# alibaba/graph-gpt

Measured on AMD Instinct MI355X. Metric: graph-tokens/sec (un-padded Eulerian tokens, whole job) + SMTP loss, PCQM4M-v2 base pre-train, higher is better.
Workload: dtype bf16; 1 GPU; pcqm4m-v2-pretrain-base; model=base d768/L12/H12 (122.1M params), per_gpu_batch=256, global_batch=256, seq_len=32, stacked_feat=13, vocab=756, parallelism=dp1, step=fwd+bwd+allreduce+clip+AdamW, reproducible_mode=True

## Files before the change

graph-gpt_amd/_lib.py:

```python
from __future__ import annotations

import contextlib
import ctypes as C
import os

HERE = os.path.dirname(os.path.abspath(__file__))
LIB_PATH = os.environ.get("GGET_LIB_PATH") or os.path.join(HERE, "lib", "libgget_hip.so")

i32, i64, u64, f32, vp, cp = C.c_int32, C.c_int64, C.c_uint64, C.c_float, C.c_void_p, C.c_char_p


class GgetConfig(C.Structure):
    _fields_ = [(n, i32) for n in ("kind", "vocab_size", "hidden_size", "intermediate_size", "num_layers", "num_heads",
                                   "stacked_feat", "next_n_token", "gated_agg", "causal", "max_position", "num_labels",
                                   "score_bias", "pad_token_id")] + \
               [("rms_eps", f32), ("rope_theta", f32), ("layer_scale_init", f32), ("max_tokens", i32), ("max_batch", i32),
                ("path_pdrop", f32), ("mlp_pdrop", f32), ("head_mlp_layers", i32), ("head_mlp", i32 * 4), ("embed_dim", i32)]


class GgetSizes(C.Structure):
    _fields_ = [(n, u64) for n in ("n_params", "param_bf16_bytes", "master_bytes", "adam_bytes", "grad_bf16_bytes",
                                   "workspace_bytes")]


class GgetBuffers(C.Structure):
    _fields_ = [(n, vp) for n in ("param_bf16_dev", "master_dev", "adam_m_dev", "adam_v_dev", "grad_bf16_dev",
                                  "workspace_dev", "rope_cos_dev", "rope_sin_dev")]


class GgetParamInfo(C.Structure):
    _fields_ = [("name", C.c_char * 96), ("ndim", i32), ("shape", i64 * 2), ("offset", u64), ("layer", i32)]


SIGNATURES = {
    "gget_last_error": (cp, []),
    "gget_version": (i32, []),
    "gget_query_sizes": (i32, [C.POINTER(GgetConfig), C.POINTER(GgetSizes)]),
    "gget_create": (i32, [C.POINTER(GgetConfig), C.POINTER(GgetBuffers), C.POINTER(vp)]),
    "gget_destroy": (i32, [vp]),
    "gget_param_count": (i32, [vp]),
    "gget_param_info": (i32, [vp, i32, C.POINTER(GgetParamInfo)]),
    "gget_bucket_count": (i32, [vp]),
    "gget_bucket_range": (i32, [vp, i32, C.POINTER(u64), C.POINTER(u64)]),
    "gget_sync_params": (i32, [vp, vp]),
    "gget_grad_acc_attach": (i32, [vp, vp]),
    "gget_grad_accumulate": (i32, [vp, vp]),
    "gget_grad_acc_count": (i32, [vp, C.POINTER(i32)]),
    "gget_grad_acc_set_count": (i32, [vp, i32]),
    "gget_set_frozen": (i32, [vp, i32]),
    "gget_trainable_ranges": (i32, [vp, vp, vp]),
    "gget_bucket_train_range": (i32, [vp, i32, C.POINTER(u64), C.POINTER(u64)]),
    "gget_ema_attach": (i32, [vp, vp]),
    "gget_set_ema_decay": (i32, [vp, f32]),
    "gget_ema_update": (i32, [vp, f32, vp]),
    "gget_ema_to_params": (i32, [vp, vp]),
    "gget_forward_pretrain": (i32, [vp, vp, vp, vp, vp, vp, i32, i32, vp, vp]),
    "gget_forward_pretrain_packed": (i32, [vp, vp, vp, vp, vp, vp, i32, i32, vp, vp]),
    "gget_forward_task": (i32, [vp, vp, vp, vp, vp, vp, i32, i32, i32, vp, vp, vp, vp]),
    "gget_backward": (i32, [vp, f32, vp]),
    "gget_backward_begin": (i32, [vp, f32, vp]),
    "gget_backward_layer": (i32, [vp, i32, vp]),
    "gget_backward_end": (i32, [vp, vp]),
    "gget_adamw_step": (i32, [vp, f32, f32, f32, f32, f32, f32, f32, i32, vp, vp]),
    "gget_comm_unique_id": (i32, [vp]),
    "gget_comm_init": (i32, [vp, i32, i32, vp]),
    "gget_comm_destroy": (i32, [vp]),
    "gget_comm_move": (i32, [vp, vp]),
    "gget_allreduce_grads_async": (i32, [vp, i32, i32, vp]),
    "gget_allreduce_range_async": (i32, [vp, u64, u64, i32, vp]),
    "gget_comm_init_loopback": (i32, [vp, i32]),
    "gget_shard_plan": (i32, [C.POINTER(GgetConfig), i32, i32, C.POINTER(u64)]),
    "gget_shard_init": (i32, [vp, i32, i32, C.POINTER(i32)]),
    "gget_shard_bucket": (i32, [vp, i32, C.POINTER(u64)]),
    "gget_reduce_scatter_grads_async": (i32, [vp, i32, i32, vp]),
    "gget_shard_sqnorm_partials": (i32, [vp, vp, vp]),
    "gget_shard_allgather_async": (i32, [vp, i32, vp, vp]),
    "gget_adamw_step_sharded": (i32, [vp, f32, f32, f32, f32, f32, f32, f32, i32, vp, vp, vp]),
    "gget_head_counts": (i32, [vp, C.POINTER(i32 * 2), vp]),
    "gget_head_logits": (i32, [vp, C.POINTER(vp), C.POINTER(i32)]),
    "gget_hidden_states": (i32, [vp, C.POINTER(vp)]),
    "gget_layer_hidden_states": (i32, [vp, i32, C.POINTER(vp)]),
    "gget_hidden_states_grid": (i32, [vp, i32, vp, vp]),
    "gget_op_gemm": (i32, [i32, i32, vp, vp, vp, vp, i32, i32, i32, i32, i32, i32, i32, vp]),
    "gget_op_gemm_streamk": (i32, [i32, i32, vp, vp, vp, vp, i32, i32, i32, i32, i32, i32, vp, vp]),
    "gget_op_gemm_streamk_bytes": (u64, []),
    "gget_debug_set": (i32, [i32, i32]),
    "gget_debug_get": (i32, [i32, C.POINTER(i32)]),
    "gget_debug_occupy": (i32, [vp, u64, i32, i32, i32, vp]),
    "gget_op_gemm_grouped": (i32, [i32, i32, vp, vp, vp, vp, vp, vp, vp, vp, vp, vp]),
    "gget_op_rmsnorm_fwd": (i32, [vp, vp, vp, vp, i32, i32, f32, vp]),
    "gget_op_rmsnorm_bwd": (i32, [vp, vp, vp, vp, vp, vp, vp, i32, i32, vp]),
    "gget_op_embed_fwd": (i32, [vp, vp, vp, vp, i32, i32, i32, i32, vp]),
    "gget_op_embed_bwd": (i32, [vp, vp, vp, vp, vp, vp, i32, i32, i32, i32, i32, i32, vp]),
    "gget_op_qkv_rope": (i32, [vp, vp, vp, vp, vp, vp, i32, i32, i32, vp]),
    "gget_op_smtp2d": (i32, [vp, i32, vp, i32, vp, vp, i32, i32, i32, f32, f32, f32, i32, i32, C.c_uint32, vp]),
    "gget_op_token_sample": (i32, [vp, i32, i32, i32, i32, f32, f32, i32, f32, C.c_uint32, vp, vp, vp]),
    "gget_op_unmask_origin": (i32, [vp, vp, i32, i32, f32, C.c_uint32, i32, vp]),
    "gget_op_token_confidence": (i32, [vp, i32, i32, i32, i32, vp, vp, vp]),
    "gget_op_smtp_rows": (i32, [vp, vp, vp, vp, vp, i32, i32, i32, C.c_double, C.c_double, C.c_double, C.c_uint32, vp]),
    "gget_op_rope": (i32, [vp, vp, vp, vp, i32, i32, i32, i32, vp]),
    "gget_op_attn_fwd": (i32, [vp, vp, vp, vp, i32, i32, i32, i32, vp, vp, vp, f32, C.c_uint32, vp]),
    "gget_op_attn_bwd": (i32, [vp, vp, vp, vp, vp, vp, vp, i32, i32, i32, i32, vp, vp, vp, f32, C.c_uint32, vp]),
    "gget_op_copy_from_host": (i32, [vp, vp, C.c_uint64, vp]),
    "gget_op_attn_fwd_varlen": (i32, [vp, vp, vp, vp, vp, i32, i32, i32, i32, vp, vp, vp, i32, f32, C.c_uint32, vp]),
    "gget_op_attn_bwd_varlen": (i32, [vp, vp, vp, vp, vp, vp, vp, vp, i32, i32, i32, i32, vp, vp, vp, i32, f32, C.c_uint32, vp]),
    "gget_op_attn_oproj_fwd": (i32, [vp, vp, vp, vp, vp, vp, vp, vp, vp, vp, vp, i32, i32, i32, i32, f32, f32, C.c_uint32, vp, vp]),
    "gget_op_pack_wo": (i32, [vp, C.c_uint64, vp, vp, i32, i32, vp]),
    "gget_op_attn_oproj_bwd": (i32, [vp, vp, vp, vp, vp, vp, vp, i32, C.c_uint64, vp, vp, vp, vp, vp, vp, i32, i32, i32, i32, vp, vp, vp, f32,
                                      C.c_uint32, i32, vp, vp, vp]),
    "gget_op_attn_fwd_ranges": (i32, [vp, vp, vp, vp, vp, i32, i32, i32, i32, f32, C.c_uint32, vp]),
    "gget_op_attn_bwd_ranges": (i32, [vp, vp, vp, vp, vp, vp, vp, vp, i32, i32, i32, i32, f32, C.c_uint32, vp]),
    "gget_op_ranges_from_mask3d": (i32, [vp, vp, vp, i32, i32, vp]),
    "gget_op_attn_bwd_fused": (i32, [vp, vp, vp, vp, vp, vp, vp, vp, vp, vp, i32, i32, i32, i32, f32, C.c_uint32, vp]),
    "gget_set_dropout": (i32, [vp, f32, f32, C.c_uint32]),
    "gget_set_auc": (i32, [vp, i32, C.c_uint32]),
    "gget_set_token_count": (i32, [vp, C.c_int64]),
    "gget_set_option": (i32, [vp, i32, i32]),
    "gget_set_dp_menu": (i32, [vp, i32, i32]),
    "gget_varlen_status": (i32, [vp, vp, vp]),
    "gget_position_status": (i32, [vp, vp, vp]),
    "gget_deferred_status": (i32, [vp, vp, vp]),
    "gget_set_focal_gamma": (i32, [vp, f32]),
    "gget_set_stack_method": (i32, [vp, i32]),
    "gget_set_rope_range": (i32, [vp, f32]),
    "gget_set_raw_embeds": (i32, [vp, vp, i32]),
    "gget_debug_probe": (i32, [vp, i32, C.POINTER(f32)]),
    "gget_debug_gemm_probe": (i32, [i32, C.POINTER(C.c_double), C.POINTER(C.c_double), C.POINTER(i32), C.POINTER(i32)]),
    "gget_set_dropout_ex": (i32, [vp, f32, f32, f32]),
    "gget_op_gateup_geglu": (i32, [vp, vp, vp, vp, i32, i32, i32, vp]),
    "gget_op_down_dgrad_geglu": (i32, [vp, vp, vp, vp, vp, i32, i32, i32, vp]),
    "gget_op_geglu_fwd": (i32, [vp, vp, i32, i32, vp]),
    "gget_op_geglu_bwd": (i32, [vp, vp, vp, i32, i32, vp]),
    "gget_op_ce_fwd_bwd": (i32, [vp, i32, vp, vp, vp, i32, i32, vp, vp, f32, i32, vp]),
    "gget_op_score_fwd": (i32, [vp, vp, vp, vp, vp, vp, i32, i32, i32, vp]),
    "gget_op_score_bwd": (i32, [vp, vp, vp, vp, vp, vp, vp, i32, i32, i32, vp]),
    "gget_op_tok_score_fwd": (i32, [vp, vp, vp, vp, i32, i32, i32, vp]),
    "gget_op_tok_intra_fwd": (i32, [vp, vp, vp, vp, i32, i32, i32, vp]),
    "gget_op_tok_intra_bwd": (i32, [vp, vp, vp, vp, vp, vp, i32, i32, i32, vp]),
    "gget_set_cls_idx": (i32, [vp, vp]),
    "gget_op_tok_ce": (i32, [vp, vp, vp, vp, vp, i32, i32, vp, i32, vp]),
    "gget_op_tok_score_bwd": (i32, [vp, vp, vp, vp, vp, vp, vp, i32, i32, i32, vp]),
    "gget_op_task_loss": (i32, [vp, vp, vp, i32, i32, i32, vp, vp, vp]),
    "gget_op_auc_loss": (i32, [vp, vp, i32, i32, i32, C.c_uint32, vp, vp, vp, vp]),
    "gget_op_pool_rows": (i32, [vp, vp, vp, i32, i32, vp]),
    "gget_op_scatter_rows_f32": (i32, [vp, vp, vp, i32, i32, vp]),
    "gget_op_head_linear_fwd": (i32, [vp, vp, vp, vp, vp, vp, i32, i32, i32, i32, vp]),
    "gget_op_head_linear_bwd": (i32, [vp, vp, vp, vp, vp, vp, vp, i32, i32, i32, i32, vp]),
    "gget_op_rank_metrics_workspace": (C.c_size_t, [i32, i32]),
    "gget_op_rank_metrics": (i32, [vp, i32, vp, i32, i32, i32, vp, vp, vp, vp, vp, vp, C.c_size_t, vp]),
    "gget_op_link_hits_workspace": (C.c_size_t, [i32]),
    "gget_op_link_hits": (i32, [vp, vp, i32, i64, vp, vp, vp, vp, vp, vp, C.c_size_t, vp]),
    "gget_op_link_mrr_workspace": (C.c_size_t, [i32]),
    "gget_op_link_mrr": (i32, [vp, vp, vp, i32, i32, i32, vp, vp, vp, vp, vp, vp, vp, vp, C.c_size_t, vp]),
}

GEMM_NT, GEMM_NN, GEMM_TN = 0, 1, 2
OPT_NORM_FROM_BACKWARD = 1
OPT_SKIP_NONFINITE_STEP = 2
SHARD_CHUNK = 4096
SHARD_PARAMS, SHARD_MASTER, SHARD_ADAM_M, SHARD_ADAM_V, SHARD_SLOTS, SHARD_EMA = 0, 1, 2, 3, 4, 5
TOKENS_AUTO = -2
EPI_NONE, EPI_RESIDUAL, EPI_ATOMIC_F32, EPI_SLAB_F32 = 0, 1, 2, 3

KEY_GEMM_VARIANT, KEY_GEMM_LDS_HEADROOM, KEY_GEMM_SPLIT_LAST, KEY_DETERMINISTIC, KEY_GEMM_STAGGER = 1, 2, 3, 4, 5
KEY_GEMM_ABLATE, KEY_HEAD_DENSE, KEY_HEAD_TILE, KEY_ATTN_OPROJ_OFF, KEY_LS_NORM_BWD_WIDE = 7, 8, 9, 10, 11
KEY_RMS_WIDE, KEY_CE_PARTS, KEY_GEMM_CU_RESERVE, KEY_OCCUPY_FAT, KEY_LINK_GRID = 13, 14, 15, 16, 18
MENU_KEYS = (1, 2, 3, 4, 5, 7, 8, 9, 10, 11, 13, 14, 15, 16, 18)
GEMM_NO_KSPLIT_ND, GEMM_NO_KSPLIT_WGRAD, GEMM_NO_192_ROWS, GEMM_NO_SPLIT_LAST, GEMM_KSPLIT_128_ONLY, GEMM_ONE_BLOCK_PER_CU = 1, 2, 4, 8, 16, 32
GEMM_KSPLIT_DMA8, GEMM_AREA_RULE = 128, 512


def debug_get(key: int) -> int:
    v = i32()
    check(load().gget_debug_get(int(key), C.byref(v)))
    return int(v.value)


@contextlib.contextmanager
def debug_menu(keys):
    saved = {k: debug_get(k) for k in keys}
    try:
        for k, v in keys.items():
            check(load().gget_debug_set(int(k), int(v)))
        yield
    finally:
        for k, v in saved.items():
            check(load().gget_debug_set(k, v))


def gemm_grouped(lib, mode, problems, stream):
    n = len(problems)
    PA, IA = vp * n, i32 * n
    ptr = lambda k: PA(*[p[k].data_ptr() for p in problems])
    num = lambda k: IA(*[int(p[k]) for p in problems])
    return lib.gget_op_gemm_grouped(mode, n, ptr(0), ptr(1), ptr(2), num(3), num(4), num(5), num(6), num(7), num(8), stream)
PROBLEM_SINGLE_LABEL, PROBLEM_REGRESSION_L1, PROBLEM_REGRESSION_MSE, PROBLEM_MULTI_LABEL, PROBLEM_AUC = 0, 1, 2, 3, 4
PROBLEM_TOKEN_CE_INTRA = 6
PROBLEM_TOKEN_CE = 5

_lib = None


class GgetError(RuntimeError):
    pass


def load(path: str = LIB_PATH):
    global _lib
    if _lib is not None:
        return _lib
    import torch
    if not os.path.exists(path):
        raise GgetError(f"{path} is missing: build it with `python graph-gpt_amd/build.py` "
                        "(or __graft_entry__.build()); this engine has no CPU fallback")
    lib = C.CDLL(path)
    for name, (res, args) in SIGNATURES.items():
        fn = getattr(lib, name)
        fn.restype = res
        fn.argtypes = args
    _lib = lib
    return lib


def check(rc: int):
    if rc != 0:
        raise GgetError(f"gget error {rc}: {load().gget_last_error().decode()}")
```

graph-gpt_amd/build.py:

```python
from __future__ import annotations

import hashlib
import os
import shutil
import subprocess
import sys

HERE = os.path.dirname(os.path.abspath(__file__))
CSRC = os.path.join(HERE, "csrc")
LIBDIR = os.path.join(HERE, "lib")
LIB = os.path.join(LIBDIR, "libgget_hip.so")
SOURCES = ["engine.hip", "gemm.hip", "kernels.hip", "attention.hip", "menu.hip", "metrics.hip"]
HEADERS = ["common.h", "gemm.h", "kernels.h", "menu.h", os.path.join("..", "..", "include", "gget.h")]
FLAGS = ["--offload-arch=gfx950", "-O3", "-std=c++17", "-fPIC", "-fno-gpu-rdc", "-Wall", "-Wno-unused-function"]
EXTRA_FLAGS = {}


def _hipcc() -> str:
    for cand in (os.environ.get("HIPCC"), shutil.which("hipcc"), "/opt/rocm/bin/hipcc"):
        if cand and os.path.exists(cand):
            return cand
    raise RuntimeError("hipcc not found (set HIPCC)")


def _digest() -> str:
    h = hashlib.sha256()
    for f in SOURCES + HEADERS:
        with open(os.path.join(CSRC, f), "rb") as fh:
            h.update(fh.read())
    h.update(" ".join(FLAGS).encode())
    h.update(repr(sorted(EXTRA_FLAGS.items())).encode())
    return h.hexdigest()


def build(force: bool = False, verbose: bool = False) -> str:
    os.makedirs(LIBDIR, exist_ok=True)
    stamp = os.path.join(LIBDIR, "libgget_hip.stamp")
    dig = _digest()
    if not force and os.path.exists(LIB) and os.path.exists(stamp) and open(stamp).read().strip() == dig:
        return LIB
    hipcc = _hipcc()
    objdir = os.path.join(HERE, "build")
    os.makedirs(objdir, exist_ok=True)
    objs = []
    procs = []
    for src in SOURCES:
        obj = os.path.join(objdir, src.replace(".hip", ".o"))
        cmd = [hipcc, *FLAGS, *EXTRA_FLAGS.get(src, []), "-c", os.path.join(CSRC, src), "-o", obj]
        if verbose:
            print(" ".join(cmd), flush=True)
        procs.append((src, subprocess.Popen(cmd, stdout=subprocess.PIPE, stderr=subprocess.STDOUT, text=True)))
        objs.append(obj)
    for src, p in procs:
        out, _ = p.communicate()
        if p.returncode != 0:
            raise RuntimeError(f"hipcc failed on {src}:\n{out}")
        if verbose and out.strip():
            print(out)
    cmd = [hipcc, "--offload-arch=gfx950", "-shared", "-fPIC", "-o", LIB, *objs]
    r = subprocess.run(cmd, stdout=subprocess.PIPE, stderr=subprocess.STDOUT, text=True)
    if r.returncode != 0:
        raise RuntimeError(f"link failed:\n{r.stdout}")
    with open(stamp, "w") as fh:
        fh.write(dig)
    return LIB


if __name__ == "__main__":
    print(build(force="--force" in sys.argv, verbose=True))
```

graph-gpt_amd/csrc/engine.hip:

```cpp
#include <dlfcn.h>
#include <stdarg.h>
#include <stdio.h>
#include <string.h>

#include <algorithm>
#include <chrono>
#include <string>
#include <functional>
#include <vector>

#include "common.h"
#include "gemm.h"
#include "kernels.h"
#include <rccl/rccl.h>

static thread_local char g_err[512] = "";
void gget_set_error(const char* fmt, ...) {
  va_list ap;
  va_start(ap, fmt);
  vsnprintf(g_err, sizeof(g_err), fmt, ap);
  va_end(ap);
}
extern "C" const char* gget_last_error(void) { return g_err; }
extern "C" int gget_version(void) { return 101; }
// ... 1505 lines not shown
    if (int e = k_gather_rows_remap(h->wsp<bf16_t>(w.hidden), h->wsp<int32_t>(w.row_idx), counts, h->wsp<int32_t>(w.vl_pad2c),
                                    h->wsp<bf16_t>(w.Hm), T, d, h->T > h->tc ? h->tc : 0, labels_dev ? h->wsp<int32_t>(w.vl_status) : nullptr, st))
      return e;
  } else if (int e = k_gather_rows(h->wsp<bf16_t>(w.hidden), h->wsp<int32_t>(w.row_idx), counts, h->wsp<bf16_t>(w.Hm), T, d, 0, st))
    return e;
  h->head_sorted_fwd = false;
  if (sorted_head) {
    if (int e = k_head_slot_sort(h->wsp<int32_t>(w.sel_src), h->wsp<int32_t>(w.row_idx), counts + 1, h->wsp<int32_t>(w.ss_state),
                                 h->wsp<int32_t>(w.ss_tok), h->wsp<int32_t>(w.ss_cell), h->wsp<int32_t>(w.ss_l), h->wsp<int32_t>(w.ss_pos),
                                 h->wsp<int32_t>(w.ss_tile), h->wsp<int32_t>(w.ss_total), T * n, n, (long)d * d, head_tile_rows(d), st))
      return e;
    GemmGroup g;
    memset(&g, 0, sizeof(g));
    g.count = 1;
    GemmProblem& p = g.p[0];
    p.A = h->wsp<bf16_t>(w.hidden); p.B = h->P + h->plan.ntp; p.C = h->wsp<bf16_t>(w.Hl);
    p.M = T * n + n * 256; p.N = d; p.K = d; p.lda = d; p.ldb = d; p.ldc = d;
    p.m_dev = h->wsp<int32_t>(w.ss_total);
    p.a_rows = h->wsp<int32_t>(w.ss_tok); p.b_tile_off = h->wsp<int32_t>(w.ss_tile); p.c_rows = h->wsp<int32_t>(w.ss_l);
    p.b_tile_rows = head_tile_rows(d);
    if (int e = gget_gemm_launch(GGET_GEMM_NT, GGET_EPI_NONE, g, 1, st)) return e;
    h->head_sorted_fwd = true;
  } else if (h->plan.has_ntp) {
    if (int e = gemm_nt(h->wsp<bf16_t>(w.Hm), h->P + h->plan.ntp, h->wsp<bf16_t>(w.Pp), nullptr, T, n * d, d, d, d, n * d,
                        counts, st))
      return e;
    if (int e = k_gather_rows(h->wsp<bf16_t>(w.Pp), h->wsp<int32_t>(w.sel_src), counts + 1, h->wsp<bf16_t>(w.Hl), T * n, d, 0,
                              st))
      return e;
  }
  if (int e = gemm_nt(h->wsp<bf16_t>(w.Hl), h->P + h->plan.lm, h->wsp<bf16_t>(w.logits), nullptr, T * n, V, d, d, d, Vp,
                      counts + 1, st))
    return e;
  h->have_labels = labels_dev != nullptr;
  if (h->stack_long && labels_dev) {
    if (int e = k_sample_mask_wgt(labels_dev, h->wsp<float>(w.long_wgt), B, S * n, st)) return e;
    sample_wgt_dev = h->wsp<float>(w.long_wgt);
  }
  h->sample_wgt = sample_wgt_dev;
  if (labels_dev) {
    const int mean_rows = sample_wgt_dev == nullptr;
    const float base = 1.0f / (float)((long)B * S * n);
    if (int e = k_ce_fwd_bwd(h->wsp<bf16_t>(w.logits), Vp, h->wsp<int32_t>(w.sel_label), h->wsp<int32_t>(w.sel_tok),
                             sample_wgt_dev, S, counts + 1, T * n, V, h->wsp<float>(w.loss_sum), h->wsp<bf16_t>(w.dlogits),
                             base, mean_rows, loss_dev, st, mean_rows ? h->focal_gamma : 0.f, h->wsp<float>(w.loss_part), 2048))
      return e;
    if (h->varlen && h->tc_from_caller && loss_dev)
      if (int e = k_poison_loss(h->wsp<int32_t>(w.vl_status), loss_dev, st)) return e;
  }
  h->fwd_valid = true;
  return 0;
}

extern "C" int gget_forward_pretrain(gget_handle_t h, const int64_t* input_ids_dev, const int64_t* attention_mask_dev,
                                     const int64_t* labels_dev, const float* sample_wgt_dev,
                                     const int64_t* position_ids_dev, int B, int S, float* loss_dev, void* stream) {
  return forward_pretrain_impl(h, input_ids_dev, attention_mask_dev, false, labels_dev, sample_wgt_dev, position_ids_dev, B, S,
                               loss_dev, stream);
}

extern "C" int gget_forward_pretrain_packed(gget_handle_t h, const int64_t* input_ids_dev, const int64_t* attention_mask3d_dev,
                                            const int64_t* labels_dev, const float* sample_wgt_dev,
                                            const int64_t* position_ids_dev, int B, int S, float* loss_dev, void* stream) {
  GGET_REQUIRE(attention_mask3d_dev != nullptr, "the packed forward needs the [B,S,S] mask");
  return forward_pretrain_impl(h, input_ids_dev, attention_mask3d_dev, true, labels_dev, sample_wgt_dev, position_ids_dev, B, S,
                               loss_dev, stream);
}

extern "C" int gget_forward_task(gget_handle_t h, const int64_t* input_ids_dev, const int64_t* attention_mask_dev,
                                 const int64_t* position_ids_dev, const void* task_labels_dev, const float* sample_wgt_dev,
                                 int problem_type, int B, int S, float* loss_dev, float* task_logits_dev,
                                 void* task_hidden_dev, void* stream) {
  GGET_REQUIRE(h != nullptr, "null argument");
  const long tc_hint = h->tc_next;
  h->tc_next = -1;
  const int64_t* cls_idx_dev = h->cls_idx_next;
  h->cls_idx_next = nullptr;
  GGET_REQUIRE(input_ids_dev, "null argument");
  GGET_REQUIRE(h->cfg.kind == GGET_KIND_TASK, "handle was not created as a task model");
  const bool tok = problem_type == GGET_PROBLEM_TOKEN_CE || problem_type == GGET_PROBLEM_TOKEN_CE_INTRA;
  GGET_REQUIRE(problem_type != GGET_PROBLEM_TOKEN_CE_INTRA || cls_idx_dev, "the intra-instance token head needs cls_idx (gget_set_cls_idx)");
  hipStream_t st = (hipStream_t)stream;
  const gget_config_t& c = h->cfg;
  CallScope scope(h);
  h->fwd_valid = false;
  if (int e = backbone_forward(h, tc_hint, input_ids_dev, c.stacked_feat, attention_mask_dev, position_ids_dev, B, S, st, false, nullptr))
    return e;
  const Ws& w = h->ws;
  const int d = c.hidden_size, C = c.num_labels;
  float* lg = h->wsp<float>(w.tlogits);
  GGET_REQUIRE(!tok || h->plan.n_lin == 0, "the token-level head is the Linear `score` (no MLP head)");
  if (h->plan.n_lin > 0) {
    const Plan& pl = h->plan;
    if (int e = k_pool_rows(h->wsp<bf16_t>(w.hidden), h->wsp<int32_t>(w.pool_row), h->wsp<bf16_t>(w.pooled_h), B, d, st)) return e;
    for (int i = 0; i < pl.n_lin; ++i)
      if (int e = k_head_linear_fwd(h->wsp<bf16_t>(w.head_x[i]), h->wsp<bf16_t>(w.head_a[i]), h->P + pl.head_w[i],
                                    c.score_bias ? h->P + pl.head_b[i] : nullptr, h->wsp<bf16_t>(w.head_x[i + 1]),
                                    i + 1 == pl.n_lin ? lg : nullptr, B, pl.head_dim[i], pl.head_dim[i + 1], i, h->head_drop(), st))
        return e;
  } else if (problem_type == GGET_PROBLEM_TOKEN_CE) {
    if (int e = k_tok_score_fwd(h->wsp<bf16_t>(w.hidden), h->P + h->plan.score, c.score_bias ? h->P + h->plan.sbias : nullptr, lg, h->T, C,
                                d, st))
      return e;
    if (int e = k_pool_rows(h->wsp<bf16_t>(w.hidden), h->wsp<int32_t>(w.pool_row), h->wsp<bf16_t>(w.pooled_h), B, d, st)) return e;
  } else if (problem_type == GGET_PROBLEM_TOKEN_CE_INTRA) {
    if (int e = k_intra_plan(cls_idx_dev, h->wsp<int32_t>(w.key_len), h->varlen ? h->wsp<int32_t>(w.vl_cu) : nullptr, h->wsp<int32_t>(w.intra_rs),
                             h->wsp<int64_t>(w.intra_cls), h->wsp<int32_t>(w.vl_status) + 4, B, S, C, st))
      return e;
    if (int e = k_tok_intra_fwd(h->wsp<bf16_t>(w.hidden), h->wsp<int32_t>(w.intra_rs), h->wsp<int64_t>(w.intra_cls), lg, B, C, d, st)) return e;
    if (int e = k_pool_rows(h->wsp<bf16_t>(w.hidden), h->wsp<int32_t>(w.pool_row), h->wsp<bf16_t>(w.pooled_h), B, d, st)) return e;
  } else if (int e = k_score_fwd(h->wsp<bf16_t>(w.hidden), h->wsp<int32_t>(w.pool_row), h->P + h->plan.score,
                                 c.score_bias ? h->P + h->plan.sbias : nullptr, lg, h->wsp<bf16_t>(w.pooled_h), B, C, d, st))
    return e;
  const int rows = tok ? h->T : B;
  const bool tok_vl = tok && h->varlen;
  if (task_logits_dev && tok_vl) {
    GGET_HIP_CHECK(hipMemsetAsync(task_logits_dev, 0, (size_t)B * S * C * 4, st));
    if (int e = k_scatter_rows_map_f32(lg, h->wsp<int32_t>(w.vl_c2p), task_logits_dev, h->T, C, B * S, st)) return e;
  } else if (task_logits_dev) GGET_HIP_CHECK(hipMemcpyAsync(task_logits_dev, lg, (size_t)rows * C * 4, hipMemcpyDeviceToDevice, st));
  if (task_hidden_dev)
    GGET_HIP_CHECK(hipMemcpyAsync(task_hidden_dev, h->wsp<bf16_t>(w.pooled_h), (size_t)B * d * 2, hipMemcpyDeviceToDevice, st));
  h->have_labels = task_labels_dev != nullptr;
  h->problem = problem_type;
  if (task_labels_dev) {
    GGET_REQUIRE(loss_dev != nullptr, "loss_dev is required when task labels are given");
    if (problem_type == GGET_PROBLEM_AUC) {
      GGET_REQUIRE(C >= 2, "the AUC loss reads logits[:, 1] - logits[:, 0]");
      if (int e = k_auc_loss(lg, (const int64_t*)task_labels_dev, B, C, h->auc_num_neg, h->auc_seed, loss_dev,
                             h->wsp<float>(w.tdlogits), h->wsp<int32_t>(w.auc_lists), st))
        return e;
    } else if (tok) {
      if (int e = k_tok_ce(lg, (const int64_t*)task_labels_dev, h->wsp<float>(w.tdlogits), h->wsp<float>(w.tok_stat), loss_dev, rows, C, st,
                           tok_vl ? h->wsp<int32_t>(w.vl_c2p) : nullptr, B * S))
        return e;
    } else if (int e = k_task_loss(lg, task_labels_dev, sample_wgt_dev, problem_type, B, C, loss_dev, h->wsp<float>(w.tdlogits), st))
      return e;
    if (h->varlen && h->tc_from_caller)
      if (int e = k_poison_loss(h->wsp<int32_t>(w.vl_status), loss_dev, st)) return e;
  }
  h->fwd_valid = true;
  return 0;
}

namespace {

int convert_bucket(gget_engine* h, int bucket, hipStream_t st) {
  if (h->defer_convert) return 0;
  if (h->truncated() && h->bucket_train_range(bucket).second == 0) return 0;
  const auto& bs = h->bucket_segs[bucket];
  return k_convert_segments(h->wsp<float>(h->ws.scratch32), h->G,
                            reinterpret_cast<const GgetSegment*>(h->W + h->ws.segs) + bs.first, bs.second, st);
}

int layer_backward(gget_engine* h, int i, hipStream_t st) {
  const gget_config_t& c = h->cfg;
  const int T = h->T, d = c.hidden_size, ff = c.intermediate_size, H = c.num_heads;
  const LayerOff& lo = h->plan.layers[i];
  const LayerWs& lw = h->ws.lw[i];
  const Ws& w = h->ws;
  float* s32 = h->wsp<float>(w.scratch32);
  bf16_t* bufs[3] = {h->wsp<bf16_t>(w.dxa), h->wsp<bf16_t>(w.dxb), h->wsp<bf16_t>(w.dxc)};
  bf16_t* dx_out = h->dx_cur;
  int oi = 0;
  while (oi < 3 && bufs[oi] != dx_out) ++oi;
  GGET_REQUIRE(oi < 3, "backward stages called out of order");
  bf16_t* dx_mid = bufs[(oi + 1) % 3];
  bf16_t* dx_in = bufs[(oi + 2) % 3];
  bf16_t* x_in = h->wsp<bf16_t>(w.xres[i]);
  bf16_t* xmid = h->wsp<bf16_t>(lw.xmid);
  bf16_t* dxn = h->wsp<bf16_t>(w.dxn);
  bf16_t* dqkv = h->wsp<bf16_t>(w.dqkv);
  bf16_t* dattn = h->wsp<bf16_t>(w.dattn);
  bf16_t* dgu = h->wsp<bf16_t>(w.dgu);
  bf16_t* dh = h->wsp<bf16_t>(w.dh);
  const bf16_t* dy_down = dx_out;
  const bf16_t* dy_o = nullptr;
  const int ls_rl = 256 / (d / 8);
  dim3 lsgrid((unsigned)std::min(512, (T + ls_rl - 1) / ls_rl));
  const size_t ls_lds_bytes = (size_t)ls_rl * d * sizeof(float);
  const bool fuse_ls = h->plan.has_res && ls_norm_fused();
  if (h->plan.has_res) {
    bf16_t* dsc = h->wsp<bf16_t>(w.dscaled);
    if (!h->ls2_done)
      hipLaunchKernelGGL(ls_bwd_kernel, lsgrid, dim3(256), ls_lds_bytes, st, dx_out, h->wsp<bf16_t>(lw.mraw),
                         h->plan.has_ls ? h->P + lo.lam2 : nullptr, dsc, h->plan.has_ls ? s32 + lo.lam2_32 : nullptr, T, d,
                         h->path_drop(i, 1), kAccumCopies, align_up((uint64_t)d, 128), h->mlp_drop(i));
    h->ls2_done = false;
    dy_down = dsc;
  }
  if (h->mlp_drop_p > 0.f) {
    if (int e = gemm_nn(dy_down, h->P + lo.wdown, dh, T, ff, d, d, ff, ff, nullptr, st)) return e;
    if (int e = k_elem_dropout(dh, T, ff, GGET_DROP_STREAM_MLP_ACT, h->mlp_drop(i), st)) return e;
    if (int e = k_geglu_bwd(h->wsp<bf16_t>(lw.gu), dh, dgu, T, ff, st)) return e;
  } else if (int e = down_dgrad_geglu(dy_down, h->P + lo.wdown, h->wsp<bf16_t>(lw.gu), dgu, dh, T, d, ff, st)) return e;
  if (int e = gemm_nn(dgu, h->P + lo.wgu, dxn, T, d, 2 * ff, 2 * ff, d, d, nullptr, st)) return e;
  bool front_fused = false;
  const bool ao_bwd_ok = menu().gemm_cu_reserve > 0 ? h->B <= gget_gemm_num_cu() : menu().gemm_lds_headroom < 2;
  if (!h->plan.has_res && !h->klo() && h->wo_packed && ao_bwd_ok) {
    int taken = 0;
    if (int e = k_attn_oproj_bwd(dxn, xmid, h->P + lo.ln2, h->wsp<float>(lw.rstd2), dx_out, dx_mid, s32 + lo.ln2_32, kAccumCopies,
                                 align_up((uint64_t)d, 128), h->wsp<bf16_t>(w.wot_pack) + (size_t)i * d * d, h->wsp<bf16_t>(lw.qkv),
                                 h->wsp<float>(lw.lse), h->wsp<int32_t>(w.key_len), h->row_base(), dqkv, h->B, h->S, H, c.causal, h->cos_cur,
                                 h->sin_cur, h->pos_cur, h->attn_drop_p, h->attn_drop_seed + 0x9E37u * (unsigned)i, T, st, &taken,
                                 dattn, h->long_list()))
      return e;
    front_fused = taken != 0;
  }
  if (front_fused) {
  } else if (fuse_ls) {
    if (int e = rmsnorm_bwd_ls(dxn, xmid, h->P + lo.ln2, h->wsp<float>(lw.rstd2), dx_out, dx_mid, s32 + lo.ln2_32, h->wsp<bf16_t>(lw.araw),
                               h->plan.has_ls ? h->P + lo.lam1 : nullptr, h->wsp<bf16_t>(w.dscaled2),
                               h->plan.has_ls ? s32 + lo.lam1_32 : nullptr, T, d, h->path_drop(i, 0), ElemDropArg{0, 1.f, 0}, st))
      return e;
  } else if (int e = k_rmsnorm_bwd(dxn, xmid, h->P + lo.ln2, h->wsp<float>(lw.rstd2), dx_out, dx_mid, s32 + lo.ln2_32, T, d, st, kAccumCopies, align_up((uint64_t)d, 128)))
    return e;
  dy_o = dx_mid;
  if (fuse_ls) {
    dy_o = h->wsp<bf16_t>(w.dscaled2);
  } else if (h->plan.has_res) {
    bf16_t* dsc = h->wsp<bf16_t>(w.dscaled2);
    hipLaunchKernelGGL(ls_bwd_kernel, lsgrid, dim3(256), ls_lds_bytes, st, dx_mid, h->wsp<bf16_t>(lw.araw),
                       h->plan.has_ls ? h->P + lo.lam1 : nullptr, dsc, h->plan.has_ls ? s32 + lo.lam1_32 : nullptr, T, d,
                       h->path_drop(i, 0), kAccumCopies, align_up((uint64_t)d, 128), ElemDropArg{0, 1.f, 0});
    dy_o = dsc;
  }
  if (!front_fused)
  if (int e = gemm_nn(dy_o, h->P + lo.wo, dattn, T, d, d, d, d, d, nullptr, st)) return e;
  if (!front_fused)
  if (int e = k_attn_bwd(h->wsp<bf16_t>(lw.qkv), h->wsp<bf16_t>(lw.attn), dattn, h->wsp<float>(lw.lse),
                         h->wsp<int32_t>(w.key_len), dqkv, h->wsp<float>(w.delta), h->B, h->S, H, c.causal, h->cos_cur,
                         h->sin_cur, h->pos_cur, 1, h->attn_drop_p, h->attn_drop_seed + 0x9E37u * (unsigned)i, st,
                         h->klo(), h->khi(), h->row_base(),
                         (w.dq_acc && (uint64_t)(h->S + 255) / 256 <= (c.max_tokens / (c.max_batch > 0 ? c.max_batch : 1) + 255) / 256) ? h->wsp<bf16_t>(w.dq_acc) : nullptr,
                         (size_t)c.max_tokens * d, h->long_list()))
    return e;
  if (int e = gemm_nn(dqkv, h->P + lo.wqkv, dxn, T, d, 3 * d, 3 * d, d, d, nullptr, st)) return e;
  const bool boundary = h->truncated() && i == h->frozen;
  const bool fuse_next = fuse_ls && i > 0 && !boundary;
  if (boundary) {
    if (int e = k_rmsnorm_dw(dxn, x_in, h->wsp<float>(lw.rstd1), s32 + lo.ln1_32, T, d, st, kAccumCopies, align_up((uint64_t)d, 128))) return e;
  } else if (!fuse_next)
    if (int e = k_rmsnorm_bwd(dxn, x_in, h->P + lo.ln1, h->wsp<float>(lw.rstd1), dx_mid, dx_in, s32 + lo.ln1_32, T, d, st, kAccumCopies, align_up((uint64_t)d, 128)))
      return e;
  const GemmProblem wg_gu{dgu, h->wsp<bf16_t>(lw.xn2), h->G + lo.wgu, nullptr, 2 * ff, d, T, 2 * ff, d, d, nullptr, nullptr, 0, 0};
  const GemmProblem wg_dn{dy_down, h->wsp<bf16_t>(lw.h), h->G + lo.wdown, nullptr, d, ff, T, d, ff, ff, nullptr, nullptr, 0, 0};
  const long t192[4] = {(long)2 * ff * d / (192 * 192), (long)d * ff / (192 * 192), (long)3 * d * d / (192 * 192), (long)d * d / (192 * 192)};
  int n_grouped = 4;
  if (d % 192 == 0 && ff % 192 == 0 && menu().gemm_cu_reserve > 0) {
    long acc_t = 0;
    n_grouped = 0;
    for (int q = 0; q < 4 && acc_t + t192[q] <= gget_gemm_num_cu(); ++q) { acc_t += t192[q]; ++n_grouped; }
    if (n_grouped < 2) n_grouped = 4;
  }
  if (d % 192 == 0 && ff % 192 == 0) {
    GemmGroup g;
    memset(&g, 0, sizeof(g));
    g.count = n_grouped;
    g.p[0] = wg_gu;
    g.p[1] = wg_dn;
    g.p[2] = GemmProblem{dqkv, h->wsp<bf16_t>(lw.xn1), h->G + lo.wqkv, nullptr, 3 * d, d, T, 3 * d, d, d, nullptr, nullptr, 0, 0};
    g.p[3] = GemmProblem{dy_o, h->wsp<bf16_t>(lw.attn), h->G + lo.wo, nullptr, d, d, T, d, d, d, nullptr, nullptr, 0, 0};
    const long wg_tiles = ((long)2 * ff * d + (long)d * ff + (long)4 * d * d) / (192 * 192);
    g.sq_partials = n_grouped == 4 && h->opt_norm_from_backward && wg_tiles <= kSqTilesPerLayer ? h->wsp<float>(w.sq_tiles) + (size_t)i * kSqTilesPerLayer : nullptr;
    if (h->probe) GGET_HIP_CHECK(hipEventRecord(h->probe_event(0, 2 * i), st));
    if (int e = gget_gemm_launch(GGET_GEMM_TN, GGET_EPI_NONE, g, 1, st)) return e;
    if (h->probe) GGET_HIP_CHECK(hipEventRecord(h->probe_event(0, 2 * i + 1), st));
    if (g.sq_written) {
      if (wg_tiles < kSqTilesPerLayer)
        GGET_HIP_CHECK(hipMemsetAsync(h->wsp<float>(w.sq_tiles) + (size_t)i * kSqTilesPerLayer + wg_tiles, 0, (kSqTilesPerLayer - wg_tiles) * sizeof(float), st));
      ++h->sq_layers;
    }
    if (n_grouped < 4) {
      float* wg = h->wsp<float>(w.wg32);
      const bool with_qkv = n_grouped == 2;
      const long slab = with_qkv ? (long)4 * d * d : (long)d * d;
      const int max_slabs = with_qkv ? kWgSplit : 4 * kWgSplit;
      const int rows_out = with_qkv ? 4 * d : d;
      const int t_big = ((rows_out + 255) / 256) * ((d + 127) / 128), t_small = ((rows_out + 127) / 128) * ((d + 127) / 128);
      int split = fit_split(t_big, max_slabs);
      if (t_big * split < 160) split = fit_split(t_small, max_slabs);
      while (split > 1 && (T + 63) / 64 < 4 * split) --split;
      GemmGroup go;
      memset(&go, 0, sizeof(go));
      if (with_qkv) {
        go.count = 2;
        go.p[0] = GemmProblem{dqkv, h->wsp<bf16_t>(lw.xn1), wg, nullptr, 3 * d, d, T, 3 * d, d, d, nullptr, nullptr, 0, 0, slab};
        go.p[1] = GemmProblem{dy_o, h->wsp<bf16_t>(lw.attn), wg + (size_t)3 * d * d, nullptr, d, d, T, d, d, d, nullptr, nullptr, 0, 0, slab};
      } else {
        go.count = 1;
        go.p[0] = GemmProblem{dy_o, h->wsp<bf16_t>(lw.attn), wg, nullptr, d, d, T, d, d, d, nullptr, nullptr, 0, 0, slab};
      }
      if (int e = gget_gemm_launch(GGET_GEMM_TN, GGET_EPI_SLAB_F32, go, split, st)) return e;
      const int ktiles = (T + 63) / 64, per = (ktiles + split - 1) / split;
      if (int e = k_slab_reduce(wg, slab, (ktiles + per - 1) / per, h->G + (with_qkv ? lo.wqkv : lo.wo), (size_t)slab, st)) return e;
    }
  } else {
    {
      GemmGroup g;
      memset(&g, 0, sizeof(g));
      g.count = 2;
      g.p[0] = wg_gu;
      g.p[1] = wg_dn;
      if (int e = gget_gemm_launch(GGET_GEMM_TN, GGET_EPI_NONE, g, 1, st)) return e;
    }
    float* wg = h->wsp<float>(w.wg32);
    const long slab = (long)4 * d * d;
    GemmGroup g;
    memset(&g, 0, sizeof(g));
    g.count = 2;
    g.p[0] = GemmProblem{dqkv, h->wsp<bf16_t>(lw.xn1), wg, nullptr, 3 * d, d, T, 3 * d, d, d, nullptr, nullptr, 0, 0, slab};
    g.p[1] = GemmProblem{dy_o, h->wsp<bf16_t>(lw.attn), wg + (size_t)3 * d * d, nullptr, d, d, T, d, d, d, nullptr, nullptr, 0, 0, slab};
    const int split = T >= kWgSplit * 1024 ? kWgSplit : 1;
    if (int e = gget_gemm_launch(GGET_GEMM_TN, GGET_EPI_SLAB_F32, g, split, st)) return e;
    if (int e = k_slab_reduce(wg, slab, split, h->G + lo.wqkv, (size_t)4 * d * d, st)) return e;
  }
  if (fuse_next) {
    const LayerOff& lp = h->plan.layers[i - 1];
    if (int e = rmsnorm_bwd_ls(dxn, x_in, h->P + lo.ln1, h->wsp<float>(lw.rstd1), dx_mid, dx_in, s32 + lo.ln1_32,
                               h->wsp<bf16_t>(h->ws.lw[i - 1].mraw), h->plan.has_ls ? h->P + lp.lam2 : nullptr, h->wsp<bf16_t>(w.dscaled),
                               h->plan.has_ls ? s32 + lp.lam2_32 : nullptr, T, d, h->path_drop(i - 1, 1), h->mlp_drop(i - 1), st))
      return e;
    h->ls2_done = true;
  }
  h->dx_cur = dx_in;
  return convert_bucket(h, h->bucket_of_layer(i), st);
}

}

static bool embed_dense_path(int T, int d, int V, bool gated, const ElemDropArg& E) {
  return !menu().embed_sorted && E.thresh == 0 && k_embed_dense_ok(V, gated) && T > 0 && ((long)V * d) % 4 == 0;
}

extern "C" int gget_backward_begin(gget_handle_t h, float loss_scale, void* stream) {
  GGET_REQUIRE(h, "null handle");
  GGET_REQUIRE(h->fwd_valid && h->have_labels, "backward needs a preceding forward with labels");
  GGET_REQUIRE(loss_scale == 1.0f, "loss scaling is not used on the bf16 path (pass 1.0)");
  h->sq_layers = 0;
  CallScope scope(h);
  hipStream_t st = (hipStream_t)stream;
  const gget_config_t& c = h->cfg;
  const Ws& w = h->ws;
  const int d = c.hidden_size;
  float* s32 = h->wsp<float>(w.scratch32);
  GgetZeroRanges zr;
  zr.n = 0;
  zr.add(s32, (size_t)h->plan.n_scratch32 * 4);
  bf16_t* dhid = h->wsp<bf16_t>(w.dxb);
  zr.add(dhid, (size_t)h->T * d * 2);
  if (h->varlen && h->T > h->tc)
    zr.add(h->wsp<bf16_t>(w.dqkv) + (size_t)h->tc * 3 * d, (size_t)(h->T - h->tc) * 3 * d * 2);
  int T = h->TP;
  if (c.kind == GGET_KIND_PRETRAIN) {
    if (h->plan.has_ntp && head_scatter_fused())
      zr.add(h->wsp<bf16_t>(w.dP), (size_t)(h->varlen ? h->T : T) * c.next_n_token * d * 2);
    zr.add(h->wsp<float>(w.lm_slab), (size_t)kLmSplit * c.vocab_size * d * sizeof(float));
  }
  h->emb_cnt_cleared = false;
  if (h->ws.emb_cnt && embed_dense_path(h->T, d, c.vocab_size, h->plan.has_gate, h->embed_drop()) && zr.n < kZeroRanges &&
      !h->truncated()) {
    zr.add(h->wsp<unsigned char>(h->ws.emb_cnt), (size_t)h->T * align_up((uint64_t)c.vocab_size, 64) * 2);
    h->emb_cnt_cleared = true;
  }
  if (int e = k_zero_ranges(zr, st)) return e;
  if (c.kind == GGET_KIND_PRETRAIN) {
    const int n = c.next_n_token, V = c.vocab_size, Vp = (int)align_up(V, 64);
    int32_t* counts = h->wsp<int32_t>(w.counts);
    bf16_t* dlog = h->wsp<bf16_t>(w.dlogits);
    const bool fuse_sc = h->plan.has_ntp && head_scatter_fused();
    if (fuse_sc) {
      if (int e = gemm_nn(dlog, h->P + h->plan.lm, h->wsp<bf16_t>(w.dP), T * n, d, Vp, Vp, d, d, counts + 1, st, h->wsp<int32_t>(w.sel_src)))
        return e;
    } else if (int e = gemm_nn(dlog, h->P + h->plan.lm, h->wsp<bf16_t>(w.dHl), T * n, d, Vp, Vp, d, d, counts + 1, st)) return e;
    {
      float* slabs = h->wsp<float>(w.lm_slab);
      const long slab = (long)V * d;
      GemmGroup g;
      memset(&g, 0, sizeof(g));
      g.count = 1;
      g.p[0] = GemmProblem{dlog, h->wsp<bf16_t>(w.Hl), slabs, nullptr, V, d, T * n, Vp, d, d, nullptr, counts + 1, 0, 0, slab};
      int lm_split = fit_split(((V + 255) / 256) * ((d + 127) / 128), kLmSplit);
      if (((V + 255) / 256) * ((d + 127) / 128) * lm_split < 160) lm_split = fit_split(((V + 127) / 128) * ((d + 127) / 128), kLmSplit);
      if (int e = gget_gemm_launch(GGET_GEMM_TN, GGET_EPI_SLAB_F32, g, lm_split, st)) return e;
      if (int e = k_slab_reduce(slabs, slab, lm_split, h->G + h->plan.lm, (size_t)V * d, st)) return e;
    }
    if (h->plan.has_ntp) {
      bf16_t* dP = h->wsp<bf16_t>(w.dP);
      if (!fuse_sc) {
        GGET_HIP_CHECK(hipMemsetAsync(dP, 0, (size_t)(h->varlen ? h->T : T) * n * d * 2, st));
        if (int e = k_gather_rows(h->wsp<bf16_t>(w.dHl), h->wsp<int32_t>(w.sel_src), counts + 1, dP, T * n, d, 1, st)) return e;
      }
      if (h->head_sorted_fwd) {
        bf16_t* dxs = h->wsp<bf16_t>(w.Pp);
        GemmGroup g;
        memset(&g, 0, sizeof(g));
        g.count = 1;
        GemmProblem& p = g.p[0];
        p.A = dP; p.B = h->P + h->plan.ntp; p.C = dxs;
        p.M = T * n + n * 256; p.N = d; p.K = d; p.lda = d; p.ldb = d; p.ldc = d;
        p.m_dev = h->wsp<int32_t>(w.ss_total);
        p.a_rows = h->wsp<int32_t>(w.ss_cell); p.b_tile_off = h->wsp<int32_t>(w.ss_tile);
        p.b_tile_rows = head_tile_rows(d);
        if (int e = gget_gemm_launch(GGET_GEMM_NN, GGET_EPI_NONE, g, 1, st)) return e;
        if (int e = k_head_cell_sum(dxs, h->wsp<int32_t>(w.ss_pos), h->wsp<int32_t>(w.cnt), h->wsp<int32_t>(w.l_off),
                                    h->varlen ? h->wsp<int32_t>(w.vl_pad2c) : nullptr, dhid, T, d, h->T > h->tc ? h->tc : 0, st))
          return e;
      } else if (head_scatter_fused()) {
        if (int e = gemm_nn(dP, h->P + h->plan.ntp, dhid, T, d, n * d, n * d, d, d, counts, st, h->wsp<int32_t>(w.row_idx))) return e;
      } else if (int e = gemm_nn(dP, h->P + h->plan.ntp, h->wsp<bf16_t>(w.dHm), T, d, n * d, n * d, d, d, counts, st)) return e;
      if (int e = gget_gemm_single(GGET_GEMM_TN, GGET_EPI_NONE, dP, h->wsp<bf16_t>(w.Hm), h->G + h->plan.ntp, nullptr, n * d, d,
                                   T, n * d, d, d, nullptr, counts, 1, st, true))
        return e;
    }
    if (!(h->plan.has_ntp && (head_scatter_fused() || h->head_sorted_fwd)))
      if (int e = k_gather_rows(h->wsp<bf16_t>(w.dHm), h->wsp<int32_t>(w.row_idx), counts, dhid, T, d, 1, st)) return e;
  } else if (h->plan.n_lin > 0) {
    const Plan& pl = h->plan;
    const float* dy = h->wsp<float>(w.tdlogits);
    for (int i = pl.n_lin - 1; i >= 0; --i) {
// ... 269 lines not shown
                          float grad_scale, int step, const float* slots_dev, float* gnorm_dev, hipStream_t st) {
  GgetAdamwArgs a{};
  a.master = h->master, a.m = h->am, a.v = h->av, a.param = h->P;
  a.lr = lr, a.beta1 = beta1, a.beta2 = beta2, a.eps = eps, a.wd = weight_decay, a.step = step;
  a.max_norm = max_grad_norm, a.grad_scale = grad_scale, a.gnorm_out = gnorm_dev, a.skip_nonfinite = h->opt_skip_nonfinite;
  a.ema_decay = h->ema_decay_next;
  h->ema_decay_next = -1.f;
  a.ema = a.ema_decay >= 0.f ? h->ema : nullptr;
  h->wo_packed = false;
  float* sq = h->wsp<float>(h->ws.sqnorm);
  const bool need_norm = h->step_needs_norm(max_grad_norm, gnorm_dev);
  a.sqnorm = need_norm ? sq : nullptr;
  a.grad_f32 = h->grad_from_acc();
  a.grad = h->grad_src();
  h->grad_acc_count = 0;
  const OptWork* w = h->opt_work(sharded);
  if (need_norm) {
    if (sharded) {
      if (int e = k_grad_sqnorm_slots(slots_dev, w->slot_of, w->nglobal, sq, st)) return e;
    } else if (w) {
      if (int e = k_grad_sqnorm_chunks(a.grad, w->chunks, w->nchunks, nullptr, 0, sq, st, a.grad_f32)) return e;
    } else if (h->opt_norm_from_backward && !a.grad_f32 && grad_scale == 1.0f && h->sq_layers == h->cfg.num_layers && h->n_sq_chunks >= 0) {
      if (int e = k_grad_sqnorm_chunks(h->G, h->wsp<GgetSqChunk>(h->ws.sq_chunks), h->n_sq_chunks, h->wsp<float>(h->ws.sq_tiles),
                                       h->cfg.num_layers * kSqTilesPerLayer, sq, st))
        return e;
    } else if (int e = k_grad_sqnorm(a.grad, h->plan.n_params, sq, st, a.grad_f32)) return e;
  }
  return w ? k_adamw_items(a, w->items, w->nitems, st) : k_adamw(a, h->plan.n_params, st);
}

extern "C" int gget_adamw_step(gget_handle_t h, float lr, float beta1, float beta2, float eps, float weight_decay,
                               float max_grad_norm, float grad_scale, int step, float* gnorm_dev, void* stream) {
  GGET_REQUIRE(h && h->master && h->am && h->av, "adamw needs master/m/v arenas");
  GGET_REQUIRE(step >= 1, "step is 1-based");
  return optimizer_step(h, false, lr, beta1, beta2, eps, weight_decay, max_grad_norm, grad_scale, step, nullptr, gnorm_dev, (hipStream_t)stream);
}

extern "C" int gget_shard_plan(const gget_config_t* cfg, int world, int bucket, uint64_t out[5]) {
  if (int e = check_cfg(cfg)) return e;
  GGET_REQUIRE(out && world >= 1, "shard_plan: bad arguments (world %d)", world);
  GGET_REQUIRE(bucket >= 0 && bucket < cfg->num_layers + 2, "shard_plan: bucket %d out of range", bucket);
  const auto r = bucket_ranges(*cfg, make_plan(*cfg))[bucket];
  const ShardBucket sb = shard_bucket(r.first, r.second - r.first, world);
  out[0] = sb.off, out[1] = sb.cnt, out[2] = sb.slice, out[3] = sb.tail_off, out[4] = sb.tail_cnt;
  return 0;
}

extern "C" int gget_shard_init(gget_handle_t h, int world, int rank, int32_t* slots_per_rank) {
  GGET_REQUIRE(h && world >= 0 && (world == 0 || (rank >= 0 && rank < world)), "shard_init: bad arguments (rank %d world %d)", rank, world);
  GGET_REQUIRE(world == 0 || !(h->comm || h->comm_loopback) || (world == h->comm_world && rank == h->comm_rank),
               "shard_init: rank %d of %d does not match the communicator (rank %d of %d)", rank, world, h->comm_rank, h->comm_world);
  if (int e = h->shard_work.reset()) return e;
  h->shard_world = h->shard_rank = h->shard_slots = 0;
  h->shard_plan.clear();
  if (slots_per_rank) *slots_per_rank = 0;
  if (world == 0) return 0;
  const bool all_ranks = h->comm_loopback;
  const uint64_t C = GGET_SHARD_CHUNK;
  std::vector<ShardBucket> plan;
  for (int b = 0; b < (int)h->bucket_range.size(); ++b) {
    const auto r = h->bucket_train_range(b);
    plan.push_back(shard_bucket(r.first, r.second, world));
  }
  std::vector<GgetSqChunk> grid;
  std::vector<int> owner;
  for (const ShardBucket& b : plan)
    for (uint64_t j = 0; j * C < b.cnt; ++j) {
      grid.push_back(GgetSqChunk{b.off + j * C, std::min(C, b.cnt - j * C)});
      owner.push_back(j * C < (uint64_t)world * b.slice ? (int)(j * C / b.slice) : 0);
    }
  std::vector<int> count(world, 0);
  std::vector<int32_t> local(grid.size());
  for (size_t j = 0; j < grid.size(); ++j) local[j] = count[owner[j]]++;
  const int S = *std::max_element(count.begin(), count.end());
  std::vector<int32_t> slot_of(grid.size()), chunk_slot;
  std::vector<GgetSqChunk> chunks;
  for (size_t j = 0; j < grid.size(); ++j) {
    slot_of[j] = owner[j] * S + local[j];
    if (all_ranks || owner[j] == rank) {
      chunks.push_back(grid[j]);
      chunk_slot.push_back(slot_of[j]);
    }
  }
  std::vector<std::pair<uint64_t, uint64_t>> share;
  for (const ShardBucket& b : plan) {
    for (int r = 0; r < world; ++r)
      if (all_ranks || r == rank) share.push_back({b.off + (uint64_t)r * b.slice, b.slice});
    share.push_back({b.tail_off, b.tail_cnt});
  }
  if (int e = h->shard_work.upload(cut_items(share), chunks, chunk_slot, slot_of)) return e;
  h->shard_world = world;
  h->shard_rank = rank;
  h->shard_slots = S;
  h->shard_plan = plan;
  if (slots_per_rank) *slots_per_rank = S;
  return 0;
}

extern "C" int gget_shard_bucket(gget_handle_t h, int bucket, uint64_t out[5]) {
  GGET_REQUIRE(h != nullptr && out != nullptr, "shard_bucket: null argument");
  GGET_REQUIRE(h->shard_world > 0, "shard_bucket: no plan is active (gget_shard_init)");
  GGET_REQUIRE(bucket >= 0 && bucket < (int)h->shard_plan.size(), "shard_bucket: bucket %d out of range", bucket);
  const ShardBucket& sb = h->shard_plan[bucket];
  out[0] = sb.off, out[1] = sb.cnt, out[2] = sb.slice, out[3] = sb.tail_off, out[4] = sb.tail_cnt;
  return 0;
}

extern "C" int gget_shard_sqnorm_partials(gget_handle_t h, float* slots_dev, void* stream) {
  GGET_REQUIRE(h && h->shard_world > 0 && slots_dev, "shard_sqnorm_partials: call gget_shard_init first (and pass the slot vector)");
  const OptWork& w = h->shard_work;
  return k_grad_sqnorm_partials(h->grad_src(), w.chunks, w.chunk_slot, w.nchunks, slots_dev, (hipStream_t)stream, h->grad_from_acc());
}

extern "C" int gget_adamw_step_sharded(gget_handle_t h, float lr, float beta1, float beta2, float eps, float weight_decay,
                                       float max_grad_norm, float grad_scale, int step, const float* slots_dev, float* gnorm_dev, void* stream) {
  GGET_REQUIRE(h && h->master && h->am && h->av, "adamw needs master/m/v arenas");
  GGET_REQUIRE(h->shard_world > 0, "adamw_step_sharded: call gget_shard_init first");
  GGET_REQUIRE(step >= 1, "step is 1-based");
  GGET_REQUIRE(slots_dev || !h->step_needs_norm(max_grad_norm, gnorm_dev), "adamw_step_sharded: the norm needs the gathered partial vector");
  return optimizer_step(h, true, lr, beta1, beta2, eps, weight_decay, max_grad_norm, grad_scale, step, slots_dev, gnorm_dev, (hipStream_t)stream);
}

extern "C" int gget_head_counts(gget_handle_t h, int32_t counts[2], void* stream) {
  GGET_REQUIRE(h && counts, "null argument");
  GGET_REQUIRE(h->cfg.kind == GGET_KIND_PRETRAIN, "head counts exist only for the pre-train head");
  GGET_HIP_CHECK(hipMemcpyAsync(counts, h->wsp<int32_t>(h->ws.counts), 8, hipMemcpyDeviceToHost, (hipStream_t)stream));
  GGET_HIP_CHECK(hipStreamSynchronize((hipStream_t)stream));
  return 0;
}

extern "C" int gget_head_logits(gget_handle_t h, const void** logits_dev, int32_t* ld) {
  GGET_REQUIRE(h && logits_dev && ld, "null argument");
  GGET_REQUIRE(h->cfg.kind == GGET_KIND_PRETRAIN, "head logits exist only for the pre-train head");
  *logits_dev = h->wsp<bf16_t>(h->ws.logits);
  *ld = (int32_t)align_up(h->cfg.vocab_size, 64);
  return 0;
}

extern "C" int gget_hidden_states(gget_handle_t h, const void** hidden_dev) {
  GGET_REQUIRE(h && hidden_dev, "null argument");
  GGET_REQUIRE(!h->varlen, "hidden_states: the last forward ran on the var-len token layout (rows are compacted): run that forward on the padded grid - no token count at the C ABI, num_tokens=None with a host-side mask or GGET_VARLEN=0 through the model classes, or ask the model for output_hidden_states=True");
  *hidden_dev = h->wsp<bf16_t>(h->ws.hidden);
  return 0;
}

extern "C" int gget_layer_hidden_states(gget_handle_t h, int layer, const void** hidden_dev) {
  GGET_REQUIRE(h && hidden_dev, "null argument");
  GGET_REQUIRE(layer >= 0 && layer <= h->cfg.num_layers, "layer_hidden_states: layer %d out of range", layer);
  GGET_REQUIRE(!h->varlen, "layer_hidden_states: the last forward ran on the var-len token layout (rows are compacted): run that forward on the padded grid - no token count at the C ABI, num_tokens=None with a host-side mask or GGET_VARLEN=0 through the model classes, or ask the model for output_hidden_states=True");
  *hidden_dev = h->wsp<bf16_t>(h->ws.xres[layer]);
  return 0;
}

extern "C" int gget_hidden_states_grid(gget_handle_t h, int layer, void* out_dev, void* stream) {
  GGET_REQUIRE(h && out_dev, "null argument");
  GGET_REQUIRE(layer >= -1 && layer <= h->cfg.num_layers, "hidden_states_grid: layer %d out of range", layer);
  GGET_REQUIRE(h->B > 0 && h->S > 0, "hidden_states_grid: no forward has run");
  const bf16_t* src = layer < 0 ? h->wsp<bf16_t>(h->ws.hidden) : h->wsp<bf16_t>(h->ws.xres[layer]);
  const int d = h->cfg.hidden_size;
  const long n_pos = (long)h->B * h->S;
  if (!h->varlen) {
    GGET_HIP_CHECK(hipMemcpyAsync(out_dev, src, (size_t)n_pos * d * 2, hipMemcpyDeviceToDevice, (hipStream_t)stream));
    return 0;
  }
  return k_rows_to_grid(src, h->wsp<int32_t>(h->ws.vl_pad2c), out_dev, n_pos, d, (hipStream_t)stream);
}

__global__ void __launch_bounds__(256) occupy_kernel(float* buf, size_t n, long long ticks) {
  extern __shared__ float occ_lds[];
  const long long t0 = wall_clock64();
  float acc = 0.f;
  size_t i = ((size_t)blockIdx.x * 256 + threadIdx.x) % n;
  while (wall_clock64() - t0 < ticks) {
    acc += buf[i];
    i = (i + 65536) % n;
    if (threadIdx.x == 0) occ_lds[0] = acc;
  }
  if (acc == 1.2345e-30f) buf[0] = acc;
}
__global__ void __launch_bounds__(256) occupy_fat_kernel(float* buf, size_t n, long long ticks) {
  extern __shared__ float occ_lds[];
  asm volatile("" ::: "v255", "a7");
  const long long t0 = wall_clock64();
  float acc = 0.f;
  size_t i = ((size_t)blockIdx.x * 256 + threadIdx.x) % n;
  while (wall_clock64() - t0 < ticks) {
    acc += buf[i];
    i = (i + 65536) % n;
    if (threadIdx.x == 0) occ_lds[0] = acc;
  }
  if (acc == 1.2345e-30f) buf[0] = acc;
}
extern "C" int gget_debug_occupy(void* scratch, uint64_t scratch_bytes, int blocks, int lds_bytes, int microseconds, void* stream) {
  GGET_REQUIRE(scratch && scratch_bytes >= 4096 && blocks > 0 && lds_bytes >= 4 && lds_bytes <= 160 * 1024, "debug_occupy: bad arguments");
  static bool attr = false;
  if (!attr) {
    GGET_HIP_CHECK(hipFuncSetAttribute(reinterpret_cast<const void*>(&occupy_kernel), hipFuncAttributeMaxDynamicSharedMemorySize, 160 * 1024));
    GGET_HIP_CHECK(hipFuncSetAttribute(reinterpret_cast<const void*>(&occupy_fat_kernel), hipFuncAttributeMaxDynamicSharedMemorySize, 160 * 1024));
    attr = true;
  }
  if (menu().occupy_fat) {
    hipLaunchKernelGGL(occupy_fat_kernel, dim3(blocks), dim3(256), lds_bytes, (hipStream_t)stream, (float*)scratch, scratch_bytes / 4,
                       (long long)microseconds * 100);
    GGET_LAUNCH_CHECK();
    return 0;
  }
  hipLaunchKernelGGL(occupy_kernel, dim3(blocks), dim3(256), lds_bytes, (hipStream_t)stream, (float*)scratch, scratch_bytes / 4,
                     (long long)microseconds * 100);
  GGET_LAUNCH_CHECK();
  return 0;
}

extern "C" int gget_debug_probe(gget_handle_t h, int enable, float* avg_ms_out ) {
  GGET_REQUIRE(h != nullptr, "null handle");
  if (avg_ms_out) {
    for (int w = 0; w < 2; ++w) {
      double sum = 0.0;
      int n = 0;
      for (size_t k = 0; k + 1 < h->probe_ev[w].size(); k += 2) {
        float ms = 0.f;
        if (hipEventSynchronize(h->probe_ev[w][k + 1]) == hipSuccess && hipEventElapsedTime(&ms, h->probe_ev[w][k], h->probe_ev[w][k + 1]) == hipSuccess) {
          sum += ms;
          ++n;
        }
      }
      avg_ms_out[w] = n ? (float)(sum / n) : 0.f;
    }
  }
  h->probe = enable != 0;
  return 0;
}
extern "C" int gget_op_gemm(int mode, int epilogue, const void* A, const void* B, void* C, const void* R, int M, int N, int K,
                            int lda, int ldb, int ldc, int split_k, void* stream) {
  return gget_gemm_single(mode, epilogue, A, B, C, R, M, N, K, lda, ldb, ldc, nullptr, nullptr, split_k, (hipStream_t)stream);
}
extern "C" int gget_op_gemm_streamk(int mode, int epilogue, const void* A, const void* B, void* C, const void* R, int M, int N, int K,
                                    int lda, int ldb, int ldc, void* streamk_ws, void* stream) {
  GGET_REQUIRE(streamk_ws != nullptr, "gemm_streamk: null workspace");
  gget_gemm_streamk_workspace(streamk_ws);
  const int rc = gget_gemm_single(mode, epilogue, A, B, C, R, M, N, K, lda, ldb, ldc, nullptr, nullptr, 1, (hipStream_t)stream);
  gget_gemm_streamk_workspace(nullptr);
  return rc;
}
extern "C" uint64_t gget_op_gemm_streamk_bytes(void) { return gget_gemm_streamk_bytes(); }
extern "C" int gget_op_gemm_grouped(int mode, int count, const void* const* A, const void* const* B, void* const* Cs, const int* M,
                                   const int* N, const int* K, const int* lda, const int* ldb, const int* ldc, void* stream) {
  GGET_REQUIRE(count >= 1 && count <= GGET_MAX_GROUP && A && B && Cs && M && N && K && lda && ldb && ldc, "gemm_grouped: bad arguments");
  GemmGroup g;
  memset(&g, 0, sizeof(g));
  g.count = count;
  for (int i = 0; i < count; ++i) {
    GemmProblem& p = g.p[i];
    p.A = static_cast<const bf16_t*>(A[i]); p.B = static_cast<const bf16_t*>(B[i]); p.C = Cs[i];
    p.M = M[i]; p.N = N[i]; p.K = K[i]; p.lda = lda[i]; p.ldb = ldb[i]; p.ldc = ldc[i];
  }
  return gget_gemm_launch(mode, GGET_EPI_NONE, g, 1, (hipStream_t)stream);
}
extern "C" int gget_op_qkv_rope(const void* x, const void* wqkv, void* qkv, const float* cos_tab, const float* sin_tab,
                                const int64_t* position_ids, int T, int S, int d, void* stream) {
  GGET_REQUIRE(x && wqkv && qkv && cos_tab && sin_tab, "qkv_rope: null argument");
  GGET_REQUIRE(d > 0 && d % 64 == 0 && T > 0 && S > 0, "qkv_rope: bad shape T %d S %d d %d", T, S, d);
  GemmGroup g;
  memset(&g, 0, sizeof(g));
  g.count = 1;
  GemmProblem& p = g.p[0];
  p.A = static_cast<const bf16_t*>(x); p.B = static_cast<const bf16_t*>(wqkv); p.C = qkv;
  p.M = T; p.N = 3 * d; p.K = d; p.lda = d; p.ldb = d; p.ldc = 3 * d;
  p.rope_cos = cos_tab; p.rope_sin = sin_tab; p.rope_pos = position_ids; p.rope_S = S; p.rope_cols = 2 * d;
  return gget_gemm_launch(GGET_GEMM_NT, GGET_EPI_ROPE, g, 1, (hipStream_t)stream);
}
extern "C" int gget_op_smtp2d(const int64_t* ids_in, int ld_in, const int64_t* node_idx, int ld_node, int64_t* ids_out,
                              int64_t* labels_out, int B, int S, int F, float smtp_2d_rate, float power, float replace_rate,
                              int vocab, int global_2d_mask, uint32_t seed, void* stream) {
  GGET_REQUIRE(ids_in && node_idx && ids_out && labels_out, "smtp2d: null argument");
  GGET_REQUIRE(B >= 0 && S >= 0 && F >= 1 && ld_in >= F && ld_node >= 1 && vocab >= 2, "smtp2d: bad shape");
  return k_smtp2d(ids_in, ld_in, node_idx, ld_node, ids_out, labels_out, B, S, F, smtp_2d_rate, power, replace_rate, vocab,
                  global_2d_mask, seed, (hipStream_t)stream);
}
extern "C" int gget_op_token_sample(const void* logits, int ld, int R, int V, int mode, float temperature, float top_p, int top_k,
                                   float alg_temp, uint32_t seed, float* conf, int64_t* tok, void* stream) {
  GGET_REQUIRE(logits && conf && tok && R >= 0 && V >= 1 && ld >= V && mode >= 0 && mode <= 2, "token_sample: bad arguments");
  return k_token_sample(logits, ld, R, V, mode, temperature, top_p, top_k, alg_temp, seed, conf, tok, (hipStream_t)stream);
}
extern "C" int gget_op_unmask_origin(int64_t* x, const int64_t* cand, int B, int N, float p_transfer, uint32_t seed, int mask_token_id,
                                     void* stream) {
  GGET_REQUIRE(x && cand && B >= 0 && N >= 0, "unmask_origin: bad arguments");
  return k_unmask_origin(x, cand, B, N, p_transfer, seed, mask_token_id, (hipStream_t)stream);
}
extern "C" int gget_op_token_confidence(const void* logits, int ld, int R, int V, int mode, float* conf, int64_t* tok, void* stream) {
  GGET_REQUIRE(logits && conf && tok, "token_confidence: null argument");
  GGET_REQUIRE(R >= 0 && V >= 2 && ld >= V && mode >= 0 && mode <= 2, "token_confidence: bad arguments (R %d V %d ld %d mode %d)", R, V, ld, mode);
  return k_token_confidence(logits, ld, R, V, mode, conf, tok, (hipStream_t)stream);
}
extern "C" int gget_op_smtp_rows(const int64_t* ids_in, const int32_t* lengths, int64_t* ids_out, int64_t* labels_out,
                                 float* wgt_out, int B, int S, int F, double umr_min, double umr_max, double power, uint32_t seed,
                                 void* stream) {
  GGET_REQUIRE(ids_in && lengths && ids_out && labels_out, "smtp_rows: null argument");
  GGET_REQUIRE(B >= 0 && S >= 1 && F >= 1 && (long)S * F < (1l << 20), "smtp_rows: bad shape (S*F must be < 2^20)");
  GGET_REQUIRE(0.0 <= umr_min && umr_min <= umr_max && umr_max <= 1.0 && power > 0.0, "smtp_rows: bad schedule");
  return k_smtp_rows(ids_in, lengths, ids_out, labels_out, wgt_out, B, S, F, umr_min, umr_max, power, seed, (hipStream_t)stream);
}
extern "C" int gget_op_rmsnorm_fwd(const void* x, const void* w, void* y, float* rstd, int T, int d, float eps, void* stream) {
  return k_rmsnorm_fwd(x, w, y, rstd, T, d, eps, (hipStream_t)stream);
}
extern "C" int gget_op_rmsnorm_bwd(const void* dy, const void* x, const void* w, const float* rstd, const void* dres, void* dx,
                                   float* dw_accum, int T, int d, void* stream) {
  return k_rmsnorm_bwd(dy, x, w, rstd, dres, dx, dw_accum, T, d, (hipStream_t)stream);
}
extern "C" int gget_op_embed_fwd(const int64_t* ids, const void* emb, const void* gate, void* out, int T, int F, int ldF, int d,
                                 void* stream) {
  return k_embed_fwd(ids, emb, gate, out, T, F, ldF, d, (hipStream_t)stream);
}
extern "C" int gget_op_embed_bwd(const int64_t* ids, const void* dx, const void* emb, const void* gate, float* demb_accum,
                                 float* dgate_accum, int T, int F, int ldF, int d, int V, int pad_id, void* stream) {
  int32_t* ws = nullptr;
  GGET_HIP_CHECK(hipMalloc(&ws, k_embed_bwd_ws_elems((size_t)T * F, (size_t)V) * sizeof(int32_t)));
  void* cnt = nullptr;
  if (k_embed_dense_ok(V, gate != nullptr))
    GGET_HIP_CHECK(hipMalloc(&cnt, (size_t)T * align_up((uint64_t)V, 64) * 2 + (size_t)kEmbDenseSplit * V * d * 4));
  void* slab = cnt ? static_cast<unsigned char*>(cnt) + (size_t)T * align_up((uint64_t)V, 64) * 2 : nullptr;
  const int rc = embed_bwd(ids, dx, emb, gate, demb_accum, dgate_accum, T, F, ldF, d, V, pad_id, ws, cnt, slab, (hipStream_t)stream,
                           ElemDropArg{0, 1.f, 0});
  (void)hipStreamSynchronize((hipStream_t)stream);
  (void)hipFree(ws);
  if (cnt) (void)hipFree(cnt);
  return rc;
}
extern "C" int gget_op_rope(void* qkv, const float* cos_tab, const float* sin_tab, const int64_t* position_ids, int B, int S,
                            int H, int inverse, void* stream) {
  return k_rope(qkv, cos_tab, sin_tab, position_ids, B * S, S, H, inverse, (hipStream_t)stream);
}
extern "C" int gget_op_attn_fwd(const void* qkv, const int32_t* key_len, void* out, float* lse, int B, int S, int H, int causal,
                                const float* cos_tab, const float* sin_tab, const int64_t* position_ids, float dropout_p,
                                uint32_t dropout_seed, void* stream) {
  return k_attn_fwd(qkv, key_len, out, lse, B, S, H, causal, cos_tab, sin_tab, position_ids, dropout_p, dropout_seed,
                    (hipStream_t)stream);
}
extern "C" int gget_op_attn_oproj_fwd(const void* qkv, const int32_t* key_len, const int32_t* row_base, void* attn_out, float* lse,
                                      const void* wo, const void* x_in, void* x_mid, const void* norm_w, void* xn, float* rstd, int B, int S,
                                      int H, int causal, float eps, float dropout_p, uint32_t dropout_seed, void* stream, int32_t* taken) {
  GGET_REQUIRE(qkv && attn_out && wo && x_in && x_mid && norm_w && xn && taken, "null argument");
  int t = 0;
  const int rc = k_attn_oproj_fwd(qkv, key_len, row_base, attn_out, lse, wo, x_in, x_mid, norm_w, xn, rstd, B, S, H, causal, eps, dropout_p,
                                  dropout_seed, (hipStream_t)stream, &t);
  *taken = t;
  return rc;
}
extern "C" int gget_op_pack_wo(const void* w, uint64_t layer_stride, void* fwd, void* bwd, int d, int layers, void* stream) {
  GGET_REQUIRE(w && fwd && bwd, "null argument");
  return k_pack_wo(w, (size_t)layer_stride, fwd, bwd, d, layers, (hipStream_t)stream);
}
extern "C" int gget_op_attn_oproj_bwd(const void* dxn, const void* x_mid, const void* norm_w, const float* rstd, const void* dres, void* dx_mid,
                                      float* dw_accum, int copies, uint64_t copy_stride, const void* wot_packed, const void* qkv, const float* lse,
                                      const int32_t* key_len, const int32_t* row_base, void* dqkv, int B, int S, int H, int causal,
                                      const float* cos_tab, const float* sin_tab, const int64_t* position_ids, float dropout_p,
                                      uint32_t dropout_seed, int t_rows, void* stream, int32_t* taken, void* dattn_long) {
  GGET_REQUIRE(dxn && x_mid && norm_w && rstd && dres && dx_mid && dw_accum && wot_packed && qkv && lse && dqkv && taken, "null argument");
  int t = 0;
  const int rc = k_attn_oproj_bwd(dxn, x_mid, norm_w, rstd, dres, dx_mid, dw_accum, copies, copy_stride, wot_packed, qkv, lse, key_len, row_base,
                                  dqkv, B, S, H, causal, cos_tab, sin_tab, position_ids, dropout_p, dropout_seed, t_rows, (hipStream_t)stream, &t,
                                  dattn_long, nullptr);
  *taken = t;
  return rc;
}
extern "C" int gget_op_attn_fwd_ranges(const void* qkv, const int32_t* key_lo, const int32_t* key_hi, void* out, float* lse, int B,
                                       int S, int H, int causal, float dropout_p, uint32_t dropout_seed, void* stream) {
  GGET_REQUIRE(key_lo && key_hi, "attn_fwd_ranges: null ranges");
  return k_attn_fwd(qkv, nullptr, out, lse, B, S, H, causal, nullptr, nullptr, nullptr, dropout_p, dropout_seed,
                    (hipStream_t)stream, key_lo, key_hi);
}
extern "C" int gget_op_attn_bwd_ranges(const void* qkv, const void* out, const void* dout, const float* lse, const int32_t* key_lo,
                                       const int32_t* key_hi, void* dqkv, float* delta_ws, int B, int S, int H, int causal,
                                       float dropout_p, uint32_t dropout_seed, void* stream) {
  GGET_REQUIRE(key_lo && key_hi, "attn_bwd_ranges: null ranges");
  return k_attn_bwd(qkv, out, dout, lse, nullptr, dqkv, delta_ws, B, S, H, causal, nullptr, nullptr, nullptr, 0, dropout_p,
                    dropout_seed, (hipStream_t)stream, key_lo, key_hi);
}
extern "C" int gget_op_ranges_from_mask3d(const int64_t* mask3d, int32_t* key_lo, int32_t* key_hi, int B, int S, void* stream) {
  GGET_REQUIRE(mask3d && key_lo && key_hi, "ranges_from_mask3d: null argument");
  return k_ranges_from_mask3d(mask3d, key_lo, key_hi, B, S, (hipStream_t)stream);
}
extern "C" int gget_op_attn_bwd(const void* qkv, const void* out, const void* dout, const float* lse, const int32_t* key_len,
                                void* dqkv, float* delta_ws, int B, int S, int H, int causal, const float* cos_tab,
                                const float* sin_tab, const int64_t* position_ids, float dropout_p, uint32_t dropout_seed,
                                void* stream) {
  return k_attn_bwd(qkv, out, dout, lse, key_len, dqkv, delta_ws, B, S, H, causal, cos_tab, sin_tab, position_ids,
                    0, dropout_p, dropout_seed, (hipStream_t)stream);
}
extern "C" int gget_op_copy_from_host(const void* src_pinned_host, void* dst_dev, uint64_t bytes, void* stream) {
  GGET_REQUIRE(src_pinned_host && dst_dev, "copy_from_host: null argument");
  return k_copy_from_host(src_pinned_host, dst_dev, (size_t)bytes, (hipStream_t)stream);
}
extern "C" int gget_op_attn_fwd_varlen(const void* qkv, const int32_t* key_len, const int32_t* row_base, void* out, float* lse, int B, int S,
                                       int H, int causal, const float* cos_tab, const float* sin_tab, const int64_t* position_ids,
                                       int qk_rotated, float dropout_p, uint32_t dropout_seed, void* stream) {
  GGET_REQUIRE(qkv && key_len && row_base && out, "attn_fwd_varlen: null argument");
  return k_attn_fwd(qkv, key_len, out, lse, B, S, H, causal, qk_rotated ? nullptr : cos_tab, qk_rotated ? nullptr : sin_tab,
                    qk_rotated ? nullptr : position_ids, dropout_p, dropout_seed, (hipStream_t)stream, nullptr, nullptr, row_base);
}
extern "C" int gget_op_attn_bwd_varlen(const void* qkv, const void* out, const void* dout, const float* lse, const int32_t* key_len,
                                       const int32_t* row_base, void* dqkv, float* delta_ws, int B, int S, int H, int causal,
                                       const float* cos_tab, const float* sin_tab, const int64_t* position_ids, int qk_rotated,
                                       float dropout_p, uint32_t dropout_seed, void* stream) {
  GGET_REQUIRE(qkv && dout && key_len && row_base && dqkv, "attn_bwd_varlen: null argument");
  return k_attn_bwd(qkv, out, dout, lse, key_len, dqkv, delta_ws, B, S, H, causal, cos_tab, sin_tab, position_ids, qk_rotated, dropout_p,
                    dropout_seed, (hipStream_t)stream, nullptr, nullptr, row_base);
}
extern "C" int gget_op_attn_bwd_fused(const void* qkv, const void* out, const void* dout, const float* lse, const int32_t* key_len,
                                      const int32_t* key_lo, const int32_t* key_hi, void* dqkv, float* delta_ws, void* dq_ws, int B, int S,
// ... 357 lines not shown
```

graph-gpt_amd/csrc/gemm.h:

```cpp
#pragma once
#include <hip/hip_runtime.h>
#include "../../include/gget.h"
#include "common.h"

#define GGET_MAX_GROUP 4

struct GemmProblem {
  const bf16_t* A;
  const bf16_t* B;
  void* C;
  const bf16_t* R;
  int M, N, K;
  int lda, ldb, ldc;
  const int* m_dev;
  const int* k_dev;
  int tiles_n, tile_begin;
  long slab_stride;
  const float* rope_cos;
  const float* rope_sin;
  const int64_t* rope_pos;
  int rope_S, rope_cols;
  int k_pad_zero;
  void* C2;
  const bf16_t* G;
  int ldc2, ldg, ff;
  const int* c_rows;
  const int* a_rows;
  const int* b_tile_off;
  int b_tile_rows;
};

struct GemmGroup {
  GemmProblem p[GGET_MAX_GROUP];
  int count;
  int super;
  int ablate;
  float* sk_partial;
  unsigned* sk_flags;
  unsigned sk_epoch;
  int sk_rounds, sk_rem, sk_parts, sk_a;
  unsigned* cu_slots;
  int stagger_ticks;
  float* sq_partials;
  int sq_written;
};

constexpr size_t kStreamKBlocks = 512;
constexpr size_t kStreamKSlotBytes = (size_t)128 * 192 * 4;
constexpr size_t kStreamKFlagBytes = (kStreamKBlocks + 64) * sizeof(unsigned);
inline size_t gget_gemm_streamk_bytes() { return kStreamKFlagBytes + kStreamKBlocks * kStreamKSlotBytes; }
void gget_gemm_streamk_workspace(void* ws);

int gget_gemm_num_cu();

int gget_gemm_launch(int mode, int epi, GemmGroup& g, int split_k, hipStream_t st);
int gget_gemm_single(int mode, int epi, const void* A, const void* B, void* C, const void* R, int M, int N, int K,
                     int lda, int ldb, int ldc, const int* m_dev, const int* k_dev, int split_k, hipStream_t st, bool k_pad_zero = false,
                     const int* c_rows = nullptr);
```

graph-gpt_amd/csrc/gemm.hip:

```cpp
#include <stdlib.h>
#include <string.h>
#include <deque>

#include "common.h"
#include "gemm.h"

#define LDS_AS __attribute__((address_space(3)))

int gget_gemm_num_cu() {
  static int dev_cus = 0;
  if (!dev_cus) {
    int dev = 0;
    hipDeviceProp_t prop;
    dev_cus = (hipGetDevice(&dev) == hipSuccess && hipGetDeviceProperties(&prop, dev) == hipSuccess && prop.multiProcessorCount > 0)
                  ? prop.multiProcessorCount : 256;
  }
  const LaunchMenu& m = menu();
  int n = (m.gemm_num_cu > 0 ? m.gemm_num_cu : dev_cus) - (m.gemm_cu_reserve > 0 ? m.gemm_cu_reserve : 0);
  if (m.gemm_cu_reserve > 0) n &= ~7;
  return n < 8 ? 8 : n;
}

namespace {

// ... 747 lines not shown
    }
  }

  Ctx ic, cc;
  int ir = 0, ik = 0, cr = 0, ck = 0;
  bool ivalid = tile_at(0, ic);
  bool cvalid = ivalid;
  cc = ic;
  int islot = 0, cslot = 0, inflight = 0;
  const unsigned lds0 = __builtin_amdgcn_readfirstlane((unsigned)(uintptr_t)(LDS_AS const void*)smem) + (unsigned)wave * 1024u;
  const unsigned char* kA = nullptr;
  const unsigned char* kB = nullptr;
  long strideA = 0, strideB = 0;
  unsigned islot_off = lds0;
  unsigned offA[TA::PIECES], offB[TB::PIECES];
  auto load_issue_tile = [&]() {
    if (!ivalid) return;
    const GemmProblem& P = g.p[ic.pi];
    strideA = A_MC ? (long)BK * P.lda * 2 : (long)BK * 2;
    strideB = B_MC ? (long)BK * P.ldb * 2 : (long)BK * 2;
    kA = reinterpret_cast<const unsigned char*>(P.A) + (SK ? ic.kb * strideA : 0);
    kB = reinterpret_cast<const unsigned char*>(P.B) + (SK ? ic.kb * strideB : 0);
    if (P.b_tile_off)
      kB += (long)__builtin_amdgcn_readfirstlane(P.b_tile_off[__builtin_amdgcn_readfirstlane(ic.m0) / BM]) * 2;
#pragma unroll
    for (int i = 0; i < TA::PIECES; ++i) offA[i] = TA::piece_off(P.lda, ic.m0, ic.M, wave, lane, i, A_MC ? nullptr : P.a_rows);
#pragma unroll
    for (int i = 0; i < TB::PIECES; ++i) {
      if constexpr (EPI == GGET_EPI_GEGLU_FWD) offB[i] = TB::template piece_off_geglu<BN / WN>(P.ldb, ic.n0, P.ff, wave, lane, i);
      else offB[i] = TB::piece_off(P.ldb, ic.n0, P.N, wave, lane, i);
    }
  };
  load_issue_tile();
  auto issue_piece = [&](int q) {
    if (q < TA::PIECES) glds16m(kA, offA[q < TA::PIECES ? q : 0], islot_off + (unsigned)(q * TA::NWAVES * 1024));
    else glds16m(kB, offB[q >= TA::PIECES ? q - TA::PIECES : 0], islot_off + (unsigned)(A_BYTES + (q - TA::PIECES) * TB::NWAVES * 1024));
  };
  auto issue_advance = [&]() {
    islot = islot == NSLOT - 1 ? 0 : islot + 1;
    islot_off = islot == 0 ? lds0 : islot_off + (unsigned)STAGE;
    ++inflight;
    kA += strideA;
    kB += strideB;
    if (++ik == ic.nk) { ik = 0; ++ir; ivalid = tile_at(ir, ic); load_issue_tile(); }
  };
  auto issue_next = [&]() {
    if (!ivalid) return;
#pragma unroll
    for (int q = 0; q < PIECES; ++q) issue_piece(q);
    issue_advance();
  };
#pragma unroll
  for (int i = 0; i < NSLOT - 1; ++i) issue_next();
  auto wait_oldest = [&]() {
    if (inflight == NSLOT - 1) vm_wait<(NSLOT - 2) * PIECES>();
    else vm_wait<0>();
  };
  auto finish_tile = [&]() {
    const GemmProblem& P = g.p[cc.pi];
    bool store = true;
    if constexpr (SK) {
      typedef __attribute__((address_space(1))) unsigned gu32;
      constexpr int SLOT4 = BM * BN / 4;
      if (!cc.owner) {
        float4* slot = reinterpret_cast<float4*>(g.sk_partial) + (size_t)cc.slot * SLOT4;
#pragma unroll
        for (int i = 0; i < MI; ++i)
#pragma unroll
          for (int j = 0; j < NJ; ++j)
            slot[(i * NJ + j) * NT + tid] = make_float4(acc[i][j][0], acc[i][j][1], acc[i][j][2], acc[i][j][3]);
        asm volatile("s_waitcnt vmcnt(0)" ::: "memory");
        __syncthreads();
        if (tid == 0) {
          __builtin_amdgcn_fence(__ATOMIC_RELEASE, "agent");
          asm volatile("s_waitcnt vmcnt(0)" ::: "memory");
          __hip_atomic_store((gu32*)(g.sk_flags + cc.slot), g.sk_epoch, __ATOMIC_RELAXED, __HIP_MEMORY_SCOPE_AGENT);
        }
        store = false;
      } else {
        for (int w = 0; w < cc.nwait; ++w) {
          const int sl = cc.slot + w * g.sk_rem;
          if (tid == 0) {
            unsigned spins = 0;
            while (__hip_atomic_load((gu32*)(g.sk_flags + sl), __ATOMIC_RELAXED, __HIP_MEMORY_SCOPE_AGENT) != g.sk_epoch) {
              __builtin_amdgcn_s_sleep(2);
              if (++spins > (1u << 24)) {
                __hip_atomic_store((gu32*)(g.sk_flags + kStreamKBlocks), 1u, __ATOMIC_RELAXED, __HIP_MEMORY_SCOPE_AGENT);
                break;
              }
            }
            __builtin_amdgcn_fence(__ATOMIC_ACQUIRE, "agent");
          }
          __syncthreads();
          const float4* slot = reinterpret_cast<const float4*>(g.sk_partial) + (size_t)sl * SLOT4;
#pragma unroll
          for (int i = 0; i < MI; ++i)
#pragma unroll
            for (int j = 0; j < NJ; ++j) {
              const float4 v = slot[(i * NJ + j) * NT + tid];
              acc[i][j][0] += v.x; acc[i][j][1] += v.y; acc[i][j][2] += v.z; acc[i][j][3] += v.w;
            }
        }
      }
    }
    if (store && (g.ablate != 32 || acc[0][0][0] == 123.456f))
      store_tile<EPI, MI, NJ, ILV>(acc, P, cc.M, (P.N + 3) & ~3, cc.m0 + wm * (MI * 16),
                                   EPI == GGET_EPI_GEGLU_FWD ? (cc.n0 >> 1) + wn * (NJ * 8) : cc.n0 + wn * (ILV ? 16 : NJ * 16), lane, 0, wn * 16);
#pragma unroll
    for (int i = 0; i < MI; ++i)
#pragma unroll
      for (int j = 0; j < NJ; ++j) acc[i][j] = f32x4_t{0.f, 0.f, 0.f, 0.f};
    ck = 0;
    ++cr;
    cvalid = tile_at(cr, cc);
  };
  while (cvalid) {
    wait_oldest();
    __syncthreads();
    const bool did = ivalid;
    --inflight;
    {
      const unsigned char* a_l = smem + cslot * STAGE;
      const unsigned char* b_l = a_l + A_BYTES;
      constexpr int KK = BK / 32, NG = KK * MI;
      bf16x8_t af[KK][MI], bf[KK][NJ];
#pragma unroll
      for (int kk = 0; kk < KK; ++kk) {
#pragma unroll
        for (int i = 0; i < MI; ++i) af[kk][i] = TA::frag(a_l, wm * MI + i, kk, lane);
#pragma unroll
        for (int j = 0; j < NJ; ++j) bf[kk][j] = TB::frag(b_l, ILV ? (j >> 1) * 4 + (j & 1) * 2 + wn : wn * NJ + j, kk, lane);
      }
#pragma unroll
      for (int kk = 0; kk < KK; ++kk)
#pragma unroll
        for (int i = 0; i < MI; ++i) {
#pragma unroll
          for (int j = 0; j < NJ; ++j)
            acc[i][j] = __builtin_amdgcn_mfma_f32_16x16x32_bf16(bf[kk][j], af[kk][i], acc[i][j], 0, 0, 0);
          const int grp = kk * MI + i;
          constexpr int NGI = NSLOT == 2 ? 1 : NG;
          if (did && grp < NGI) {
#pragma unroll
            for (int q = grp * PIECES / NGI; q < (grp + 1) * PIECES / NGI; ++q) issue_piece(q);
          }
        }
    }
    if (did) issue_advance();
    cslot = cslot == NSLOT - 1 ? 0 : cslot + 1;
    if (++ck == cc.nk) finish_tile();
  }
}

template <int BM, int BN, bool A_MC, bool B_MC, int EPI, int NSLOT_ = 0, int DW = 8>
__global__ void __launch_bounds__(512, 2) gemm_ks_kernel(const GemmGroup g, int total_tiles) {
  extern __shared__ __attribute__((aligned(16))) unsigned char smem[];
  constexpr int BK = 64, NT = DW * 64;
  using TA = TileIO<BM, A_MC, NT, BK>;
  using TB = TileIO<BN, B_MC, NT, BK>;
  constexpr int A_BYTES = BM * BK * 2, B_BYTES = BN * BK * 2;
  constexpr int STAGE = A_BYTES + B_BYTES;
  constexpr int NSLOT = NSLOT_ > 0 ? NSLOT_ : persist_slots(STAGE);
  constexpr int PIECES = TA::PIECES + TB::PIECES;
  constexpr int MI = BM / 2 / 16, NJ = BN / 2 / 16, H0 = (MI + 1) / 2, H1 = MI - H0, HT = H0 * NJ;
  static_assert(H1 >= 1, "at least two row blocks per wave");
  static_assert(8 * HT * 64 * 16 <= NSLOT * STAGE, "accumulator exchange fits in the ring");
  static_assert(!TB::WRAP, "only the A tile may have a wrapped piece list");

  const int G = gridDim.x;
  const int tile = (blockIdx.x & 7) * (G >> 3) + (blockIdx.x >> 3);
  if (tile >= total_tiles) return;
  const int tid = threadIdx.x, lane = tid & 63;
  const int wave = __builtin_amdgcn_readfirstlane(tid >> 6);
  const int wk = wave >> 2, wm = (wave >> 1) & 1, wn = wave & 1;
  int pi = 0;
#pragma unroll
  for (int i = 1; i < GGET_MAX_GROUP; ++i)
    if (i < g.count && tile >= g.p[i].tile_begin) pi = i;
  const GemmProblem& P = g.p[pi];
  int m0, n0;
  tile_origin(P, P.M, tile - P.tile_begin, BM, BN, g.super, m0, n0);
  const int nk = P.K >> 6;

  f32x4_t acc[MI][NJ];
#pragma unroll
  for (int i = 0; i < MI; ++i)
#pragma unroll
    for (int j = 0; j < NJ; ++j) acc[i][j] = f32x4_t{0.f, 0.f, 0.f, 0.f};

  const int pw = DW == 8 ? wave : (wave & (DW - 1));
  const unsigned lds0 = __builtin_amdgcn_readfirstlane((unsigned)(uintptr_t)(LDS_AS const void*)smem) + (unsigned)pw * 1024u;
  const unsigned char* kA = reinterpret_cast<const unsigned char*>(P.A);
  const unsigned char* kB = reinterpret_cast<const unsigned char*>(P.B);
  const long strideA = A_MC ? (long)BK * P.lda * 2 : (long)BK * 2;
  const long strideB = B_MC ? (long)BK * P.ldb * 2 : (long)BK * 2;
  unsigned offA[TA::PIECES], offB[TB::PIECES];
#pragma unroll
  for (int i = 0; i < TA::PIECES; ++i) offA[i] = TA::piece_off(P.lda, m0, P.M, pw, lane, i);
#pragma unroll
  for (int i = 0; i < TB::PIECES; ++i) offB[i] = TB::piece_off(P.ldb, n0, P.N, pw, lane, i);
  int islot = 0, cslot = 0, issued = 0;
  unsigned islot_off = lds0;
  int adjA[TA::PIECES];
#pragma unroll
  for (int i = 0; i < TA::PIECES; ++i) adjA[i] = (TA::piece_index(pw, i) - (pw + i * TA::NWAVES)) * 1024;
  auto issue_piece = [&](int q) {
    if (q < TA::PIECES) glds16m(kA, offA[q < TA::PIECES ? q : 0], islot_off + (unsigned)(q * TA::NWAVES * 1024 + (TA::WRAP ? adjA[q < TA::PIECES ? q : 0] : 0)));
    else glds16m(kB, offB[q >= TA::PIECES ? q - TA::PIECES : 0], islot_off + (unsigned)(A_BYTES + (q - TA::PIECES) * TB::NWAVES * 1024));
  };
  auto issue_advance = [&]() {
    islot = islot == NSLOT - 1 ? 0 : islot + 1;
    islot_off = islot == 0 ? lds0 : islot_off + (unsigned)STAGE;
    kA += strideA;
    kB += strideB;
    ++issued;
  };
  const bool dma_wave = DW == 8 || wave < DW;
#pragma unroll
  for (int i = 0; i < NSLOT - 1; ++i) {
    if (issued < nk) {
      if (dma_wave) {
#pragma unroll
        for (int q = 0; q < PIECES; ++q) issue_piece(q);
      }
      issue_advance();
    }
  }
  for (int t = 0; t < nk; ++t) {
    if (dma_wave) {
      if (issued - t == NSLOT - 1) vm_wait<(NSLOT - 2) * PIECES>();
      else vm_wait<0>();
    }
    __syncthreads();
    const bool did = issued < nk;
    const unsigned char* a_l = smem + cslot * STAGE;
    const unsigned char* b_l = a_l + A_BYTES;
    bf16x8_t af[MI], bf[NJ];
#pragma unroll
    for (int i = 0; i < MI; ++i) af[i] = TA::frag(a_l, wm * MI + i, wk, lane);
#pragma unroll
    for (int j = 0; j < NJ; ++j) bf[j] = TB::frag(b_l, wn * NJ + j, wk, lane);
#pragma unroll
    for (int i = 0; i < MI; ++i) {
#pragma unroll
      for (int j = 0; j < NJ; ++j) acc[i][j] = __builtin_amdgcn_mfma_f32_16x16x32_bf16(bf[j], af[i], acc[i][j], 0, 0, 0);
      if (did && dma_wave) {
#pragma unroll
        for (int q = i * PIECES / MI; q < (i + 1) * PIECES / MI; ++q) issue_piece(q);
      }
    }
    if (did) issue_advance();
    cslot = cslot == NSLOT - 1 ? 0 : cslot + 1;
  }
  __syncthreads();
  float4* xch = reinterpret_cast<float4*>(smem);
  const int partner = wave ^ 4;
  if (wk == 0) {
#pragma unroll
    for (int ii = 0; ii < H1; ++ii)
#pragma unroll
      for (int j = 0; j < NJ; ++j) {
        const f32x4_t v = acc[H0 + ii][j];
        xch[(size_t)(wave * HT + ii * NJ + j) * 64 + lane] = make_float4(v[0], v[1], v[2], v[3]);
      }
  } else {
#pragma unroll
    for (int ii = 0; ii < H0; ++ii)
#pragma unroll
      for (int j = 0; j < NJ; ++j) {
        const f32x4_t v = acc[ii][j];
        xch[(size_t)(wave * HT + ii * NJ + j) * 64 + lane] = make_float4(v[0], v[1], v[2], v[3]);
      }
  }
  __syncthreads();
  constexpr bool SQ = A_MC && B_MC && EPI == GGET_EPI_NONE;
  float sq = 0.f;
  auto sq_add = [&](const f32x4_t& v) {
#pragma unroll
    for (int e = 0; e < 4; ++e) { const float r = bf2f(f2bf(v[e])); sq = fmaf(r, r, sq); }
  };
  if (wk == 0) {
    f32x4_t own[H0][NJ];
#pragma unroll
    for (int ii = 0; ii < H0; ++ii)
#pragma unroll
      for (int j = 0; j < NJ; ++j) {
        const float4 o = xch[(size_t)(partner * HT + ii * NJ + j) * 64 + lane];
        const f32x4_t mine = acc[ii][j];
        own[ii][j] = f32x4_t{mine[0] + o.x, mine[1] + o.y, mine[2] + o.z, mine[3] + o.w};
        if constexpr (SQ) sq_add(own[ii][j]);
      }
    store_tile<EPI, H0, NJ>(own, P, P.M, (P.N + 3) & ~3, m0 + wm * (MI * 16), n0 + wn * (NJ * 16), lane);
  } else {
    f32x4_t own[H1][NJ];
#pragma unroll
    for (int ii = 0; ii < H1; ++ii)
#pragma unroll
      for (int j = 0; j < NJ; ++j) {
        const float4 o = xch[(size_t)(partner * HT + ii * NJ + j) * 64 + lane];
        const f32x4_t mine = acc[H0 + ii][j];
        own[ii][j] = f32x4_t{mine[0] + o.x, mine[1] + o.y, mine[2] + o.z, mine[3] + o.w};
        if constexpr (SQ) sq_add(own[ii][j]);
      }
    store_tile<EPI, H1, NJ>(own, P, P.M, (P.N + 3) & ~3, m0 + wm * (MI * 16) + H0 * 16, n0 + wn * (NJ * 16), lane);
  }
  if constexpr (SQ) {
    if (g.sq_partials) {
      float* red = reinterpret_cast<float*>(smem + NSLOT * STAGE);
      sq = wave_sum(sq);
      if (lane == 0) red[wave] = sq;
      __syncthreads();
      if (tid == 0) {
        float t = 0.f;
#pragma unroll
        for (int w = 0; w < 8; ++w) t += red[w];
        g.sq_partials[tile] = t;
      }
    }
  }
}

template <int BM, int BN, bool A_MC, bool B_MC, int EPI, int NSLOT_ = 0, int DW = 8>
int launch_ks_cfg(GemmGroup& g, int total, hipStream_t st) {
  if constexpr (DW == 8 && BM != 64) {
    if (!(menu().gemm_variant & kGemmKsplitDma8)) return launch_ks_cfg<BM, BN, A_MC, B_MC, EPI, NSLOT_, 4>(g, total, st);
  }
  constexpr int STG = (BM + BN) * 64 * 2;
  constexpr int SM = (NSLOT_ > 0 ? NSLOT_ : persist_slots(STG)) * STG + (A_MC && B_MC && EPI == GGET_EPI_NONE ? 64 : 0);
  static_assert(SM <= 160 * 1024, "LDS ring");
  const int G = (total + 7) & ~7;
  static bool attr0 = false;
  if (!attr0) {
    GGET_HIP_CHECK(hipFuncSetAttribute(reinterpret_cast<const void*>(&gemm_ks_kernel<BM, BN, A_MC, B_MC, EPI, NSLOT_, DW>),
                                       hipFuncAttributeMaxDynamicSharedMemorySize, SM));
    attr0 = true;
  }
  hipLaunchKernelGGL((gemm_ks_kernel<BM, BN, A_MC, B_MC, EPI, NSLOT_, DW>), dim3(G), dim3(512), SM, st, g, total);
  GGET_LAUNCH_CHECK();
  return 0;
}

template <int BM, int BN, int BK, int WM, int WN, bool A_MC, bool B_MC, int EPI, int NSLOT_ = 0, bool SK = false, int MODE = 0>
int launch_persist_cfg(GemmGroup& g, int total, int num_cu, hipStream_t st) {
  constexpr int STG = (BM + BN) * BK * 2;
  constexpr int SM = (NSLOT_ > 0 ? NSLOT_ : persist_slots(STG)) * STG;
  if (MODE == 2) num_cu *= 2;
  static_assert(SM <= 160 * 1024, "LDS ring");
  static_assert(!SK || (size_t)BM * BN * 4 <= kStreamKSlotBytes, "stream-K slot");
  if constexpr (MODE == 2) {
    static unsigned* cu_slots = nullptr;
    const int stagger = menu().gemm_stagger_ticks;
    if (!cu_slots && stagger > 0) {
      GGET_HIP_CHECK(hipMalloc(reinterpret_cast<void**>(&cu_slots), 2048 * sizeof(unsigned)));
      GGET_HIP_CHECK(hipMemset(cu_slots, 0, 2048 * sizeof(unsigned)));
    }
    g.cu_slots = cu_slots;
    g.stagger_ticks = cu_slots ? stagger : 0;
  }
  int G = total < num_cu && !SK ? total : num_cu;
  G = (G + 7) & ~7;
  static bool attr0 = false;
  if (!attr0) {
    GGET_HIP_CHECK(hipFuncSetAttribute(reinterpret_cast<const void*>(&gemm_persist_kernel<BM, BN, BK, WM, WN, A_MC, B_MC, EPI, NSLOT_, SK, MODE>),
                                       hipFuncAttributeMaxDynamicSharedMemorySize, SM));
    attr0 = true;
  }
  hipLaunchKernelGGL((gemm_persist_kernel<BM, BN, BK, WM, WN, A_MC, B_MC, EPI, NSLOT_, SK, MODE>), dim3(G), dim3(WM * WN * 64), SM, st, g, total);
  GGET_LAUNCH_CHECK();
  return 0;
}

thread_local void* t_streamk_ws = nullptr;
unsigned g_streamk_epoch = 0;
inline bool streamk_plan(GemmGroup& g, int tiles, int num_cu, int bk) {
  if (!menu().gemm_split_last || !t_streamk_ws || g.count != 1 || (menu().gemm_variant & kGemmNoSplitLast)) return false;
  const GemmProblem& p = g.p[0];
  if (p.m_dev || p.k_dev || num_cu > 256 || num_cu % 8 != 0) return false;
  const int nk = p.K / bk, G = num_cu;
  const int R = tiles / G, rem = tiles % G;
  if (rem == 0 || nk < 8) return false;
  int parts = 1, a = nk, last;
  if (rem <= G / 2) {
    parts = G / rem < 4 ? G / rem : 4;
    last = (nk + parts - 1) / parts;
  } else {
    const int H = G - rem, q = (rem + H - 1) / H;
    a = (nk * q + q) / (q + 1);
    if (a >= nk) return false;
    last = a > q * (nk - a) ? a : q * (nk - a);
  }
  const long plain = (long)(R + 1) * nk, split = (long)R * nk + last + 4;
  if (split > plain - plain / 16) return false;
  g.sk_rounds = R; g.sk_rem = rem; g.sk_parts = parts; g.sk_a = a;
  g.sk_flags = static_cast<unsigned*>(t_streamk_ws);
  g.sk_partial = reinterpret_cast<float*>(static_cast<unsigned char*>(t_streamk_ws) + kStreamKFlagBytes);
  g.sk_epoch = ++g_streamk_epoch ? g_streamk_epoch : ++g_streamk_epoch;
  return true;
}

template <int WM, int WN, bool A_MC, bool B_MC, int EPI>
int launch_t(GemmGroup& g, int split_k, hipStream_t st) {
  constexpr int BM = WM * 64, BN = WN * 64;
  int total = 0;
  for (int i = 0; i < g.count; ++i) {
    GemmProblem& p = g.p[i];
    const int tm = (p.M + BM - 1) / BM;
    p.tiles_n = (p.N + BN - 1) / BN;
    p.tile_begin = total;
    total += tm * p.tiles_n;
  }
  if (total == 0) return 0;
  constexpr int SMEM = kStages * (BM + BN) * 128;
  const LaunchMenu& menu = ::menu();
  const int variant = menu.gemm_variant;
  bool persist = split_k <= 1 && EPI != GGET_EPI_ATOMIC_F32 && EPI != GGET_EPI_SLAB_F32 && (!g.ablate || g.ablate >= 8) && !menu.gemm_no_persist;
  for (int i = 0; i < g.count; ++i)
    persist = persist && (g.p[i].m_dev == nullptr || (g.count == 1 && !A_MC && !menu.gemm_no_dyn)) &&
              (g.p[i].k_dev == nullptr || (g.count == 1 && g.p[i].k_pad_zero && !menu.gemm_no_dyn)) &&
              (g.p[i].K % 64) == 0 && g.p[i].K >= 64;
  if (persist) {
    const int num_cu = gget_gemm_num_cu();
    if constexpr (WM == 4 && WN == 2 && !A_MC && EPI != GGET_EPI_SLAB_F32 && EPI != GGET_EPI_ATOMIC_F32 && EPI != GGET_EPI_GEGLU_FWD) {
      long t256 = 0;
      bool ok256 = !menu.gemm_no_256;
      for (int i = 0; i < g.count; ++i) {
        t256 += (long)((g.p[i].M + 255) / 256) * ((g.p[i].N + 255) / 256);
        ok256 = ok256 && (g.p[i].N % 256) == 0;
      }
      const long r256 = (t256 + num_cu - 1) / num_cu, r_cur = (total + num_cu - 1) / num_cu;
      const bool near = 2 * t256 >= 3L * num_cu && r256 * 256 * 256 * 9 <= r_cur * BM * BN * 10;
      if (ok256 && EPI != GGET_EPI_ROPE && (t256 >= (5 * num_cu) / 2 || near)) {
        int tot2 = 0;
        for (int i = 0; i < g.count; ++i) {
          GemmProblem& p = g.p[i];
          p.tiles_n = (p.N + 255) / 256;
          p.tile_begin = tot2;
          tot2 += ((p.M + 255) / 256) * p.tiles_n;
        }
        if constexpr (!B_MC) {
          if (menu.gemm_bk64) return launch_persist_cfg<256, 256, 64, 2, 4, A_MC, B_MC, EPI, 2>(g, tot2, num_cu, st);
        }
        return launch_persist_cfg<256, 256, 32, 2, 4, A_MC, B_MC, EPI>(g, tot2, num_cu, st);
      }
    }
    if constexpr (!A_MC && (EPI == GGET_EPI_NONE || EPI == GGET_EPI_RESIDUAL || EPI == GGET_EPI_ROPE)) {
      bool ok = menu.gemm_192 != 0;
      long t192 = 0;
      for (int i = 0; i < g.count; ++i) {
        ok = ok && ((g.p[i].N % 192) == 0 || (!B_MC && EPI != GGET_EPI_ROPE && g.p[i].N > 384));
        t192 += (long)((g.p[i].M + 127) / 128) * ((g.p[i].N + 191) / 192);
      }
      const long cur_rounds = (total + num_cu - 1) / num_cu, r192 = (t192 + num_cu - 1) / num_cu;
      bool ks_first = false;
      if constexpr (EPI != GGET_EPI_ROPE) {
        if (ok && !(variant & kGemmNoKsplitNd) && cur_rounds == 1 && total * 10 >= (long)num_cu * 3 && !(variant & kGemmAreaRule)) {
          bool can = true;
          for (int i = 0; i < g.count; ++i) can = can && !g.p[i].m_dev && !g.p[i].k_dev && (g.p[i].N % 192) == 0 && g.p[i].K >= 1536;
          if (can)
            for (int cand : {64, 96, 128}) {
              long t = 0;
              for (int i = 0; i < g.count; ++i) t += (long)((g.p[i].M + cand - 1) / cand) * (g.p[i].N / 192);
              if (t <= num_cu) { ks_first = (long)cand * 192 * 10 <= (long)BM * BN * 13; break; }
            }
        }
      }
      if (ok && (r192 * 128 * 192 < cur_rounds * BM * BN || ks_first)) {
        int tot3 = 0;
        for (int i = 0; i < g.count; ++i) {
          GemmProblem& p = g.p[i];
          p.tiles_n = (p.N + 191) / 192;
          p.tile_begin = tot3;
          tot3 += ((p.M + 127) / 128) * p.tiles_n;
        }
        if constexpr (EPI != GGET_EPI_ROPE) {
          bool ks = tot3 <= num_cu && !(variant & kGemmNoKsplitNd);
          for (int i = 0; i < g.count; ++i)
            ks = ks && !g.p[i].m_dev && !g.p[i].k_dev && (g.p[i].N % 192) == 0 && g.p[i].K >= 1536;
          if (ks) {
            int bm = 128;
            if (!(variant & kGemmKsplit128Only))
              for (int cand : {64, 96}) {
                long t = 0;
                for (int i = 0; i < g.count; ++i) t += (long)((g.p[i].M + cand - 1) / cand) * (g.p[i].N / 192);
                if (t <= num_cu) { bm = cand; break; }
              }
            int tot = 0;
            for (int i = 0; i < g.count; ++i) {
              GemmProblem& p = g.p[i];
              p.tiles_n = p.N / 192;
              p.tile_begin = tot;
              tot += ((p.M + bm - 1) / bm) * p.tiles_n;
            }
            if (bm == 64) return launch_ks_cfg<64, 192, A_MC, B_MC, EPI, 3>(g, tot, st);
            if (bm == 96) return launch_ks_cfg<96, 192, A_MC, B_MC, EPI, 3>(g, tot, st);
            if (menu.gemm_lds_headroom) return launch_ks_cfg<128, 192, A_MC, B_MC, EPI, 3>(g, tot, st);
            return launch_ks_cfg<128, 192, A_MC, B_MC, EPI>(g, tot, st);
          }
        }
        if constexpr (EPI != GGET_EPI_ROPE) {
          if (streamk_plan(g, tot3, num_cu, 64)) {
            return launch_persist_cfg<128, 192, 64, 4, 2, A_MC, B_MC, EPI, 3, true>(g, tot3, num_cu, st);
          }
        }
        if (menu.gemm_lds_headroom) return launch_persist_cfg<128, 192, 64, 4, 2, A_MC, B_MC, EPI, 3>(g, tot3, num_cu, st);
        return launch_persist_cfg<128, 192, 64, 4, 2, A_MC, B_MC, EPI>(g, tot3, num_cu, st);
      }
    }
    if constexpr (A_MC && B_MC && EPI == GGET_EPI_NONE) {
      bool ok = menu.gemm_192 != 0;
      long t192 = 0;
      for (int i = 0; i < g.count; ++i) {
        ok = ok && (g.p[i].N % 192) == 0 && (g.p[i].M % 192) == 0;
        t192 += (long)(g.p[i].M / 192) * (g.p[i].N / 192);
      }
      const long cur_rounds = (total + num_cu - 1) / num_cu, r192 = (t192 + num_cu - 1) / num_cu;
      if (ok && r192 * 192 * 192 < cur_rounds * BM * BN) {
        int tot4 = 0;
        for (int i = 0; i < g.count; ++i) {
          GemmProblem& p = g.p[i];
          p.tiles_n = p.N / 192;
          p.tile_begin = tot4;
          tot4 += (p.M / 192) * p.tiles_n;
        }
        if (tot4 <= num_cu && !(variant & kGemmNoKsplitWgrad)) {
          bool ks = true;
          for (int i = 0; i < g.count; ++i) ks = ks && !g.p[i].m_dev && !g.p[i].k_dev;
          if (ks) {
            g.sq_written = g.sq_partials != nullptr;
            return launch_ks_cfg<192, 192, true, true, EPI>(g, tot4, st);
          }
        }
        return launch_persist_cfg<192, 192, 64, 4, 2, true, true, EPI>(g, tot4, num_cu, st);
      }
    }
    if constexpr (WM == 4 && WN == 2 && !A_MC && (EPI == GGET_EPI_GEGLU_BWD || EPI == GGET_EPI_NONE || EPI == GGET_EPI_RESIDUAL)) {
      bool ok = !(variant & kGemmNo192Rows);
      long t192 = 0;
      for (int i = 0; i < g.count; ++i) {
        ok = ok && !g.p[i].m_dev && !g.p[i].k_dev && (g.p[i].N % BN) == 0;
        t192 += (long)((g.p[i].M + 191) / 192) * (g.p[i].N / BN);
      }
      const long cur_rounds = (total + num_cu - 1) / num_cu, r192 = (t192 + num_cu - 1) / num_cu;
      if (ok && r192 * 192 * 100 < cur_rounds * 256 * 92) {
        int tot5 = 0;
        for (int i = 0; i < g.count; ++i) {
          GemmProblem& p = g.p[i];
          p.tiles_n = p.N / BN;
          p.tile_begin = tot5;
          tot5 += ((p.M + 191) / 192) * p.tiles_n;
        }
        if constexpr (EPI == GGET_EPI_GEGLU_BWD && BN == 128) {
          if (!(variant & kGemmOneBlockPerCu) && menu.gemm_lds_headroom < 2) return launch_persist_cfg<192, BN, 64, WM, WN, A_MC, B_MC, EPI, 2, false, 2>(g, tot5, num_cu, st);
        }
        if (menu.gemm_lds_headroom) return launch_persist_cfg<192, BN, 64, WM, WN, A_MC, B_MC, EPI, 3>(g, tot5, num_cu, st);
        return launch_persist_cfg<192, BN, 64, WM, WN, A_MC, B_MC, EPI>(g, tot5, num_cu, st);
      }
    }
    return launch_persist_cfg<BM, BN, 64, WM, WN, A_MC, B_MC, EPI>(g, total, num_cu, st);
  }
  static bool attr_done = false;
  if (!attr_done) {
    GGET_HIP_CHECK(hipFuncSetAttribute(reinterpret_cast<const void*>(&gemm_kernel<WM, WN, A_MC, B_MC, EPI>),
                                       hipFuncAttributeMaxDynamicSharedMemorySize, SMEM));
    attr_done = true;
  }
  dim3 grid(total, split_k > 0 ? split_k : 1, 1);
  hipLaunchKernelGGL((gemm_kernel<WM, WN, A_MC, B_MC, EPI>), grid, dim3(WM * WN * 64), SMEM, st, g);
  GGET_LAUNCH_CHECK();
  return 0;
}

template <bool A_MC, bool B_MC, int EPI>
int launch_shape(GemmGroup& g, int split_k, hipStream_t st) {
  long tiles_big = 0;
  for (int i = 0; i < g.count; ++i) tiles_big += (long)((g.p[i].M + 255) / 256) * ((g.p[i].N + 127) / 128);
  tiles_big *= (split_k > 1 ? split_k : 1);
  if (tiles_big >= 160) return launch_t<4, 2, A_MC, B_MC, EPI>(g, split_k, st);
  return launch_t<2, 2, A_MC, B_MC, EPI>(g, split_k, st);
}

template <bool A_MC, bool B_MC>
int launch_mode(GemmGroup& g, int epi, int split_k, hipStream_t st) {
  switch (epi) {
    case GGET_EPI_NONE: return launch_shape<A_MC, B_MC, GGET_EPI_NONE>(g, split_k, st);
    case GGET_EPI_RESIDUAL: return launch_shape<A_MC, B_MC, GGET_EPI_RESIDUAL>(g, split_k, st);
    case GGET_EPI_ATOMIC_F32: return launch_shape<A_MC, B_MC, GGET_EPI_ATOMIC_F32>(g, split_k, st);
    case GGET_EPI_SLAB_F32: return launch_shape<A_MC, B_MC, GGET_EPI_SLAB_F32>(g, split_k, st);
    case GGET_EPI_ROPE:
      if constexpr (!A_MC && !B_MC) return launch_shape<false, false, GGET_EPI_ROPE>(g, split_k, st);
      break;
    case GGET_EPI_GEGLU_BWD:
      if constexpr (!A_MC && B_MC) return launch_shape<false, true, GGET_EPI_GEGLU_BWD>(g, split_k, st);
      break;
    case GGET_EPI_GEGLU_FWD:
      if constexpr (!A_MC && !B_MC) {
        int total = 0;
        for (int i = 0; i < g.count; ++i) {
          GemmProblem& p = g.p[i];
          p.tiles_n = p.N / 256;
          p.tile_begin = total;
          total += ((p.M + 255) / 256) * p.tiles_n;
        }
        if (total == 0) return 0;
        const int num_cu = gget_gemm_num_cu();
        long t192 = 0;
        for (int i = 0; i < g.count; ++i) t192 += (long)((g.p[i].M + 191) / 192) * (g.p[i].N / 256);
        if (!(menu().gemm_variant & kGemmNo192Rows) && ((t192 + num_cu - 1) / num_cu) * 192 * 100 < ((total + num_cu - 1) / num_cu) * 256 * 92) {
          int tot2 = 0;
          for (int i = 0; i < g.count; ++i) {
            GemmProblem& p = g.p[i];
            p.tile_begin = tot2;
            tot2 += ((p.M + 191) / 192) * p.tiles_n;
          }
          return launch_persist_cfg<192, 256, 64, 4, 2, false, false, GGET_EPI_GEGLU_FWD, 2>(g, tot2, num_cu, st);
        }
        return launch_persist_cfg<256, 256, 64, 4, 2, false, false, GGET_EPI_GEGLU_FWD, 2>(g, total, num_cu, st);
      }
      break;
  }
  gget_set_error("gemm: unknown epilogue %d", epi);
  return 2;
}

}

void gget_gemm_streamk_workspace(void* ws) { t_streamk_ws = ws; }

struct GemmProbeRec { hipEvent_t e0, e1; double flops; bool dyn; };
static std::deque<GemmProbeRec> g_probe;
static bool g_probe_on = false;

int gget_gemm_launch(int mode, int epi, GemmGroup& g, int split_k, hipStream_t st) {
  GGET_REQUIRE(g.count >= 1 && g.count <= GGET_MAX_GROUP, "gemm: bad group size %d", g.count);
  g.sk_partial = nullptr; g.sk_flags = nullptr; g.sk_epoch = 0;
  g.sk_rounds = g.sk_rem = g.sk_a = 0; g.sk_parts = 1;
  g.cu_slots = nullptr; g.stagger_ticks = 0;
  g.sq_written = 0;
  const LaunchMenu& m = menu();
  g.ablate = m.gemm_ablate > 0 ? m.gemm_ablate : 0;
  g.super = m.gemm_super > 0 ? m.gemm_super : (mode == GGET_GEMM_TN ? 1 : kSuper);
  GGET_REQUIRE(split_k <= 1 || epi == GGET_EPI_ATOMIC_F32 || epi == GGET_EPI_SLAB_F32,
               "gemm: split-K needs the fp32 atomic or slab epilogue");
  for (int i = 0; i < g.count; ++i) {
    const GemmProblem& p = g.p[i];
    GGET_REQUIRE(p.c_rows == nullptr || (epi == GGET_EPI_NONE && split_k <= 1), "gemm: the fused row scatter needs the plain bf16 epilogue");
    if (epi == GGET_EPI_GEGLU_FWD || epi == GGET_EPI_GEGLU_BWD) {
      const bool fwd = epi == GGET_EPI_GEGLU_FWD;
      GGET_REQUIRE(mode == (fwd ? GGET_GEMM_NT : GGET_GEMM_NN) && split_k <= 1 && !p.m_dev && !p.k_dev, "gemm: GEGLU epilogue: wrong mode");
      GGET_REQUIRE(p.ff > 0 && p.N == (fwd ? 2 * p.ff : p.ff) && p.N % (fwd ? 256 : 64) == 0 && (p.K % 64) == 0,
                   "gemm: GEGLU epilogue needs ff %% %d == 0 and K %% 64 == 0 (ff %d N %d K %d)", fwd ? 128 : 64, p.ff, p.N, p.K);
      GGET_REQUIRE((p.ldc % 64) == 0 && ((uintptr_t)p.C & 127) == 0 && p.ldc >= 2 * p.ff, "gemm: GEGLU epilogue: gu / dgu must be [M][>= 2 ff], 128-byte aligned rows");
      if (fwd) GGET_REQUIRE(p.C2 && (p.ldc2 % 64) == 0 && ((uintptr_t)p.C2 & 127) == 0 && p.ldc2 >= p.ff, "gemm: GEGLU forward: h must be [M][>= ff], 128-byte aligned rows");
      else GGET_REQUIRE(p.G && (p.ldg % 8) == 0 && ((uintptr_t)p.G & 15) == 0 && p.ldg >= 2 * p.ff, "gemm: GEGLU backward: gu must be [M][>= 2 ff]");
    }
    GGET_REQUIRE((p.lda % 8) == 0 && (p.ldb % 8) == 0 && (p.ldc % 8) == 0,
                 "gemm: leading dims must be multiples of 8 (lda %d ldb %d ldc %d)", p.lda, p.ldb, p.ldc);
    GGET_REQUIRE((p.N % 4) == 0 || (mode == GGET_GEMM_NT && p.ldc >= ((p.N + 3) & ~3) && epi != GGET_EPI_RESIDUAL),
                 "gemm: N = %d must be a multiple of 4 (or NT mode with ldc >= N rounded up to 4)", p.N);
    GGET_REQUIRE(((size_t)p.M + 64) * (size_t)p.lda * 2 < (1ull << 32) && ((size_t)p.N + 64) * (size_t)p.ldb * 2 < (1ull << 32),
                 "gemm: operand spans more than 4 GiB (M %d lda %d N %d ldb %d)", p.M, p.lda, p.N, p.ldb);
  }
  GemmProbeRec* rec = nullptr;
  if (g_probe_on) {
    double fl = 0;
    bool dyn = false;
    for (int i = 0; i < g.count; ++i) {
      fl += 2.0 * g.p[i].M * g.p[i].N * g.p[i].K;
      dyn = dyn || g.p[i].m_dev || g.p[i].k_dev;
    }
    g_probe.emplace_back();
    rec = &g_probe.back();
    rec->flops = fl;
    rec->dyn = dyn;
    GGET_HIP_CHECK(hipEventCreate(&rec->e0));
    GGET_HIP_CHECK(hipEventCreate(&rec->e1));
    GGET_HIP_CHECK(hipEventRecord(rec->e0, st));
  }
  int rc = 2;
  if (g.count == 1 && (g.p[0].b_tile_off || g.p[0].a_rows)) {
    GemmProblem& p = g.p[0];
    GGET_REQUIRE((mode == GGET_GEMM_NT || mode == GGET_GEMM_NN) && epi == GGET_EPI_NONE && split_k <= 1 && p.m_dev && !p.k_dev &&
                 (p.N % 192) == 0 && (p.K % 64) == 0 && p.K >= 64,
                 "gemm: a_rows / b_tile_off need a single NT / NN problem with the plain epilogue, a device-side row count, N %% 192 == 0 and K %% 64 == 0");
    static int ncu = 0;
    if (!ncu) {
      int dev = 0;
      hipDeviceProp_t prop;
      GGET_HIP_CHECK(hipGetDevice(&dev));
      GGET_HIP_CHECK(hipGetDeviceProperties(&prop, dev));
      ncu = prop.multiProcessorCount > 0 ? prop.multiProcessorCount : 256;
    }
    const bool big = p.b_tile_rows == 256 && (p.N % 256) == 0;
    p.tiles_n = big ? p.N / 256 : p.N / 192;
    p.tile_begin = 0;
    const int total = big ? ((p.M + 255) / 256) * p.tiles_n : ((p.M + 127) / 128) * p.tiles_n;
    if (total <= 0) rc = 0;
    else if (big && mode == GGET_GEMM_NT) rc = launch_persist_cfg<256, 256, 64, 2, 4, false, false, GGET_EPI_NONE, 2>(g, total, ncu, st);
    else if (big) rc = launch_persist_cfg<256, 256, 32, 2, 4, false, true, GGET_EPI_NONE>(g, total, ncu, st);
    else if (mode == GGET_GEMM_NT) rc = launch_persist_cfg<128, 192, 64, 4, 2, false, false, GGET_EPI_NONE, 3>(g, total, ncu, st);
    else rc = launch_persist_cfg<128, 192, 64, 4, 2, false, true, GGET_EPI_NONE, 3>(g, total, ncu, st);
    if (rec) GGET_HIP_CHECK(hipEventRecord(rec->e1, st));
    return rc;
  }
  switch (mode) {
    case GGET_GEMM_NT: rc = launch_mode<false, false>(g, epi, split_k, st); break;
    case GGET_GEMM_NN: rc = launch_mode<false, true>(g, epi, split_k, st); break;
    case GGET_GEMM_TN: rc = launch_mode<true, true>(g, epi, split_k, st); break;
    default: gget_set_error("gemm: unknown mode %d", mode);
  }
  if (rec) GGET_HIP_CHECK(hipEventRecord(rec->e1, st));
  return rc;
}

extern "C" int gget_debug_gemm_probe(int enable, double* flops_out, double* ms_out, int* launches_out, int* skipped_out) {
  if (enable) {
    for (auto& r : g_probe) { (void)hipEventDestroy(r.e0); (void)hipEventDestroy(r.e1); }
    g_probe.clear();
    g_probe_on = true;
    return 0;
  }
  g_probe_on = false;
  double fl = 0, ms = 0;
  int n = 0, skipped = 0;
  for (auto& r : g_probe) {
    GGET_HIP_CHECK(hipEventSynchronize(r.e1));
    float t = 0.f;
    GGET_HIP_CHECK(hipEventElapsedTime(&t, r.e0, r.e1));
    if (r.dyn) { ++skipped; }
    else { fl += r.flops; ms += t; ++n; }
    (void)hipEventDestroy(r.e0);
    (void)hipEventDestroy(r.e1);
  }
  g_probe.clear();
  if (flops_out) *flops_out = fl;
  if (ms_out) *ms_out = ms;
  if (launches_out) *launches_out = n;
  if (skipped_out) *skipped_out = skipped;
  return 0;
}

int gget_gemm_single(int mode, int epi, const void* A, const void* B, void* C, const void* R, int M, int N, int K,
                     int lda, int ldb, int ldc, const int* m_dev, const int* k_dev, int split_k, hipStream_t st, bool k_pad_zero,
                     const int* c_rows) {
  GemmGroup g;
  memset(&g, 0, sizeof(g));
  g.count = 1;
  GemmProblem& p = g.p[0];
  p.A = static_cast<const bf16_t*>(A);
  p.B = static_cast<const bf16_t*>(B);
  p.C = C;
  p.R = static_cast<const bf16_t*>(R);
  p.M = M; p.N = N; p.K = K;
  p.lda = lda; p.ldb = ldb; p.ldc = ldc;
  p.m_dev = m_dev; p.k_dev = k_dev;
  p.k_pad_zero = k_pad_zero ? 1 : 0;
  p.slab_stride = (long)M * ldc;
  p.c_rows = c_rows;
  return gget_gemm_launch(mode, epi, g, split_k, st);
}
```

graph-gpt_amd/csrc/kernels.hip:

```cpp
#include "common.h"
#include "kernels.h"

static float* g_det_scratch = nullptr;
static size_t g_det_bytes = 0;

namespace {

constexpr int kBlock = 256;

__device__ __forceinline__ uint4 ldg16(const bf16_t* p) { return *reinterpret_cast<const uint4*>(p); }
__device__ __forceinline__ void stg16(bf16_t* p, const uint4& v) {
  typedef unsigned u4nt __attribute__((ext_vector_type(4)));
  __builtin_nontemporal_store(u4nt{v.x, v.y, v.z, v.w}, reinterpret_cast<u4nt*>(p));
}

__global__ void __launch_bounds__(128) embed_fwd_kernel(const int64_t* __restrict__ ids, const bf16_t* __restrict__ emb,
                                                        const bf16_t* __restrict__ gate, bf16_t* __restrict__ out,
                                                        int T, int F, int ldF, int d, ElemDropArg E) {
  const int t = blockIdx.x;
  const int64_t* row = ids + (size_t)t * ldF;
  for (int c = threadIdx.x; c * 8 < d; c += blockDim.x) {
    float acc[8] = {0, 0, 0, 0, 0, 0, 0, 0};
    for (int f0 = 0; f0 < F; f0 += 4) {
      uint4 r[4], gr[4];
#pragma unroll
      for (int u = 0; u < 4; ++u) {
        const int fu = min(f0 + u, F - 1);
        r[u] = ldg16(emb + (size_t)row[fu] * d + c * 8);
        if (gate) gr[u] = ldg16(gate + (size_t)fu * d + c * 8);
      }
#pragma unroll
      for (int u = 0; u < 4; ++u) {
        const int f = f0 + u;
        if (f >= F) break;
        float v[8];
        unpack8(r[u], v);
        if (E.thresh) {
#pragma unroll
          for (int e = 0; e < 8; ++e)
            v[e] = bf2f(f2bf(v[e] * elem_drop_mul(E, GGET_DROP_STREAM_EMBED, elem_row(E, t) * (unsigned)F + (unsigned)f, (unsigned)(c * 8 + e))));
        }
        if (gate) {
          float gv[8];
          unpack8(gr[u], gv);
#pragma unroll
          for (int e = 0; e < 8; ++e) acc[e] += v[e] * gv[e];
        } else {
#pragma unroll
          for (int e = 0; e < 8; ++e) acc[e] += v[e];
        }
      }
    }
    stg16(out + (size_t)t * d + c * 8, pack8(acc));
  }
}

__global__ void __launch_bounds__(128) embed_long_ratio_kernel(const int64_t* __restrict__ ids, bf16_t* __restrict__ x, int F,
                                                               int ldF, int d) {
  const int t = blockIdx.x;
  const int64_t* row = ids + (size_t)t * ldF;
  int nnz = 0;
  for (int f = 0; f < F; ++f) nnz += row[f] != 0;
  const float ratio = fminf(bf2f(f2bf(1.0f / ((float)nnz + 1e-7f))), 1.0f);
  if (ratio == 1.0f) return;
  for (int c = threadIdx.x; c * 8 < d; c += blockDim.x) {
    float v[8];
    unpack8(ldg16(x + (size_t)t * d + c * 8), v);
#pragma unroll
    for (int e = 0; e < 8; ++e) v[e] *= ratio;
    stg16(x + (size_t)t * d + c * 8, pack8(v));
  }
}

__global__ void __launch_bounds__(kBlock) sample_mask_wgt_kernel(const int64_t* __restrict__ labels, float* __restrict__ w,
                                                                 int cells) {
  __shared__ int part[kBlock / GGET_WAVE];
  const int64_t* row = labels + (size_t)blockIdx.x * cells;
  int n = 0;
  for (int i = threadIdx.x; i < cells; i += kBlock) n += row[i] != -100;
  n = (int)wave_sum((float)n);
  if ((threadIdx.x & 63) == 0) part[threadIdx.x >> 6] = n;
  __syncthreads();
  if (threadIdx.x == 0) {
    int tot = 0;
    for (int i = 0; i < kBlock / GGET_WAVE; ++i) tot += part[i];
    w[blockIdx.x] = 1.0f / ((float)tot + 1e-7f);
  }
}

__global__ void __launch_bounds__(128) raw_blend_kernel(const float* __restrict__ raw, const int64_t* __restrict__ labels, int n,
                                                        int first_only, const bf16_t* __restrict__ tok, bf16_t* __restrict__ out,
                                                        int32_t* __restrict__ flag, int e, const int32_t* __restrict__ rows_map, int n_logical) {
  const int t = blockIdx.x;
  const int lt = rows_map ? rows_map[t] : t;
  if (lt >= n_logical) {
    if (threadIdx.x == 0) flag[t] = 0;
    for (int j = threadIdx.x; j < e; j += blockDim.x) out[(size_t)t * e + j] = 0;
    return;
  }
  bool masked = false;
  if (labels) {
    const int64_t* lr = labels + (size_t)lt * n;
    int unset = 0;
    for (int f = 0; f < (first_only ? 1 : n); ++f) unset += lr[f] == -100;
    masked = unset == 0;
  }
  if (threadIdx.x == 0) flag[t] = masked ? 1 : 0;
  for (int j = threadIdx.x; j < e; j += blockDim.x) out[(size_t)t * e + j] = masked ? tok[j] : f2bf(raw[(size_t)lt * e + j]);
}
__global__ void __launch_bounds__(kBlock) raw_tok_grad_kernel(const bf16_t* __restrict__ dx, const int32_t* __restrict__ flag,
                                                              float* __restrict__ dtok, int T, int e) {
  const int t0 = blockIdx.x * 256, t1 = min(T, t0 + 256);
  for (int j = threadIdx.x; j < e; j += kBlock) {
    float s = 0.f;
    for (int t = t0; t < t1; ++t)
      if (flag[t]) s += bf2f(dx[(size_t)t * e + j]);
    if (s != 0.f) unsafeAtomicAdd(dtok + j, s);
  }
}

constexpr int kEmbLdsV = 8192;
constexpr int kEmbCells = 4096;
template <bool LDS_PATH>
__global__ void __launch_bounds__(256) embed_hist_kernel(const int64_t* __restrict__ ids, int32_t* __restrict__ hist,
                                                         long ncell, int F, int ldF, int pad_id, int V, int hot_id) {
  extern __shared__ int lh[];
  const long c0 = (long)blockIdx.x * kEmbCells;
  if (LDS_PATH) {
    for (int v = threadIdx.x; v < V; v += 256) lh[v] = 0;
    __syncthreads();
  }
  for (int i = threadIdx.x; i < kEmbCells; i += 256) {
    const long c = c0 + i;
    const bool in = c < ncell;
    const int id = in ? (int)ids[(c / F) * ldF + (c % F)] : pad_id;
    if (LDS_PATH) {
      if (id != pad_id) atomicAdd(lh + id, 1);
    } else {
      const unsigned long long hot = __ballot(id == hot_id && id != pad_id);
      if (id == hot_id) {
        if ((threadIdx.x & 63) == __builtin_ctzll(hot)) atomicAdd(hist + id, (int)__builtin_popcountll(hot));
      } else if (id != pad_id) {
        atomicAdd(hist + id, 1);
      }
    }
  }
  if (LDS_PATH) {
    __syncthreads();
    for (int v = threadIdx.x; v < V; v += 256)
      if (lh[v]) atomicAdd(hist + v, lh[v]);
  }
}
__global__ void __launch_bounds__(1024) embed_scan_kernel(const int32_t* __restrict__ hist, int32_t* __restrict__ offs,
                                                          int32_t* __restrict__ cursor, int V) {
// ... 84 lines not shown
    int cur = id_sorted[beg];
    auto flush = [&](int id, const float (&a)[8]) {
      float* dst = demb + (size_t)id * d + c * 8;
      if (offs[id] >= beg && offs[id + 1] <= end) {
        float4 lo = *reinterpret_cast<const float4*>(dst), up = *reinterpret_cast<const float4*>(dst + 4);
        lo.x += a[0]; lo.y += a[1]; lo.z += a[2]; lo.w += a[3];
        up.x += a[4]; up.y += a[5]; up.z += a[6]; up.w += a[7];
        *reinterpret_cast<float4*>(dst) = lo;
        *reinterpret_cast<float4*>(dst + 4) = up;
      } else {
#pragma unroll
        for (int e = 0; e < 8; ++e) unsafeAtomicAdd(dst + e, a[e]);
      }
    };
    for (int j0 = beg; j0 < end; j0 += 8) {
      int idv[8], cellv[8];
      uint4 raw[8];
#pragma unroll
      for (int u = 0; u < 8; ++u) {
        const int j = min(j0 + u, end - 1);
        idv[u] = id_sorted[j];
        cellv[u] = cell_sorted[j];
      }
#pragma unroll
      for (int u = 0; u < 8; ++u) raw[u] = ldg16(dx + (size_t)(cellv[u] / F) * d + c * 8);
#pragma unroll
      for (int u = 0; u < 8; ++u) {
        if (j0 + u >= end) break;
        if (idv[u] != cur) {
          flush(cur, acc);
#pragma unroll
          for (int e = 0; e < 8; ++e) acc[e] = 0.f;
          cur = idv[u];
        }
        float g[8];
        unpack8(raw[u], g);
        if (E.thresh) {
#pragma unroll
          for (int e = 0; e < 8; ++e) g[e] *= elem_drop_mul(E, GGET_DROP_STREAM_EMBED, elem_row(E, cellv[u] / F) * (unsigned)F + (unsigned)(cellv[u] % F), (unsigned)(c * 8 + e));
        }
        if (gate) {
          float gv[8];
          unpack8(ldg16(gate + (size_t)(cellv[u] % F) * d + c * 8), gv);
#pragma unroll
          for (int e = 0; e < 8; ++e) acc[e] += g[e] * gv[e];
        } else {
#pragma unroll
          for (int e = 0; e < 8; ++e) acc[e] += g[e];
        }
      }
    }
    flush(cur, acc);
  }
}
__global__ void __launch_bounds__(kBlock) embed_count_kernel(const int64_t* __restrict__ ids, bf16_t* __restrict__ cnt, int T,
                                                             int F, int ldF, int ldc, int pad_id) {
  const long cell = (long)blockIdx.x * kBlock + threadIdx.x;
  if (cell >= (long)T * F) return;
  const int t = (int)(cell / F), f = (int)(cell - (long)t * F);
  const int64_t* row = ids + (size_t)t * ldF;
  const int id = (int)row[f];
  if (id == pad_id) return;
  int c = 0;
  for (int g = 0; g < F; ++g) c += (int)row[g] == id ? 1 : 0;
  cnt[(size_t)t * ldc + id] = f2bf((float)c);
}

constexpr int kEmbTok = 64;
__global__ void __launch_bounds__(128) embed_dgate_kernel(const int64_t* __restrict__ ids, const bf16_t* __restrict__ dx,
                                                          const bf16_t* __restrict__ emb, float* __restrict__ dgate, int T,
                                                          int F, int ldF, int d, ElemDropArg E) {
  const int t0 = blockIdx.x * kEmbTok;
  const int f = blockIdx.y;
  for (int c = threadIdx.x; c * 8 < d; c += blockDim.x) {
    float acc[8] = {0, 0, 0, 0, 0, 0, 0, 0};
    for (int tt = 0; tt < kEmbTok && t0 + tt < T; ++tt) {
      const int t = t0 + tt;
      float g[8], ev[8];
      unpack8(ldg16(dx + (size_t)t * d + c * 8), g);
      unpack8(ldg16(emb + (size_t)ids[(size_t)t * ldF + f] * d + c * 8), ev);
      if (E.thresh) {
#pragma unroll
        for (int e = 0; e < 8; ++e)
          ev[e] = bf2f(f2bf(ev[e] * elem_drop_mul(E, GGET_DROP_STREAM_EMBED, elem_row(E, t) * (unsigned)F + (unsigned)f, (unsigned)(c * 8 + e))));
      }
#pragma unroll
      for (int e = 0; e < 8; ++e) acc[e] += g[e] * ev[e];
    }
#pragma unroll
    for (int e = 0; e < 8; ++e) unsafeAtomicAdd(dgate + (size_t)f * d + c * 8 + e, acc[e]);
  }
}

constexpr int kMaxChunksPerLane = 4;
template <int NCH>
__global__ void __launch_bounds__(kBlock) rmsnorm_fwd_kernel(const bf16_t* __restrict__ x, const bf16_t* __restrict__ w,
                                                             bf16_t* __restrict__ y, float* __restrict__ rstd_out,
                                                             int T, int d, float eps) {
  const int lane = threadIdx.x & 63;
  const int nchunk = d >> 3;
  const int stride = gridDim.x * (kBlock / 64);
  int row = blockIdx.x * (kBlock / 64) + (threadIdx.x >> 6);
  uint4 cur[NCH], nxt[NCH];
  float wv[NCH][8];
#pragma unroll
  for (int i = 0; i < NCH; ++i) {
    const int c = lane + i * 64;
    cur[i] = make_uint4(0, 0, 0, 0);
    if (c < nchunk) {
      unpack8(ldg16(w + c * 8), wv[i]);
      if (row < T) cur[i] = ldg16(x + (size_t)row * d + c * 8);
    }
  }
  for (; row < T; row += stride) {
    const int nrow = row + stride;
#pragma unroll
    for (int i = 0; i < NCH; ++i) {
      const int c = lane + i * 64;
      nxt[i] = (c < nchunk && nrow < T) ? ldg16(x + (size_t)nrow * d + c * 8) : make_uint4(0, 0, 0, 0);
    }
    float v[NCH][8];
    float ss = 0.f;
#pragma unroll
    for (int i = 0; i < NCH; ++i) {
      unpack8(cur[i], v[i]);
#pragma unroll
      for (int e = 0; e < 8; ++e) ss += v[i][e] * v[i][e];
    }
    ss = wave_sum(ss);
    const float rstd = rsqrtf(ss / (float)d + eps);
    if (lane == 0 && rstd_out) rstd_out[row] = rstd;
#pragma unroll
    for (int i = 0; i < NCH; ++i) {
      const int c = lane + i * 64;
      if (c < nchunk) {
        float o[8];
#pragma unroll
        for (int e = 0; e < 8; ++e) o[e] = wv[i][e] * bf2f(f2bf(v[i][e] * rstd));
        stg16(y + (size_t)row * d + c * 8, pack8(o));
      }
    }
#pragma unroll
    for (int i = 0; i < NCH; ++i) cur[i] = nxt[i];
  }
}

template <int NCH>
__global__ void __launch_bounds__(kBlock) rmsnorm_bwd_kernel(const bf16_t* __restrict__ dy, const bf16_t* __restrict__ x,
                                                             const bf16_t* __restrict__ w, const float* __restrict__ rstd_in,
                                                             const bf16_t* __restrict__ dres, bf16_t* __restrict__ dx,
                                                             float* __restrict__ dw_accum, int T, int d, int copies,
                                                             uint64_t copy_stride, float* __restrict__ dw_part) {
  extern __shared__ float dw_lds[];
  const int lane = threadIdx.x & 63, wave = threadIdx.x >> 6;
  const int nchunk = d >> 3;
  float dwp[NCH][8];
  float wv[NCH][8];
#pragma unroll
  for (int i = 0; i < NCH; ++i) {
    const int c = lane + i * 64;
#pragma unroll
    for (int e = 0; e < 8; ++e) dwp[i][e] = 0.f;
    if (c < nchunk) unpack8(ldg16(w + c * 8), wv[i]);
  }
  const int stride = gridDim.x * (kBlock / 64);
  int row = blockIdx.x * (kBlock / 64) + wave;
  uint4 xr[NCH], dr[NCH], rr[NCH];
  float rstd = 0.f;
  auto fetch = [&](int r) {
    rstd = rstd_in[r];
#pragma unroll
    for (int i = 0; i < NCH; ++i) {
      const int c = lane + i * 64;
      if (c < nchunk) {
        xr[i] = ldg16(x + (size_t)r * d + c * 8);
        dr[i] = ldg16(dy + (size_t)r * d + c * 8);
        rr[i] = dres ? ldg16(dres + (size_t)r * d + c * 8) : make_uint4(0, 0, 0, 0);
      }
    }
  };
  if (row < T) fetch(row);
  for (; row < T; row += stride) {
    const float rs = rstd;
    float xh[NCH][8], g[NCH][8], res[NCH][8];
    float dot = 0.f;
#pragma unroll
    for (int i = 0; i < NCH; ++i) {
      const int c = lane + i * 64;
      if (c < nchunk) {
        float xv[8], dv[8];
        unpack8(xr[i], xv);
        unpack8(dr[i], dv);
        unpack8(rr[i], res[i]);
#pragma unroll
        for (int e = 0; e < 8; ++e) {
          xh[i][e] = xv[e] * rs;
          g[i][e] = dv[e] * wv[i][e];
          dot += g[i][e] * xh[i][e];
          dwp[i][e] += dv[e] * xh[i][e];
        }
      }
    }
    if (row + stride < T) fetch(row + stride);
    dot = wave_sum(dot) / (float)d;
#pragma unroll
    for (int i = 0; i < NCH; ++i) {
      const int c = lane + i * 64;
      if (c < nchunk) {
        float o[8];
#pragma unroll
        for (int e = 0; e < 8; ++e) o[e] = res[i][e] + rs * (g[i][e] - xh[i][e] * dot);
        stg16(dx + (size_t)row * d + c * 8, pack8(o));
      }
    }
  }
#pragma unroll
  for (int i = 0; i < NCH; ++i) {
    const int c = lane + i * 64;
    if (c < nchunk) {
      *reinterpret_cast<float4*>(dw_lds + wave * d + c * 4) = make_float4(dwp[i][0], dwp[i][1], dwp[i][2], dwp[i][3]);
      *reinterpret_cast<float4*>(dw_lds + wave * d + (d >> 1) + c * 4) = make_float4(dwp[i][4], dwp[i][5], dwp[i][6], dwp[i][7]);
    }
  }
  __syncthreads();
  for (int t = threadIdx.x; t < d; t += kBlock) {
    const int hd = d >> 1, pl = t >= hd ? 1 : 0, ix = t - pl * hd;
    const int j = (ix >> 2) * 8 + pl * 4 + (ix & 3);
    const float s = dw_lds[t] + dw_lds[d + t] + dw_lds[2 * d + t] + dw_lds[3 * d + t];
    if (dw_part) dw_part[(size_t)blockIdx.x * d + j] = s;
    else unsafeAtomicAdd(dw_accum + (size_t)(blockIdx.x % copies) * copy_stride + j, s);
  }
}

template <int NCH>
__global__ void __launch_bounds__(kBlock) rmsnorm_dw_kernel(const bf16_t* __restrict__ dy, const bf16_t* __restrict__ x,
                                                            const float* __restrict__ rstd_in, float* __restrict__ dw_accum, int T, int d,
                                                            int copies, uint64_t copy_stride, float* __restrict__ dw_part) {
  extern __shared__ float dw_lds[];
  const int lane = threadIdx.x & 63, wave = threadIdx.x >> 6;
  const int nchunk = d >> 3;
  float dwp[NCH][8];
#pragma unroll
  for (int i = 0; i < NCH; ++i)
#pragma unroll
    for (int e = 0; e < 8; ++e) dwp[i][e] = 0.f;
  const int stride = gridDim.x * (kBlock / 64);
  int row = blockIdx.x * (kBlock / 64) + wave;
  uint4 xr[NCH], dr[NCH];
  float rstd = 0.f;
  auto fetch = [&](int r) {
    rstd = rstd_in[r];
#pragma unroll
    for (int i = 0; i < NCH; ++i) {
      const int c = lane + i * 64;
      if (c < nchunk) {
        xr[i] = ldg16(x + (size_t)r * d + c * 8);
        dr[i] = ldg16(dy + (size_t)r * d + c * 8);
      }
    }
  };
  if (row < T) fetch(row);
  for (; row < T; row += stride) {
    const float rs = rstd;
    float xv[NCH][8], dv[NCH][8];
#pragma unroll
    for (int i = 0; i < NCH; ++i) {
      unpack8(xr[i], xv[i]);
      unpack8(dr[i], dv[i]);
    }
    if (row + stride < T) fetch(row + stride);
#pragma unroll
    for (int i = 0; i < NCH; ++i) {
      const int c = lane + i * 64;
      if (c < nchunk) {
#pragma unroll
        for (int e = 0; e < 8; ++e) dwp[i][e] += dv[i][e] * (xv[i][e] * rs);
      }
    }
  }
#pragma unroll
  for (int i = 0; i < NCH; ++i) {
    const int c = lane + i * 64;
    if (c < nchunk) {
      *reinterpret_cast<float4*>(dw_lds + wave * d + c * 4) = make_float4(dwp[i][0], dwp[i][1], dwp[i][2], dwp[i][3]);
      *reinterpret_cast<float4*>(dw_lds + wave * d + (d >> 1) + c * 4) = make_float4(dwp[i][4], dwp[i][5], dwp[i][6], dwp[i][7]);
    }
  }
  __syncthreads();
  for (int t = threadIdx.x; t < d; t += kBlock) {
    const int hd = d >> 1, pl = t >= hd ? 1 : 0, ix = t - pl * hd;
    const int j = (ix >> 2) * 8 + pl * 4 + (ix & 3);
    const float s = dw_lds[t] + dw_lds[d + t] + dw_lds[2 * d + t] + dw_lds[3 * d + t];
    if (dw_part) dw_part[(size_t)blockIdx.x * d + j] = s;
    else unsafeAtomicAdd(dw_accum + (size_t)(blockIdx.x % copies) * copy_stride + j, s);
  }
}

template <int NCH, int NW>
__global__ void __launch_bounds__(NW * 64) rmsnorm_bwd_wide_kernel(const bf16_t* __restrict__ dy, const bf16_t* __restrict__ x,
                                                                  const bf16_t* __restrict__ w, const float* __restrict__ rstd_in,
                                                                  const bf16_t* __restrict__ dres, bf16_t* __restrict__ dx,
                                                                  float* __restrict__ dw_accum, int T, int d, int copies,
                                                                  uint64_t copy_stride, float* __restrict__ dw_part) {
  extern __shared__ float dw_lds[];
  const int lane = threadIdx.x & 63, wave = threadIdx.x >> 6;
  const int nchunk = d >> 3;
  float dwp[NCH][8];
  uint4 wp[NCH];
#pragma unroll
  for (int i = 0; i < NCH; ++i) {
    const int c = lane + i * 64;
#pragma unroll
    for (int e = 0; e < 8; ++e) dwp[i][e] = 0.f;
    wp[i] = c < nchunk ? ldg16(w + c * 8) : make_uint4(0, 0, 0, 0);
  }
  struct RowRegs { uint4 x[NCH], d[NCH], r[NCH]; float rs; };
  RowRegs ra, rb;
  const unsigned lo = lane * 8;
  auto fetch = [&](int r0, RowRegs& q) {
    const int r = __builtin_amdgcn_readfirstlane(r0);
    const size_t rbase = (size_t)r * d;
    const bf16_t *xrow = x + rbase, *dyrow = dy + rbase, *rrow = dres ? dres + rbase : nullptr;
    q.rs = rstd_in[r];
#pragma unroll
    for (int i = 0; i < NCH; ++i) {
      const int c = lane + i * 64;
      if (c < nchunk) {
        q.x[i] = ldg16(xrow + lo + i * 512);
        q.d[i] = ldg16(dyrow + lo + i * 512);
        q.r[i] = rrow ? ldg16(rrow + lo + i * 512) : make_uint4(0, 0, 0, 0);
      }
    }
  };
  auto keep4 = [](uint4& v) { asm volatile("" : "+v"(v.x), "+v"(v.y), "+v"(v.z), "+v"(v.w)); };
  auto work = [&](int row0, RowRegs& q) {
    const int row = __builtin_amdgcn_readfirstlane(row0);
    const float rs = q.rs;
    float dot = 0.f;
#pragma unroll
    for (int i = 0; i < NCH; ++i) {
      const int c = lane + i * 64;
      if (c < nchunk) {
        float xv[8], dv[8], wv[8];
        keep4(wp[i]);
        unpack8(q.x[i], xv);
        unpack8(q.d[i], dv);
        unpack8(wp[i], wv);
#pragma unroll
        for (int e = 0; e < 8; ++e) {
          const float xh = xv[e] * rs;
          const float g = dv[e] * wv[e];
          dot += g * xh;
          dwp[i][e] += dv[e] * xh;
        }
      }
    }
    dot = wave_sum(dot) / (float)d;
    bf16_t* dxrow = dx + (size_t)row * d;
#pragma unroll
    for (int i = 0; i < NCH; ++i) {
      const int c = lane + i * 64;
      if (c < nchunk) {
        float xv[8], dv[8], wv[8], res[8], o[8];
        keep4(q.x[i]);
        keep4(q.d[i]);
        keep4(wp[i]);
        unpack8(q.x[i], xv);
        unpack8(q.d[i], dv);
        unpack8(wp[i], wv);
        unpack8(q.r[i], res);
#pragma unroll
        for (int e = 0; e < 8; ++e) {
          const float xh = xv[e] * rs;
          float g = dv[e] * wv[e];
          asm volatile("" : "+v"(g));
          o[e] = res[e] + rs * (g - xh * dot);
        }
        stg16(dxrow + lo + i * 512, pack8(o));
      }
    }
  };
  int row = (int)((long)blockIdx.x * T / gridDim.x) + wave;
  const int r_end = (int)((long)(blockIdx.x + 1) * T / gridDim.x);
  if (row < r_end) fetch(row, ra);
// ... 2638 lines not shown
```

graph-gpt_amd/csrc/menu.h:

```cpp
#pragma once

struct LaunchMenu {
  int gemm_variant;
  int gemm_lds_headroom;
  int gemm_split_last;
  int gemm_stagger_ticks;
  int gemm_ablate;
  int gemm_cu_reserve;
  int gemm_num_cu;
  int gemm_no_persist;
  int gemm_no_dyn;
  int gemm_no_256;
  int gemm_bk64;
  int gemm_192;
  int gemm_super;
  int attn_by_sample;
  int attn_big;
  int attn_dense;
  int attn_small;
  int attn_fused;
  int attn_fused_min_s;
  int attn_stg128;
  int attn_oproj;
  int attn_oproj_off;
  int head_sorted;
  int head_dense;
  int head_tile;
  int no_head_scatter_fusion;
  int no_geglu_fusion;
  int no_ls_norm_fusion;
  int ls_norm_bwd_wide;
  int no_varlen;
  int count_copy;
  int embed_sorted;
  int occupy_fat;
  int deterministic;
  int rms_wide;
  int rms_rows;
  int ce_parts;
  int ce_generic;
  int link_grid;
};

enum : int {
  kGemmNoKsplitNd = 1,
  kGemmNoKsplitWgrad = 2,
  kGemmNo192Rows = 4,
  kGemmNoSplitLast = 8,
  kGemmKsplit128Only = 16,
  kGemmOneBlockPerCu = 32,
  kGemmKsplitDma8 = 128,
  kGemmAreaRule = 512,
};

struct MenuRow {
  int LaunchMenu::*field;
  int key;
  const char* env;
  bool env_presence;
  int def;
  const char* meaning;
};

inline constexpr MenuRow kMenuRows[] = {
    {&LaunchMenu::gemm_variant, 1, "GGET_GEMM_VARIANT", false, 0, "bit mask of GEMM kernel variants (kGemm*)"},
    {&LaunchMenu::gemm_lds_headroom, 2, "GGET_GEMM_LDS_HEADROOM", false, 1, "LDS headroom of the 128x192 / 192x128 tiles: 0 4-slot rings, 1 3-slot, 2 also one block per CU"},
    {&LaunchMenu::gemm_split_last, 3, "GGET_GEMM_SPLIT_LAST", false, 0, "1: split the K range of the last, partial round's tiles among the idle blocks"},
    {&LaunchMenu::deterministic, 4, "GGET_DETERMINISTIC", false, 0, "1: reproducible mode, RMSNorm weight gradients summed in block order"},
    {&LaunchMenu::gemm_stagger_ticks, 5, "GGET_GEMM_STAGGER", false, 0, "MODE 2 GEMM launches: start delay of a CU's second workgroup (100 MHz ticks)"},
    {&LaunchMenu::gemm_ablate, 7, "GGET_GEMM_ABLATE", false, 0, "GEMM diagnostics: 1 no LDS-DMA, 2 no MFMA, 4 no C store, 32 no epilogue (timing only)"},
    {&LaunchMenu::head_dense, 8, nullptr, false, 0, "1: SMTP head as a dense projection through all slots"},
    {&LaunchMenu::head_tile, 9, nullptr, false, 0, "SMTP head slot tile rows: 0 automatic, 128 / 256 forced"},
    {&LaunchMenu::attn_oproj_off, 10, nullptr, false, 0, "1: S <= 32 attention, o projection, RMSNorm as three launches"},
    {&LaunchMenu::ls_norm_bwd_wide, 11, "GGET_LS_NORM_BWD_WIDE", false, 0, "1: fused RMSNorm + LayerScale backward in its 16-byte-chunk form for every width"},
    {&LaunchMenu::rms_wide, 13, "GGET_RMS_WIDE", false, 1, "0: short RMSNorm backward launches in 4-wave blocks instead of one 16-wave block per CU"},
    {&LaunchMenu::ce_parts, 14, "GGET_CE_PARTS", false, 1, "0: cross-entropy adds its loss with one atomic per block instead of per-block partial sums"},
    {&LaunchMenu::gemm_cu_reserve, 15, nullptr, false, 0, "CUs every GEMM plan leaves free for a collective's workgroups"},
    {&LaunchMenu::occupy_fat, 16, nullptr, false, 0, "1: gget_debug_occupy's stand-in takes RCCL's register footprint"},
    {&LaunchMenu::link_grid, 18, nullptr, false, 0, "> 0: most workgroups a streaming launch of the link metrics takes (0: 1024)"},
    {&LaunchMenu::gemm_num_cu, 0, "GGET_GEMM_NUM_CU", false, 0, "> 0: GEMM plans pretend the chip has this many CUs"},
    {&LaunchMenu::gemm_no_persist, 0, "GGET_GEMM_NO_PERSIST", true, 0, "set: no persistent GEMM kernels"},
    {&LaunchMenu::gemm_no_dyn, 0, "GGET_GEMM_NO_DYN", true, 0, "set: no persistent GEMM kernels for device-sized launches"},
    {&LaunchMenu::gemm_no_256, 0, "GGET_GEMM_NO_256", true, 0, "set: no 256x256 GEMM tiles"},
    {&LaunchMenu::gemm_bk64, 0, "GGET_GEMM_BK64", false, 1, "0: 256x256 NT tiles with 32-deep instead of 64-deep K-tiles"},
    {&LaunchMenu::gemm_192, 0, "GGET_GEMM_192", false, 1, "0: no 128x192 / 192x192 GEMM tiles"},
    {&LaunchMenu::gemm_super, 0, "GGET_GEMM_SUPER", false, 0, "> 0: tile-order supergroup size of every GEMM launch"},
    {&LaunchMenu::attn_by_sample, 0, "GGET_ATTN_BY_SAMPLE", false, 1, "0: var-len 32 < S <= 64 attention keyed by S instead of every sample's own rows"},
    {&LaunchMenu::attn_big, 0, "GGET_ATTN_BIG", false, 1, "0: S >= 256 attention on the register-prefetch kernels"},
    {&LaunchMenu::attn_dense, 0, "GGET_ATTN_DENSE", false, 1, "0: no dense attention forward for S >= 512"},
    {&LaunchMenu::attn_small, 0, "GGET_ATTN_SMALL", false, 1, "0: no per-sample attention backward for S <= 64"},
    {&LaunchMenu::attn_fused, 0, "GGET_ATTN_FUSED", false, 1, "0: long-sequence attention backward as two kernels instead of one pass"},
    {&LaunchMenu::attn_fused_min_s, 0, "GGET_ATTN_FUSED_MIN_S", false, 256, "sequence length from which the one-pass attention backward runs"},
    {&LaunchMenu::attn_stg128, 0, "GGET_ATTN_STG128", false, 1, "0: S >= 512 dK / dV kernel with 64-row instead of 128-row stages"},
    {&LaunchMenu::attn_oproj, 0, "GGET_ATTN_OPROJ", false, 1, "0: S <= 32 attention, o projection, RMSNorm as three launches"},
    {&LaunchMenu::head_sorted, 0, "GGET_HEAD_SORTED", false, 1, "0: SMTP head as a dense projection through all slots"},
    {&LaunchMenu::no_head_scatter_fusion, 0, "GGET_NO_HEAD_SCATTER_FUSION", true, 0, "set: SMTP head rows scattered by their own launch (implies the dense head)"},
    {&LaunchMenu::no_geglu_fusion, 0, "GGET_NO_GEGLU_FUSION", true, 0, "set: GEGLU as GEMM + element-wise kernel"},
    {&LaunchMenu::no_ls_norm_fusion, 0, "GGET_NO_LS_NORM_FUSION", true, 0, "set: LayerScale residual and the next RMSNorm as separate launches"},
    {&LaunchMenu::no_varlen, 0, "GGET_NO_VARLEN", true, 0, "set: the padded token grid instead of the var-len layout"},
    {&LaunchMenu::count_copy, 0, "GGET_COUNT_COPY", false, 0, "1: token count back by device-to-host copy + event instead of a polled host word"},
    {&LaunchMenu::embed_sorted, 0, "GGET_EMBED_SORTED", true, 0, "set: embedding backward always as the sorted scatter-add"},
    {&LaunchMenu::rms_rows, 0, "GGET_RMS_ROWS", false, 4, "RMSNorm backward rows per wave"},
    {&LaunchMenu::ce_generic, 0, "GGET_CE_GENERIC", true, 0, "set: cross-entropy never on the vectorised row kernels"},
};

extern LaunchMenu g_menu;
extern thread_local const LaunchMenu* t_call_menu;
inline const LaunchMenu& menu() { return t_call_menu ? *t_call_menu : g_menu; }
```

include/gget.h:

```cpp
#ifndef GGET_H_
#define GGET_H_

#include <stddef.h>
#include <stdint.h>

#ifdef __cplusplus
extern "C" {
#endif

#define GGET_KIND_PRETRAIN 0
#define GGET_KIND_TASK 1

#define GGET_PROBLEM_SINGLE_LABEL 0
#define GGET_PROBLEM_REGRESSION_L1 1
#define GGET_PROBLEM_REGRESSION_MSE 2
#define GGET_PROBLEM_TOKEN_CE 5
#define GGET_PROBLEM_TOKEN_CE_INTRA 6
#define GGET_PROBLEM_AUC 4
#define GGET_PROBLEM_MULTI_LABEL 3

typedef struct gget_config_t {
  int32_t kind;
  int32_t vocab_size;
  int32_t hidden_size;
// ... 23 lines not shown
typedef struct gget_sizes_t {
  uint64_t n_params;
  uint64_t param_bf16_bytes;
  uint64_t master_bytes;
  uint64_t adam_bytes;
  uint64_t grad_bf16_bytes;
  uint64_t workspace_bytes;
} gget_sizes_t;

typedef struct gget_buffers_t {
  void* param_bf16_dev;
  void* master_dev;
  void* adam_m_dev;
  void* adam_v_dev;
  void* grad_bf16_dev;
  void* workspace_dev;
  const float* rope_cos_dev;
  const float* rope_sin_dev;
} gget_buffers_t;

typedef struct gget_param_info_t {
  char name[96];
  int32_t ndim;
  int64_t shape[2];
  uint64_t offset;
  int32_t layer;
} gget_param_info_t;

typedef struct gget_engine* gget_handle_t;

const char* gget_last_error(void);
int gget_version(void);

int gget_query_sizes(const gget_config_t* cfg, gget_sizes_t* out);
int gget_create(const gget_config_t* cfg, const gget_buffers_t* bufs, gget_handle_t* out);
int gget_destroy(gget_handle_t h);

int gget_param_count(gget_handle_t h);
int gget_param_info(gget_handle_t h, int index, gget_param_info_t* out);
int gget_bucket_count(gget_handle_t h);
int gget_bucket_range(gget_handle_t h, int bucket, uint64_t* offset, uint64_t* count);

int gget_set_dropout(gget_handle_t h, float attention_p, float path_p, uint32_t seed);

#define GGET_TOKENS_AUTO (-2)
int gget_set_token_count(gget_handle_t h, int64_t n_real_tokens);
int gget_position_status(gget_handle_t h, int32_t* clamped_out, void* stream);
int gget_varlen_status(gget_handle_t h, int32_t out[3], void* stream);
int gget_deferred_status(gget_handle_t h, int32_t out[2], void* stream);

int gget_set_dropout_ex(gget_handle_t h, float embed_p, float mlp_p, float head_p);

int gget_set_raw_embeds(gget_handle_t h, const float* raw_embeds_dev, int first_label_only);

int gget_set_rope_range(gget_handle_t h, float rope_range);

int gget_set_stack_method(gget_handle_t h, int stack_long);

int gget_set_focal_gamma(gget_handle_t h, float gamma);

int gget_set_auc(gget_handle_t h, int num_neg, uint32_t seed);

int gget_set_cls_idx(gget_handle_t h, const int64_t* cls_idx_dev);

int gget_sync_params(gget_handle_t h, void* stream);

int gget_forward_pretrain(gget_handle_t h, const int64_t* input_ids_dev, const int64_t* attention_mask_dev,
                          const int64_t* labels_dev, const float* sample_wgt_dev, const int64_t* position_ids_dev,
                          int B, int S, float* loss_dev, void* stream);

int gget_forward_pretrain_packed(gget_handle_t h, const int64_t* input_ids_dev, const int64_t* attention_mask3d_dev,
                                 const int64_t* labels_dev, const float* sample_wgt_dev, const int64_t* position_ids_dev,
                                 int B, int S, float* loss_dev, void* stream);
int gget_forward_task(gget_handle_t h, const int64_t* input_ids_dev, const int64_t* attention_mask_dev,
                      const int64_t* position_ids_dev, const void* task_labels_dev, const float* sample_wgt_dev,
                      int problem_type, int B, int S, float* loss_dev, float* task_logits_dev,
                      void* task_hidden_dev, void* stream);

int gget_backward(gget_handle_t h, float loss_scale, void* stream);
int gget_backward_begin(gget_handle_t h, float loss_scale, void* stream);
int gget_backward_layer(gget_handle_t h, int layer, void* stream);
int gget_backward_end(gget_handle_t h, void* stream);

#define GGET_OPT_NORM_FROM_BACKWARD 1
#define GGET_OPT_SKIP_NONFINITE_STEP 2
int gget_set_option(gget_handle_t h, int option, int value);
int gget_set_dp_menu(gget_handle_t h, int reserve_cus, int lds_headroom);

#define GGET_UNIQUE_ID_BYTES 128
int gget_comm_unique_id(void* out_bytes );
int gget_comm_init(gget_handle_t h, int rank, int world, const void* unique_id_bytes);
int gget_comm_destroy(gget_handle_t h);
int gget_comm_move(gget_handle_t dst, gget_handle_t src);
int gget_allreduce_grads_async(gget_handle_t h, int bucket, int fp32_accumulate, void* side_stream);
int gget_allreduce_range_async(gget_handle_t h, uint64_t offset, uint64_t count, int fp32_accumulate, void* side_stream);
int gget_comm_init_loopback(gget_handle_t h, int world);

int gget_adamw_step(gget_handle_t h, float lr, float beta1, float beta2, float eps, float weight_decay,
                    float max_grad_norm, float grad_scale, int step, float* gnorm_dev, void* stream);

int gget_grad_acc_attach(gget_handle_t h, float* acc_dev);
int gget_grad_accumulate(gget_handle_t h, void* stream);
int gget_grad_acc_count(gget_handle_t h, int32_t* out);
int gget_grad_acc_set_count(gget_handle_t h, int32_t n);

int gget_set_frozen(gget_handle_t h, int frozen_layers);
int gget_trainable_ranges(gget_handle_t h, uint64_t out[4], int32_t* n_out);
int gget_bucket_train_range(gget_handle_t h, int bucket, uint64_t* offset, uint64_t* count);

int gget_ema_attach(gget_handle_t h, float* ema_dev);
int gget_set_ema_decay(gget_handle_t h, float decay);
int gget_ema_update(gget_handle_t h, float decay, void* stream);
int gget_ema_to_params(gget_handle_t h, void* stream);

#define GGET_SHARD_CHUNK 4096
#define GGET_SHARD_PARAMS 0
#define GGET_SHARD_MASTER 1
#define GGET_SHARD_ADAM_M 2
#define GGET_SHARD_ADAM_V 3
#define GGET_SHARD_SLOTS 4
#define GGET_SHARD_EMA 5
int gget_shard_plan(const gget_config_t* cfg, int world, int bucket, uint64_t out[5]);
int gget_shard_init(gget_handle_t h, int world, int rank, int32_t* slots_per_rank);
int gget_shard_bucket(gget_handle_t h, int bucket, uint64_t out[5]);
int gget_reduce_scatter_grads_async(gget_handle_t h, int bucket, int fp32_accumulate, void* side_stream);
int gget_shard_sqnorm_partials(gget_handle_t h, float* slots_dev, void* stream);
int gget_shard_allgather_async(gget_handle_t h, int what, float* slots_dev, void* stream);
int gget_adamw_step_sharded(gget_handle_t h, float lr, float beta1, float beta2, float eps, float weight_decay, float max_grad_norm,
                            float grad_scale, int step, const float* slots_dev, float* gnorm_dev, void* stream);

int gget_head_counts(gget_handle_t h, int32_t counts[2], void* stream);
int gget_head_logits(gget_handle_t h, const void** logits_dev, int32_t* ld);
int gget_hidden_states(gget_handle_t h, const void** hidden_dev);
int gget_layer_hidden_states(gget_handle_t h, int layer, const void** hidden_dev);
int gget_hidden_states_grid(gget_handle_t h, int layer, void* out_dev, void* stream);

#define GGET_GEMM_NT 0
#define GGET_GEMM_NN 1
#define GGET_GEMM_TN 2
#define GGET_EPI_NONE 0
#define GGET_EPI_RESIDUAL 1
#define GGET_EPI_ATOMIC_F32 2
#define GGET_EPI_ROPE 4
#define GGET_EPI_SLAB_F32 3
#define GGET_EPI_GEGLU_FWD 5
#define GGET_EPI_GEGLU_BWD 6
int gget_op_gemm(int mode, int epilogue, const void* A, const void* B, void* C, const void* R, int M, int N, int K,
                 int lda, int ldb, int ldc, int split_k, void* stream);
int gget_op_gemm_streamk(int mode, int epilogue, const void* A, const void* B, void* C, const void* R, int M, int N, int K,
                         int lda, int ldb, int ldc, void* streamk_ws, void* stream);
uint64_t gget_op_gemm_streamk_bytes(void);
int gget_op_gemm_grouped(int mode, int count, const void* const* A, const void* const* B, void* const* C, const int* M,
                         const int* N, const int* K, const int* lda, const int* ldb, const int* ldc, void* stream);
int gget_debug_set(int key, int value);
int gget_debug_get(int key, int* value);
int gget_debug_probe(gget_handle_t h, int enable, float* avg_ms_out);
int gget_debug_gemm_probe(int enable, double* flops_out, double* ms_out, int* launches_out, int* skipped_out);
int gget_debug_occupy(void* scratch, uint64_t scratch_bytes, int blocks, int lds_bytes, int microseconds, void* stream);
int gget_op_qkv_rope(const void* x, const void* wqkv, void* qkv, const float* cos_tab, const float* sin_tab,
                     const int64_t* position_ids, int T, int S, int d, void* stream);
int gget_op_smtp2d(const int64_t* ids_in, int ld_in, const int64_t* node_idx, int ld_node, int64_t* ids_out, int64_t* labels_out,
                   int B, int S, int F, float smtp_2d_rate, float power, float replace_rate, int vocab, int global_2d_mask,
                   uint32_t seed, void* stream);
#define GGET_CONF_MAXPROB 0
#define GGET_CONF_MARGIN 1
#define GGET_CONF_NEG_ENTROPY 2
int gget_op_token_confidence(const void* logits, int ld, int R, int V, int mode, float* conf, int64_t* tok, void* stream);
int gget_op_token_sample(const void* logits, int ld, int R, int V, int mode, float temperature, float top_p, int top_k,
                         float alg_temp, uint32_t seed, float* conf, int64_t* tok, void* stream);
int gget_op_unmask_origin(int64_t* x, const int64_t* cand, int B, int N, float p_transfer, uint32_t seed, int mask_token_id,
                          void* stream);
int gget_op_smtp_rows(const int64_t* ids_in, const int32_t* lengths, int64_t* ids_out, int64_t* labels_out, float* wgt_out, int B,
                      int S, int F, double umr_min, double umr_max, double power, uint32_t seed, void* stream);
int gget_op_rmsnorm_fwd(const void* x, const void* w, void* y, float* rstd, int T, int d, float eps, void* stream);
int gget_op_rmsnorm_bwd(const void* dy, const void* x, const void* w, const float* rstd, const void* dres,
                        void* dx, float* dw_accum, int T, int d, void* stream);
int gget_op_embed_fwd(const int64_t* ids, const void* emb, const void* gate, void* out, int T, int F, int ldF,
                      int d, void* stream);
int gget_op_embed_bwd(const int64_t* ids, const void* dx, const void* emb, const void* gate, float* demb_accum,
                      float* dgate_accum, int T, int F, int ldF, int d, int V, int pad_id, void* stream);
int gget_op_rope(void* qkv, const float* cos_tab, const float* sin_tab, const int64_t* position_ids, int B, int S,
                 int H, int inverse, void* stream);
int gget_op_attn_fwd(const void* qkv, const int32_t* key_len, void* out, float* lse, int B, int S, int H,
                     int causal, const float* cos_tab, const float* sin_tab, const int64_t* position_ids,
                     float dropout_p, uint32_t dropout_seed, void* stream);
int gget_op_attn_bwd(const void* qkv, const void* out, const void* dout, const float* lse, const int32_t* key_len,
                     void* dqkv, float* delta_ws, int B, int S, int H, int causal, const float* cos_tab,
                     const float* sin_tab, const int64_t* position_ids, float dropout_p, uint32_t dropout_seed,
                     void* stream);
int gget_op_copy_from_host(const void* src_pinned_host, void* dst_dev, uint64_t bytes, void* stream);
int gget_op_attn_fwd_varlen(const void* qkv, const int32_t* key_len, const int32_t* row_base, void* out, float* lse, int B, int S, int H,
                            int causal, const float* cos_tab, const float* sin_tab, const int64_t* position_ids, int qk_rotated,
                            float dropout_p, uint32_t dropout_seed, void* stream);
int gget_op_attn_bwd_varlen(const void* qkv, const void* out, const void* dout, const float* lse, const int32_t* key_len,
                            const int32_t* row_base, void* dqkv, float* delta_ws, int B, int S, int H, int causal, const float* cos_tab,
                            const float* sin_tab, const int64_t* position_ids, int qk_rotated, float dropout_p, uint32_t dropout_seed,
                            void* stream);
int gget_op_attn_oproj_fwd(const void* qkv, const int32_t* key_len, const int32_t* row_base, void* attn_out, float* lse, const void* wo_packed,
                           const void* x_in, void* x_mid, const void* norm_w, void* xn, float* rstd, int B, int S, int H, int causal,
                           float eps, float dropout_p, uint32_t dropout_seed, void* stream, int32_t* taken);
int gget_op_pack_wo(const void* w, uint64_t layer_stride, void* fwd, void* bwd, int d, int layers, void* stream);
int gget_op_attn_oproj_bwd(const void* dxn, const void* x_mid, const void* norm_w, const float* rstd, const void* dres, void* dx_mid,
                           float* dw_accum, int copies, uint64_t copy_stride, const void* wot_packed, const void* qkv, const float* lse,
                           const int32_t* key_len, const int32_t* row_base, void* dqkv, int B, int S, int H, int causal, const float* cos_tab,
                           const float* sin_tab, const int64_t* position_ids, float dropout_p, uint32_t dropout_seed, int t_rows,
                           void* stream, int32_t* taken, void* dattn_long);
int gget_op_attn_fwd_ranges(const void* qkv, const int32_t* key_lo, const int32_t* key_hi, void* out, float* lse, int B, int S,
                            int H, int causal, float dropout_p, uint32_t dropout_seed, void* stream);
int gget_op_attn_bwd_ranges(const void* qkv, const void* out, const void* dout, const float* lse, const int32_t* key_lo,
                            const int32_t* key_hi, void* dqkv, float* delta_ws, int B, int S, int H, int causal,
                            float dropout_p, uint32_t dropout_seed, void* stream);
int gget_op_ranges_from_mask3d(const int64_t* mask3d, int32_t* key_lo, int32_t* key_hi, int B, int S, void* stream);
int gget_op_attn_bwd_fused(const void* qkv, const void* out, const void* dout, const float* lse, const int32_t* key_len,
                           const int32_t* key_lo, const int32_t* key_hi, void* dqkv, float* delta_ws, void* dq_ws, int B, int S,
                           int H, int causal, float dropout_p, uint32_t dropout_seed, void* stream);
int gget_op_gateup_geglu(const void* x, const void* wgu, void* gu, void* h, int T, int d, int ff, void* stream);
int gget_op_down_dgrad_geglu(const void* dy, const void* wdown, const void* gu, void* dgu, void* dh_scratch, int T, int d, int ff,
                             void* stream);
int gget_op_geglu_fwd(const void* gu, void* h, int T, int ff, void* stream);
int gget_op_geglu_bwd(const void* gu, const void* dh, void* dgu, int T, int ff, void* stream);
int gget_op_ce_fwd_bwd(const void* logits, int ld, const int32_t* labels, const float* row_wgt, const int32_t* n_rows_dev,
                       int n_rows_cap, int V, float* loss_sum, void* dlogits, float grad_scale_base, int mean_over_rows,
                       void* stream);

int gget_op_score_fwd(const void* hidden, const int32_t* pool_row, const void* w, const void* bias, float* logits, void* pooled_h,
                      int B, int C, int d, void* stream);
int gget_op_score_bwd(const float* dlogits, const void* hidden, const int32_t* pool_row, const void* w, float* dw, float* dbias,
                      void* dhidden, int B, int C, int d, void* stream);
int gget_op_tok_score_fwd(const void* hidden, const void* w, const void* bias, float* logits, int T, int C, int d, void* stream);
int gget_op_tok_ce(const float* logits, const int64_t* labels, float* dl, float* stat, float* loss_out, int T, int C,
                   const int32_t* rows_map, int n_logical, void* stream);
int gget_op_tok_score_bwd(const float* dl, const float* stat, const void* hidden, const void* w, float* dw, float* dbias, void* dhidden,
                          int T, int C, int d, void* stream);
int gget_op_tok_intra_fwd(const void* hidden, const int32_t* row_start, const int64_t* cls_idx, float* logits, int B, int C, int d,
                          void* stream);
int gget_op_tok_intra_bwd(const float* dl, const float* stat, const void* hidden, const int32_t* row_start, const int64_t* cls_idx,
                          void* dhidden, int B, int C, int d, void* stream);
int gget_op_task_loss(const float* logits, const void* labels, const float* sample_wgt, int problem, int B, int C, float* loss_out,
                      float* dlogits, void* stream);
int gget_op_auc_loss(const float* logits, const int64_t* labels, int B, int C, int num_neg, uint32_t seed, float* loss_out,
                     float* dlogits, int32_t* lists, void* stream);
int gget_op_pool_rows(const void* hidden, const int32_t* pool_row, void* out, int B, int d, void* stream);
int gget_op_scatter_rows_f32(const float* src, const int32_t* pool_row, void* dhidden, int B, int d, void* stream);
int gget_op_head_linear_fwd(const void* x, void* a, const void* w, const void* bias, void* y, float* y32, int B, int Din, int Dout,
                            int layer, void* stream);
int gget_op_head_linear_bwd(const float* dy, const void* x, const void* a, const void* w, float* dw, float* dbias, float* dx, int B,
                            int Din, int Dout, int layer, void* stream);

size_t gget_op_rank_metrics_workspace(int n, int C);
int gget_op_rank_metrics(const float* scores, int ld_s, const float* labels, int ld_y, int n, int C, int64_t* n_pos, int64_t* n_neg,
                         uint64_t* auc2, double* ap_sum, int32_t* n_bad, void* workspace, size_t workspace_bytes, void* stream);

size_t gget_op_link_hits_workspace(int n);
int gget_op_link_hits(const float* scores, const int64_t* labels, int n, int64_t K, int64_t* n_pos, int64_t* n_neg, float* kth, int64_t* hits,
                      int32_t* n_bad, void* workspace, size_t workspace_bytes, void* stream);
size_t gget_op_link_mrr_workspace(int n);
int gget_op_link_mrr(const float* scores, const int64_t* labels, const int64_t* idx, int n, int cnt_neg, int groups, int64_t* n_pos,
                     int64_t* n_neg, int32_t* optimistic, int32_t* pessimistic, int64_t* hits_1_3_10, double* mrr_sum, int32_t* n_bad,
                     void* workspace, size_t workspace_bytes, void* stream);

#ifdef __cplusplus
}
#endif
#endif
```

Baseline: 782,300 graph-tokens/s.

## Run input RMSNorm backward as side blocks inside grouped weight-gradient GEMM launch

```diff
diff --git a/graph-gpt_amd/_lib.py b/graph-gpt_amd/_lib.py
--- a/graph-gpt_amd/_lib.py
+++ b/graph-gpt_amd/_lib.py
@@ -88,6 +88,9 @@
     "gget_debug_get": (i32, [i32, C.POINTER(i32)]),
     "gget_debug_occupy": (i32, [vp, u64, i32, i32, i32, vp]),
     "gget_op_gemm_grouped": (i32, [i32, i32, vp, vp, vp, vp, vp, vp, vp, vp, vp, vp]),
+    "gget_op_wgrad_norm_bwd": (i32, [vp, vp, vp, vp, vp, i32, vp, vp, vp, vp, vp, vp, vp, i32, i32, u64, vp, i32, C.POINTER(i32), vp]),
+    "gget_debug_side_launches": (i32, [C.POINTER(i64)]),
+    "gget_debug_norm1_operands": (i32, [vp, i32, C.POINTER(vp), C.POINTER(vp), C.POINTER(vp), C.POINTER(i32)]),
     "gget_op_rmsnorm_fwd": (i32, [vp, vp, vp, vp, i32, i32, f32, vp]),
     "gget_op_rmsnorm_bwd": (i32, [vp, vp, vp, vp, vp, vp, vp, i32, i32, vp]),
     "gget_op_embed_fwd": (i32, [vp, vp, vp, vp, i32, i32, i32, i32, vp]),
@@ -164,8 +167,8 @@
 
 KEY_GEMM_VARIANT, KEY_GEMM_LDS_HEADROOM, KEY_GEMM_SPLIT_LAST, KEY_DETERMINISTIC, KEY_GEMM_STAGGER = 1, 2, 3, 4, 5
 KEY_GEMM_ABLATE, KEY_HEAD_DENSE, KEY_HEAD_TILE, KEY_ATTN_OPROJ_OFF, KEY_LS_NORM_BWD_WIDE = 7, 8, 9, 10, 11
-KEY_RMS_WIDE, KEY_CE_PARTS, KEY_GEMM_CU_RESERVE, KEY_OCCUPY_FAT, KEY_LINK_GRID = 13, 14, 15, 16, 18
-MENU_KEYS = (1, 2, 3, 4, 5, 7, 8, 9, 10, 11, 13, 14, 15, 16, 18)
+KEY_RMS_WIDE, KEY_CE_PARTS, KEY_GEMM_CU_RESERVE, KEY_OCCUPY_FAT, KEY_LINK_GRID, KEY_WGRAD_SIDE_NORM = 13, 14, 15, 16, 18, 19
+MENU_KEYS = (1, 2, 3, 4, 5, 7, 8, 9, 10, 11, 13, 14, 15, 16, 18, 19)
 GEMM_NO_KSPLIT_ND, GEMM_NO_KSPLIT_WGRAD, GEMM_NO_192_ROWS, GEMM_NO_SPLIT_LAST, GEMM_KSPLIT_128_ONLY, GEMM_ONE_BLOCK_PER_CU = 1, 2, 4, 8, 16, 32
 GEMM_KSPLIT_DMA8, GEMM_AREA_RULE = 128, 512
 
@@ -194,6 +197,24 @@
     ptr = lambda k: PA(*[p[k].data_ptr() for p in problems])
     num = lambda k: IA(*[int(p[k]) for p in problems])
     return lib.gget_op_gemm_grouped(mode, n, ptr(0), ptr(1), ptr(2), num(3), num(4), num(5), num(6), num(7), num(8), stream)
+
+
+def side_launches() -> int:
+    v = i64()
+    check(load().gget_debug_side_launches(C.byref(v)))
+    return int(v.value)
+
+
+def wgrad_norm_bwd(lib, problems, norm, stream, sq_tiles=None, separate=False, copies=1, copy_stride=0):
+    PA, IA = vp * 4, i32 * 4
+    ptr = lambda k: PA(*[p[k].data_ptr() for p in problems])
+    T, d = norm[0].shape
+    taken = i32(0)
+    np_ = [vp(t.data_ptr()) if t is not None else None for t in norm]
+    check(lib.gget_op_wgrad_norm_bwd(ptr(0), ptr(1), ptr(2), IA(*[p[0].shape[1] for p in problems]), IA(*[p[1].shape[1] for p in problems]), T,
+                                     *np_, d, copies, copy_stride, vp(sq_tiles.data_ptr()) if sq_tiles is not None else None,
+                                     1 if separate else 0, C.byref(taken), stream))
+    return bool(taken.value)
 PROBLEM_SINGLE_LABEL, PROBLEM_REGRESSION_L1, PROBLEM_REGRESSION_MSE, PROBLEM_MULTI_LABEL, PROBLEM_AUC = 0, 1, 2, 3, 4
 PROBLEM_TOKEN_CE_INTRA = 6
 PROBLEM_TOKEN_CE = 5
diff --git a/graph-gpt_amd/build.py b/graph-gpt_amd/build.py
--- a/graph-gpt_amd/build.py
+++ b/graph-gpt_amd/build.py
@@ -11,7 +11,7 @@
 LIBDIR = os.path.join(HERE, "lib")
 LIB = os.path.join(LIBDIR, "libgget_hip.so")
 SOURCES = ["engine.hip", "gemm.hip", "kernels.hip", "attention.hip", "menu.hip", "metrics.hip"]
-HEADERS = ["common.h", "gemm.h", "kernels.h", "menu.h", os.path.join("..", "..", "include", "gget.h")]
+HEADERS = ["common.h", "gemm.h", "kernels.h", "menu.h", "norm_bwd.h", os.path.join("..", "..", "include", "gget.h")]
 FLAGS = ["--offload-arch=gfx950", "-O3", "-std=c++17", "-fPIC", "-fno-gpu-rdc", "-Wall", "-Wno-unused-function"]
 EXTRA_FLAGS = {}
 
diff --git a/graph-gpt_amd/csrc/engine.hip b/graph-gpt_amd/csrc/engine.hip
--- a/graph-gpt_amd/csrc/engine.hip
+++ b/graph-gpt_amd/csrc/engine.hip
@@ -1681,6 +1681,17 @@
                             reinterpret_cast<const GgetSegment*>(h->W + h->ws.segs) + bs.first, bs.second, st);
 }
 
+GemmSideJob wgrad_side_norm_job(const bf16_t* dy, const bf16_t* x, const bf16_t* w, const float* rstd, const bf16_t* dres, bf16_t* dx,
+                                float* dw_accum, int T, int d, int copies, uint64_t copy_stride) {
+  GemmSideJob s;
+  memset(&s, 0, sizeof(s));
+  s.kind = kSideRmsnormBwd;
+  s.blocks = std::min(menu().wgrad_side_norm > 1 ? menu().wgrad_side_norm : gget_gemm_num_cu(), 4096);
+  s.lds_bytes = 8 * d * (int)sizeof(float);
+  s.norm = NormBwdArgs{dy, x, w, rstd, dres, dx, dw_accum, T, d, copies < 1 ? 1 : copies, copy_stride};
+  return s;
+}
+
 int layer_backward(gget_engine* h, int i, hipStream_t st) {
   const gget_config_t& c = h->cfg;
   const int T = h->T, d = c.hidden_size, ff = c.intermediate_size, H = c.num_heads;
@@ -1766,11 +1777,15 @@
   if (int e = gemm_nn(dqkv, h->P + lo.wqkv, dxn, T, d, 3 * d, 3 * d, d, d, nullptr, st)) return e;
   const bool boundary = h->truncated() && i == h->frozen;
   const bool fuse_next = fuse_ls && i > 0 && !boundary;
+  const bool side_norm = menu().wgrad_side_norm > 0 && !boundary && !h->plan.has_res && d % 192 == 0 && ff % 192 == 0 && d <= 1024 &&
+                         !menu().deterministic && menu().gemm_lds_headroom < 2 && menu().gemm_cu_reserve == 0 && T > 0;
+  auto norm1_bwd = [&]() {
+    return k_rmsnorm_bwd(dxn, x_in, h->P + lo.ln1, h->wsp<float>(lw.rstd1), dx_mid, dx_in, s32 + lo.ln1_32, T, d, st, kAccumCopies, align_up((uint64_t)d, 128));
+  };
   if (boundary) {
     if (int e = k_rmsnorm_dw(dxn, x_in, h->wsp<float>(lw.rstd1), s32 + lo.ln1_32, T, d, st, kAccumCopies, align_up((uint64_t)d, 128))) return e;
-  } else if (!fuse_next)
-    if (int e = k_rmsnorm_bwd(dxn, x_in, h->P + lo.ln1, h->wsp<float>(lw.rstd1), dx_mid, dx_in, s32 + lo.ln1_32, T, d, st, kAccumCopies, align_up((uint64_t)d, 128)))
-      return e;
+  } else if (!fuse_next && !side_norm)
+    if (int e = norm1_bwd()) return e;
   const GemmProblem wg_gu{dgu, h->wsp<bf16_t>(lw.xn2), h->G + lo.wgu, nullptr, 2 * ff, d, T, 2 * ff, d, d, nullptr, nullptr, 0, 0};
   const GemmProblem wg_dn{dy_down, h->wsp<bf16_t>(lw.h), h->G + lo.wdown, nullptr, d, ff, T, d, ff, ff, nullptr, nullptr, 0, 0};
   const long t192[4] = {(long)2 * ff * d / (192 * 192), (long)d * ff / (192 * 192), (long)3 * d * d / (192 * 192), (long)d * d / (192 * 192)};
@@ -1791,9 +1806,14 @@
     g.p[3] = GemmProblem{dy_o, h->wsp<bf16_t>(lw.attn), h->G + lo.wo, nullptr, d, d, T, d, d, d, nullptr, nullptr, 0, 0};
     const long wg_tiles = ((long)2 * ff * d + (long)d * ff + (long)4 * d * d) / (192 * 192);
     g.sq_partials = n_grouped == 4 && h->opt_norm_from_backward && wg_tiles <= kSqTilesPerLayer ? h->wsp<float>(w.sq_tiles) + (size_t)i * kSqTilesPerLayer : nullptr;
+    if (side_norm && n_grouped == 4)
+      g.side = wgrad_side_norm_job(dxn, x_in, h->P + lo.ln1, h->wsp<float>(lw.rstd1), dx_mid, dx_in, s32 + lo.ln1_32, T, d, kAccumCopies,
+                                   align_up((uint64_t)d, 128));
     if (h->probe) GGET_HIP_CHECK(hipEventRecord(h->probe_event(0, 2 * i), st));
     if (int e = gget_gemm_launch(GGET_GEMM_TN, GGET_EPI_NONE, g, 1, st)) return e;
     if (h->probe) GGET_HIP_CHECK(hipEventRecord(h->probe_event(0, 2 * i + 1), st));
+    if (side_norm && !g.side_taken)
+      if (int e = norm1_bwd()) return e;
     if (g.sq_written) {
       if (wg_tiles < kSqTilesPerLayer)
         GGET_HIP_CHECK(hipMemsetAsync(h->wsp<float>(w.sq_tiles) + (size_t)i * kSqTilesPerLayer + wg_tiles, 0, (kSqTilesPerLayer - wg_tiles) * sizeof(float), st));
@@ -2369,6 +2389,16 @@
   return 0;
 }
 
+extern "C" int gget_debug_norm1_operands(gget_handle_t h, int layer, const void** dy, const void** x, const float** rstd, int* rows) {
+  GGET_REQUIRE(h && dy && x && rstd && rows, "null argument");
+  GGET_REQUIRE(layer >= 0 && layer < h->cfg.num_layers && h->fwd_valid, "debug_norm1_operands: layer %d out of range, or no forward", layer);
+  *dy = h->wsp<bf16_t>(h->ws.dxn);
+  *x = h->wsp<bf16_t>(h->ws.xres[layer]);
+  *rstd = h->wsp<float>(h->ws.lw[layer].rstd1);
+  *rows = h->T;
+  return 0;
+}
+
 extern "C" int gget_hidden_states_grid(gget_handle_t h, int layer, void* out_dev, void* stream) {
   GGET_REQUIRE(h && out_dev, "null argument");
   GGET_REQUIRE(layer >= -1 && layer <= h->cfg.num_layers, "hidden_states_grid: layer %d out of range", layer);
@@ -2472,6 +2502,35 @@
     p.M = M[i]; p.N = N[i]; p.K = K[i]; p.lda = lda[i]; p.ldb = ldb[i]; p.ldc = ldc[i];
   }
   return gget_gemm_launch(mode, GGET_EPI_NONE, g, 1, (hipStream_t)stream);
+}
+extern "C" int gget_op_wgrad_norm_bwd(const void* const* A, const void* const* B, void* const* Cs, const int* M, const int* N, int T,
+                                      const void* dy, const void* x, const void* w, const float* rstd, const void* dres, void* dx,
+                                      float* dw_accum, int d, int copies, uint64_t copy_stride, float* sq_tiles, int separate,
+                                      int* side_taken, void* stream) {
+  GGET_REQUIRE(A && B && Cs && M && N && dy && x && w && rstd && dx && dw_accum, "wgrad_norm_bwd: null argument");
+  GGET_REQUIRE(T >= 0 && T % 64 == 0 && d > 0 && d % 8 == 0 && d <= 1024, "wgrad_norm_bwd: bad shape T %d d %d", T, d);
+  hipStream_t st = (hipStream_t)stream;
+  GemmGroup g;
+  memset(&g, 0, sizeof(g));
+  g.count = 4;
+  for (int i = 0; i < 4; ++i) {
+    GemmProblem& p = g.p[i];
+    p.A = static_cast<const bf16_t*>(A[i]); p.B = static_cast<const bf16_t*>(B[i]); p.C = Cs[i];
+    p.M = M[i]; p.N = N[i]; p.K = T; p.lda = M[i]; p.ldb = N[i]; p.ldc = N[i];
+  }
+  g.sq_partials = sq_tiles;
+  auto norm = [&]() { return k_rmsnorm_bwd(dy, x, w, rstd, dres, dx, dw_accum, T, d, st, copies, copy_stride); };
+  if (separate) {
+    if (int e = norm()) return e;
+  } else if (T > 0) {
+    g.side = wgrad_side_norm_job(static_cast<const bf16_t*>(dy), static_cast<const bf16_t*>(x), static_cast<const bf16_t*>(w), rstd,
+                                 static_cast<const bf16_t*>(dres), static_cast<bf16_t*>(dx), dw_accum, T, d, copies, copy_stride);
+  }
+  if (int e = gget_gemm_launch(GGET_GEMM_TN, GGET_EPI_NONE, g, 1, st)) return e;
+  if (side_taken) *side_taken = g.side_taken;
+  GGET_REQUIRE(!sq_tiles || g.sq_written, "wgrad_norm_bwd: the launch that was chosen writes no tile partials");
+  if (!separate && !g.side_taken) return norm();
+  return 0;
 }
 extern "C" int gget_op_qkv_rope(const void* x, const void* wqkv, void* qkv, const float* cos_tab, const float* sin_tab,
                                 const int64_t* position_ids, int T, int S, int d, void* stream) {
diff --git a/graph-gpt_amd/csrc/gemm.h b/graph-gpt_amd/csrc/gemm.h
--- a/graph-gpt_amd/csrc/gemm.h
+++ b/graph-gpt_amd/csrc/gemm.h
@@ -2,6 +2,7 @@
 #include <hip/hip_runtime.h>
 #include "../../include/gget.h"
 #include "common.h"
+#include "norm_bwd.h"
 
 #define GGET_MAX_GROUP 4
 
@@ -30,6 +31,14 @@
   int b_tile_rows;
 };
 
+enum : int { kSideNone = 0, kSideRmsnormBwd = 1 };
+struct GemmSideJob {
+  int kind;
+  int blocks;
+  int lds_bytes;
+  NormBwdArgs norm;
+};
+
 struct GemmGroup {
   GemmProblem p[GGET_MAX_GROUP];
   int count;
@@ -43,6 +52,8 @@
   int stagger_ticks;
   float* sq_partials;
   int sq_written;
+  GemmSideJob side;
+  int side_taken;
 };
 
 constexpr size_t kStreamKBlocks = 512;
diff --git a/graph-gpt_amd/csrc/gemm.hip b/graph-gpt_amd/csrc/gemm.hip
--- a/graph-gpt_amd/csrc/gemm.hip
+++ b/graph-gpt_amd/csrc/gemm.hip
@@ -923,7 +923,9 @@
   }
 }
 
-template <int BM, int BN, bool A_MC, bool B_MC, int EPI, int NSLOT_ = 0, int DW = 8>
+long long g_side_launches = 0;
+
+template <int BM, int BN, bool A_MC, bool B_MC, int EPI, int NSLOT_ = 0, int DW = 8, bool SIDE = false>
 __global__ void __launch_bounds__(512, 2) gemm_ks_kernel(const GemmGroup g, int total_tiles) {
   extern __shared__ __attribute__((aligned(16))) unsigned char smem[];
   constexpr int BK = 64, NT = DW * 64;
@@ -938,7 +940,16 @@
   static_assert(8 * HT * 64 * 16 <= NSLOT * STAGE, "accumulator exchange fits in the ring");
   static_assert(!TB::WRAP, "only the A tile may have a wrapped piece list");
 
-  const int G = gridDim.x;
+  const int G = SIDE ? ((total_tiles + 7) & ~7) : (int)gridDim.x;
+  if constexpr (SIDE) {
+    if ((int)blockIdx.x >= G) {
+      const NormBwdArgs& a = g.side.norm;
+      if (((int)blockIdx.x - G) * 8 >= a.T) return;
+      rmsnorm_bwd_rows<2, 8>((int)blockIdx.x - G, (int)gridDim.x - G, reinterpret_cast<float*>(smem), a.dy, a.x, a.w, a.rstd, a.dres, a.dx,
+                             a.dw_accum, a.T, a.d, a.copies, a.copy_stride, nullptr);
+      return;
+    }
+  }
   const int tile = (blockIdx.x & 7) * (G >> 3) + (blockIdx.x >> 3);
   if (tile >= total_tiles) return;
   const int tid = threadIdx.x, lane = tid & 63;
@@ -1105,6 +1116,25 @@
     GGET_HIP_CHECK(hipFuncSetAttribute(reinterpret_cast<const void*>(&gemm_ks_kernel<BM, BN, A_MC, B_MC, EPI, NSLOT_, DW>),
                                        hipFuncAttributeMaxDynamicSharedMemorySize, SM));
     attr0 = true;
+  }
+  if constexpr (BM == 192 && BN == 192 && A_MC && B_MC && EPI == GGET_EPI_NONE) {
+    if (g.side.kind != kSideNone && g.side.blocks > 0) {
+      const NormBwdArgs& a = g.side.norm;
+      GGET_REQUIRE(g.side.kind == kSideRmsnormBwd, "gemm: unknown side job %d", g.side.kind);
+      GGET_REQUIRE(a.d % 8 == 0 && a.d <= 1024 && a.T >= 0 && a.copies >= 1 && g.side.lds_bytes >= 8 * a.d * (int)sizeof(float) && g.side.lds_bytes <= SM,
+                   "gemm: side job: d %d lds %d (launch %d)", a.d, g.side.lds_bytes, SM);
+      static bool attr1 = false;
+      if (!attr1) {
+        GGET_HIP_CHECK(hipFuncSetAttribute(reinterpret_cast<const void*>(&gemm_ks_kernel<BM, BN, A_MC, B_MC, EPI, NSLOT_, DW, true>),
+                                           hipFuncAttributeMaxDynamicSharedMemorySize, SM));
+        attr1 = true;
+      }
+      hipLaunchKernelGGL((gemm_ks_kernel<BM, BN, A_MC, B_MC, EPI, NSLOT_, DW, true>), dim3(G + g.side.blocks), dim3(512), SM, st, g, total);
+      GGET_LAUNCH_CHECK();
+      g.side_taken = 1;
+      ++g_side_launches;
+      return 0;
+    }
   }
   hipLaunchKernelGGL((gemm_ks_kernel<BM, BN, A_MC, B_MC, EPI, NSLOT_, DW>), dim3(G), dim3(512), SM, st, g, total);
   GGET_LAUNCH_CHECK();
@@ -1397,6 +1427,12 @@
 
 void gget_gemm_streamk_workspace(void* ws) { t_streamk_ws = ws; }
 
+extern "C" int gget_debug_side_launches(int64_t* n) {
+  GGET_REQUIRE(n != nullptr, "debug_side_launches: null argument");
+  *n = g_side_launches;
+  return 0;
+}
+
 struct GemmProbeRec { hipEvent_t e0, e1; double flops; bool dyn; };
 static std::deque<GemmProbeRec> g_probe;
 static bool g_probe_on = false;
@@ -1407,6 +1443,7 @@
   g.sk_rounds = g.sk_rem = g.sk_a = 0; g.sk_parts = 1;
   g.cu_slots = nullptr; g.stagger_ticks = 0;
   g.sq_written = 0;
+  g.side_taken = 0;
   const LaunchMenu& m = menu();
   g.ablate = m.gemm_ablate > 0 ? m.gemm_ablate : 0;
   g.super = m.gemm_super > 0 ? m.gemm_super : (mode == GGET_GEMM_TN ? 1 : kSuper);
diff --git a/graph-gpt_amd/csrc/kernels.hip b/graph-gpt_amd/csrc/kernels.hip
--- a/graph-gpt_amd/csrc/kernels.hip
+++ b/graph-gpt_amd/csrc/kernels.hip
@@ -1,5 +1,6 @@
 #include "common.h"
 #include "kernels.h"
+#include "norm_bwd.h"
 
 static float* g_det_scratch = nullptr;
 static size_t g_det_bytes = 0;
@@ -390,84 +391,7 @@
                                                              float* __restrict__ dw_accum, int T, int d, int copies,
                                                              uint64_t copy_stride, float* __restrict__ dw_part) {
   extern __shared__ float dw_lds[];
-  const int lane = threadIdx.x & 63, wave = threadIdx.x >> 6;
-  const int nchunk = d >> 3;
-  float dwp[NCH][8];
-  float wv[NCH][8];
-#pragma unroll
-  for (int i = 0; i < NCH; ++i) {
-    const int c = lane + i * 64;
-#pragma unroll
-    for (int e = 0; e < 8; ++e) dwp[i][e] = 0.f;
-    if (c < nchunk) unpack8(ldg16(w + c * 8), wv[i]);
-  }
-  const int stride = gridDim.x * (kBlock / 64);
-  int row = blockIdx.x * (kBlock / 64) + wave;
-  uint4 xr[NCH], dr[NCH], rr[NCH];
-  float rstd = 0.f;
-  auto fetch = [&](int r) {
-    rstd = rstd_in[r];
-#pragma unroll
-    for (int i = 0; i < NCH; ++i) {
-      const int c = lane + i * 64;
-      if (c < nchunk) {
-        xr[i] = ldg16(x + (size_t)r * d + c * 8);
-        dr[i] = ldg16(dy + (size_t)r * d + c * 8);
-        rr[i] = dres ? ldg16(dres + (size_t)r * d + c * 8) : make_uint4(0, 0, 0, 0);
-      }
-    }
-  };
-  if (row < T) fetch(row);
-  for (; row < T; row += stride) {
-    const float rs = rstd;
-    float xh[NCH][8], g[NCH][8], res[NCH][8];
-    float dot = 0.f;
-#pragma unroll
-    for (int i = 0; i < NCH; ++i) {
-      const int c = lane + i * 64;
-      if (c < nchunk) {
-        float xv[8], dv[8];
-        unpack8(xr[i], xv);
-        unpack8(dr[i], dv);
-        unpack8(rr[i], res[i]);
-#pragma unroll
-        for (int e = 0; e < 8; ++e) {
-          xh[i][e] = xv[e] * rs;
-          g[i][e] = dv[e] * wv[i][e];
-          dot += g[i][e] * xh[i][e];
-          dwp[i][e] += dv[e] * xh[i][e];
-        }
-      }
-    }
-    if (row + stride < T) fetch(row + stride);
-    dot = wave_sum(dot) / (float)d;
-#pragma unroll
-    for (int i = 0; i < NCH; ++i) {
-      const int c = lane + i * 64;
-      if (c < nchunk) {
-        float o[8];
-#pragma unroll
-        for (int e = 0; e < 8; ++e) o[e] = res[i][e] + rs * (g[i][e] - xh[i][e] * dot);
-        stg16(dx + (size_t)row * d + c * 8, pack8(o));
-      }
-    }
-  }
-#pragma unroll
-  for (int i = 0; i < NCH; ++i) {
-    const int c = lane + i * 64;
-    if (c < nchunk) {
-      *reinterpret_cast<float4*>(dw_lds + wave * d + c * 4) = make_float4(dwp[i][0], dwp[i][1], dwp[i][2], dwp[i][3]);
-      *reinterpret_cast<float4*>(dw_lds + wave * d + (d >> 1) + c * 4) = make_float4(dwp[i][4], dwp[i][5], dwp[i][6], dwp[i][7]);
-    }
-  }
-  __syncthreads();
-  for (int t = threadIdx.x; t < d; t += kBlock) {
-    const int hd = d >> 1, pl = t >= hd ? 1 : 0, ix = t - pl * hd;
-    const int j = (ix >> 2) * 8 + pl * 4 + (ix & 3);
-    const float s = dw_lds[t] + dw_lds[d + t] + dw_lds[2 * d + t] + dw_lds[3 * d + t];
-    if (dw_part) dw_part[(size_t)blockIdx.x * d + j] = s;
-    else unsafeAtomicAdd(dw_accum + (size_t)(blockIdx.x % copies) * copy_stride + j, s);
-  }
+  rmsnorm_bwd_rows<NCH, kBlock / 64>((int)blockIdx.x, (int)gridDim.x, dw_lds, dy, x, w, rstd_in, dres, dx, dw_accum, T, d, copies, copy_stride, dw_part);
 }
 
 template <int NCH>
diff --git a/graph-gpt_amd/csrc/menu.h b/graph-gpt_amd/csrc/menu.h
--- a/graph-gpt_amd/csrc/menu.h
+++ b/graph-gpt_amd/csrc/menu.h
@@ -34,6 +34,7 @@
   int count_copy;
   int embed_sorted;
   int occupy_fat;
+  int wgrad_side_norm;
   int deterministic;
   int rms_wide;
   int rms_rows;
@@ -78,6 +79,7 @@
     {&LaunchMenu::gemm_cu_reserve, 15, nullptr, false, 0, "CUs every GEMM plan leaves free for a collective's workgroups"},
     {&LaunchMenu::occupy_fat, 16, nullptr, false, 0, "1: gget_debug_occupy's stand-in takes RCCL's register footprint"},
     {&LaunchMenu::link_grid, 18, nullptr, false, 0, "> 0: most workgroups a streaming launch of the link metrics takes (0: 1024)"},
+    {&LaunchMenu::wgrad_side_norm, 19, "GGET_WGRAD_SIDE_NORM", false, 1, "input_layernorm backward inside the grouped weight-gradient launch: 0 off, 1 one side block per CU, n > 1 n side blocks"},
     {&LaunchMenu::gemm_num_cu, 0, "GGET_GEMM_NUM_CU", false, 0, "> 0: GEMM plans pretend the chip has this many CUs"},
     {&LaunchMenu::gemm_no_persist, 0, "GGET_GEMM_NO_PERSIST", true, 0, "set: no persistent GEMM kernels"},
     {&LaunchMenu::gemm_no_dyn, 0, "GGET_GEMM_NO_DYN", true, 0, "set: no persistent GEMM kernels for device-sized launches"},
diff --git a/graph-gpt_amd/csrc/norm_bwd.h b/graph-gpt_amd/csrc/norm_bwd.h
--- /dev/null
+++ b/graph-gpt_amd/csrc/norm_bwd.h
@@ -0,0 +1,110 @@
+#pragma once
+#include "common.h"
+
+struct NormBwdArgs {
+  const bf16_t* dy;
+  const bf16_t* x;
+  const bf16_t* w;
+  const float* rstd;
+  const bf16_t* dres;
+  bf16_t* dx;
+  float* dw_accum;
+  int T, d, copies;
+  uint64_t copy_stride;
+};
+
+#ifdef __HIPCC__
+__device__ __forceinline__ uint4 nb_ldg16(const bf16_t* p) { return *reinterpret_cast<const uint4*>(p); }
+__device__ __forceinline__ void nb_stg16(bf16_t* p, const uint4& v) {
+  typedef unsigned u4nt __attribute__((ext_vector_type(4)));
+  __builtin_nontemporal_store(u4nt{v.x, v.y, v.z, v.w}, reinterpret_cast<u4nt*>(p));
+}
+
+template <int NCH, int NW>
+__device__ __forceinline__ void rmsnorm_bwd_rows(const int blk, const int nblk, float* dw_lds, const bf16_t* __restrict__ dy,
+                                                 const bf16_t* __restrict__ x, const bf16_t* __restrict__ w,
+                                                 const float* __restrict__ rstd_in, const bf16_t* __restrict__ dres,
+                                                 bf16_t* __restrict__ dx, float* __restrict__ dw_accum, int T, int d, int copies,
+                                                 uint64_t copy_stride, float* __restrict__ dw_part) {
+  const int lane = threadIdx.x & 63, wave = threadIdx.x >> 6;
+  const int nchunk = d >> 3;
+  float dwp[NCH][8];
+  float wv[NCH][8];
+#pragma unroll
+  for (int i = 0; i < NCH; ++i) {
+    const int c = lane + i * 64;
+#pragma unroll
+    for (int e = 0; e < 8; ++e) dwp[i][e] = 0.f;
+    if (c < nchunk) unpack8(nb_ldg16(w + c * 8), wv[i]);
+  }
+  const int stride = nblk * NW;
+  int row = blk * NW + wave;
+  uint4 xr[NCH], dr[NCH], rr[NCH];
+  float rstd = 0.f;
+  auto fetch = [&](int r) {
+    rstd = rstd_in[r];
+#pragma unroll
+    for (int i = 0; i < NCH; ++i) {
+      const int c = lane + i * 64;
+      if (c < nchunk) {
+        xr[i] = nb_ldg16(x + (size_t)r * d + c * 8);
+        dr[i] = nb_ldg16(dy + (size_t)r * d + c * 8);
+        rr[i] = dres ? nb_ldg16(dres + (size_t)r * d + c * 8) : make_uint4(0, 0, 0, 0);
+      }
+    }
+  };
+  if (row < T) fetch(row);
+  for (; row < T; row += stride) {
+    const float rs = rstd;
+    float xh[NCH][8], g[NCH][8], res[NCH][8];
+    float dot = 0.f;
+#pragma unroll
+    for (int i = 0; i < NCH; ++i) {
+      const int c = lane + i * 64;
+      if (c < nchunk) {
+        float xv[8], dv[8];
+        unpack8(xr[i], xv);
+        unpack8(dr[i], dv);
+        unpack8(rr[i], res[i]);
+#pragma unroll
+        for (int e = 0; e < 8; ++e) {
+          xh[i][e] = xv[e] * rs;
+          g[i][e] = dv[e] * wv[i][e];
+          dot += g[i][e] * xh[i][e];
+          dwp[i][e] += dv[e] * xh[i][e];
+        }
+      }
+    }
+    if (row + stride < T) fetch(row + stride);
+    dot = wave_sum(dot) / (float)d;
+#pragma unroll
+    for (int i = 0; i < NCH; ++i) {
+      const int c = lane + i * 64;
+      if (c < nchunk) {
+        float o[8];
+#pragma unroll
+        for (int e = 0; e < 8; ++e) o[e] = res[i][e] + rs * (g[i][e] - xh[i][e] * dot);
+        nb_stg16(dx + (size_t)row * d + c * 8, pack8(o));
+      }
+    }
+  }
+#pragma unroll
+  for (int i = 0; i < NCH; ++i) {
+    const int c = lane + i * 64;
+    if (c < nchunk) {
+      *reinterpret_cast<float4*>(dw_lds + wave * d + c * 4) = make_float4(dwp[i][0], dwp[i][1], dwp[i][2], dwp[i][3]);
+      *reinterpret_cast<float4*>(dw_lds + wave * d + (d >> 1) + c * 4) = make_float4(dwp[i][4], dwp[i][5], dwp[i][6], dwp[i][7]);
+    }
+  }
+  __syncthreads();
+  for (int t = threadIdx.x; t < d; t += NW * 64) {
+    const int hd = d >> 1, pl = t >= hd ? 1 : 0, ix = t - pl * hd;
+    const int j = (ix >> 2) * 8 + pl * 4 + (ix & 3);
+    float s = dw_lds[t];
+#pragma unroll
+    for (int v = 1; v < NW; ++v) s += dw_lds[v * d + t];
+    if (dw_part) dw_part[(size_t)blk * d + j] = s;
+    else unsafeAtomicAdd(dw_accum + (size_t)(blk % copies) * copy_stride + j, s);
+  }
+}
+#endif
diff --git a/include/gget.h b/include/gget.h
--- a/include/gget.h
+++ b/include/gget.h
@@ -199,6 +199,12 @@
 uint64_t gget_op_gemm_streamk_bytes(void);
 int gget_op_gemm_grouped(int mode, int count, const void* const* A, const void* const* B, void* const* C, const int* M,
                          const int* N, const int* K, const int* lda, const int* ldb, const int* ldc, void* stream);
+int gget_op_wgrad_norm_bwd(const void* const* A, const void* const* B, void* const* C, const int* M, const int* N, int T,
+                           const void* dy, const void* x, const void* w, const float* rstd, const void* dres, void* dx,
+                           float* dw_accum, int d, int copies, uint64_t copy_stride, float* sq_tiles, int separate,
+                           int* side_taken, void* stream);
+int gget_debug_side_launches(int64_t* n);
+int gget_debug_norm1_operands(gget_handle_t h, int layer, const void** dy, const void** x, const float** rstd, int* rows);
 int gget_debug_set(int key, int value);
 int gget_debug_get(int key, int* value);
 int gget_debug_probe(gget_handle_t h, int enable, float* avg_ms_out);
```

After: 782,000 graph-tokens/s. No clear change (-0.0%).
